# wangxb29/PPST

Hardware: AMD Instinct MI355X
Metric: 512x512 portrait swaps/sec/GPU (higher is better)
Workload: dtype bf16x3 (fp32 split into hi+lo bf16, 3 MFMA passes, fp32 accumulate); 1 GPU; simple_swapping 512x512 batch=8 per GPU, generator+encoders forward only (BASELINE configs[1]); image_parallel=1 batch per rank, no data-path collective

## Files before the change

### include/ppst_hip.h

```cpp
#ifndef PPST_HIP_H
#define PPST_HIP_H

#include <stddef.h>
#include <stdint.h>

#ifdef __cplusplus
extern "C" {
#endif

#define PPST_OK 0
#define PPST_EINVAL (-1)
#define PPST_EUNSUPPORTED (-2)
#define PPST_ENULL (-3)

enum { PPST_F32 = 0, PPST_F16 = 1, PPST_BF16 = 2, PPST_F64 = 3  };

enum { PPST_PAD_ZERO = 0, PPST_PAD_REFLECT = 1, PPST_PAD_REPLICATE = 2 };

enum { PPST_ACT_NONE = 0, PPST_ACT_LRELU = 1 , PPST_ACT_PRELU = 2 };

#define PPST_ABI_VERSION 3
int ppst_version(void);

#define PPST_ST_F32 0
// ... 80 lines not shown
  const void* noise;
  const void* prelu;
  void* stats;
  const void* residual;
  float noise_weight;
  float out_scale;
  int32_t B, in_h, in_w, in_ld;
  int32_t out_h, out_w, out_ld, cout;
  int32_t nsteps, n_groups;
  int32_t pad_mode;
  int32_t in_off_y, in_off_x;
  int32_t out_sy, out_sx;
  int32_t act;
  int32_t precision;
  int32_t res_ld;
  int32_t tile_h, tile_w;
  int32_t halo;
  int32_t bn;
  const void* in_scale_shift;
  const void* in_prelu;
  int32_t in_c, in_act;
  int32_t flop_steps;
  int32_t tile_rows;
  int32_t a_slots;
  int32_t early_a;
  int32_t variant;
  int32_t reserved0;
  int32_t dual_b;
  int32_t io_st;
  int32_t k64;
  const void* in_res;
  int32_t in_res_ld;
  int32_t ksplit;
  const int32_t* ksplit_starts;
  void* ksplit_scratch;
  unsigned* ksplit_flags;
  uint32_t ksplit_epoch;
} ppst_conv_args;

int ppst_conv2d_mfma(const ppst_conv_args* a, void* stream);
int64_t ppst_conv_pack_wino_bytes(int cout, int cin);
int ppst_conv_pack_wino(const void* w, int64_t sn, int64_t sc, int64_t sy, int64_t sx, float scale, int cout, int cin,
                        void* out, void* stream);
int ppst_conv2d_f32(const ppst_conv_args* a, const void* w, int64_t sn, int64_t sc, int64_t sy, int64_t sx, float wscale,
                    const int32_t* src_c, const int32_t* src_ky, const int32_t* src_kx, void* stream);
int ppst_conv_tiles(int tile_h, int tile_w, int tile_rows);

int ppst_conv1x1_small_cin(const void* x, const void* w, const void* bias, void* y,
                           int64_t npix, int cin, int in_ld, int cout, float wscale,
                           int act, void* stream);
int ppst_conv1x1_small_cin_st(const void* x, const void* w, const void* bias, void* y,
                              int64_t npix, int cin, int in_ld, int cout, float wscale,
                              int act, int y_st , void* stream);
int ppst_conv1x1_small_cout(const void* x, const void* w, const void* bias, void* y,
                            int64_t npix, int cin, int cout, float wscale, void* stream);
int ppst_conv1x1_small_cout_st(const void* x, const void* w, const void* bias, void* y,
                               int64_t npix, int cin, int cout, float wscale, int x_st , void* stream);
int ppst_torgb_apply_st(const void* x, const void* scale_shift, const void* res, int res_ld, float out_scale, const void* w,
                        const void* bias, void* y, int B, int H, int W, int cin, float wscale, int x_st, void* stream);

int ppst_in_stats(const void* x, void* partial, int B, int H, int W, int C, int ld,
                  int rep_pad, int* n_partials, void* stream);
int ppst_in_finalize(const void* partial, int n_partials, const void* style,
                     int style_ld ,
                     const void* post_bias ,
                     void* scale_shift , int B, int C, double count,
                     float eps, void* stream);
int ppst_affine_act(const void* x, const void* scale_shift, const void* res,
                    const void* res_scale_shift , void* y,
                    int B, int64_t hw, int C, int x_ld, int res_ld, int y_ld,
                    int act , const void* prelu,
                    float out_scale,
                    int res_up2_w ,
                    void* stream);
int ppst_affine_act_st(const void* x, const void* scale_shift, const void* res, const void* res_scale_shift, void* y,
                       int B, int64_t hw, int C, int x_ld, int res_ld, int y_ld, int act, const void* prelu,
                       float out_scale, int res_up2_w, int x_st, int y_st, void* stream);
int ppst_affine_act_stats(const void* x, const void* scale_shift, const void* res,
                          const void* res_scale_shift, void* y, void* partial,
                          int B, int H, int W, int C, int x_ld, int res_ld, int y_ld,
                          int act, const void* prelu, float out_scale, int rep_pad,
                          int res_up2 , void* stream);
int ppst_upsample_nearest2(const void* x, void* y, int B, int H, int W, int C, void* stream);
int ppst_upsample_nearest2_st(const void* x, void* y, int B, int H, int W, int C, int st, void* stream);

int64_t ppst_gap_gmp_ws(int B, int64_t hw, int C);
int ppst_gap_gmp(const void* x, const void* mask, void* out, void* ws, int B, int H, int W,
                 int C, int ld, void* stream);
int ppst_gap_gmp_st(const void* x, const void* mask, void* out, void* ws, int B, int H, int W,
                    int C, int ld, int x_st, void* stream);
int ppst_avgpool(const void* x, void* y, int B, int H, int W, int C, int x_ld, int f,
                 int y_ld, void* stream);
int ppst_bilinear(const void* x, void* y, int B, int H, int W, int C, int x_ld,
                  int OH, int OW, int y_ld, void* stream);
int ppst_head_tail(const void* x, const void* scale_shift, const void* prelu, void* feat, void* feat1,
                   int B, int H, int W, int C, int x_ld, int feat_ld, int feat1_ld, int P, int D, int act,
                   void* stream);
int ppst_maxpool2(const void* x, void* y, int B, int H, int W, int C, void* stream);

int ppst_linear(const void* x, const void* w, const void* bias, void* y,
                int B, int K, int N, float wscale, float bscale, int relu_in, int act,
                void* stream);
int ppst_l2norm_rows(const void* x, void* y, int B, int K, float eps, int mode, void* stream);
int ppst_lerp(const void* a, const void* b, void* y, int64_t n, float r, void* stream);
int ppst_spatial_modulation(const void* x, const void* scale, const void* bias, void* y,
                            int B, int64_t hw, int C, void* stream);
// ... 160 lines not shown
```

### ppst_amd/_lib.py

```python
import ctypes
import os

import torch

HERE = os.path.dirname(os.path.abspath(__file__))
LIB_PATH = os.environ.get("PPST_HIP_LIB") or os.path.join(HERE, "libppst_hip.so")

if not os.path.exists(LIB_PATH):
    raise ImportError(
        "ppst_amd: %s is missing -- build it with `python -m ppst_amd.build` "
        "(hipcc --offload-arch=gfx950). There is no CPU fallback." % LIB_PATH)

lib = ctypes.CDLL(LIB_PATH)

vp, i32, i64, f32, f64 = ctypes.c_void_p, ctypes.c_int, ctypes.c_int64, ctypes.c_float, ctypes.c_double


class PackJob(ctypes.Structure):
    _fields_ = [("w", vp), ("sn", i64), ("sc", i64), ("sy", i64), ("sx", i64), ("src_c", vp), ("src_ky", vp), ("src_kx", vp),
                ("out", vp), ("total", i64), ("block0", i64), ("scale", f32), ("cout", i32), ("bn", i32), ("nsteps", i32),
                ("n_groups", i32), ("x3", i32), ("f16", i32), ("nblocks", i32), ("dual", i32)]


class UpscaleJob(ctypes.Structure):
    _fields_ = [("w", vp), ("out", vp), ("total", i64), ("block0", i64), ("scale", f32), ("cout", i32), ("cin", i32), ("nblocks", i32)]


class ConvArgs(ctypes.Structure):
    _fields_ = [
        ("x", vp), ("wpack", vp), ("steps", vp), ("y", vp), ("bias", vp), ("noise", vp),
        ("prelu", vp), ("stats", vp), ("residual", vp),
        ("noise_weight", f32), ("out_scale", f32),
        ("B", i32), ("in_h", i32), ("in_w", i32), ("in_ld", i32),
        ("out_h", i32), ("out_w", i32), ("out_ld", i32), ("cout", i32),
        ("nsteps", i32), ("n_groups", i32), ("pad_mode", i32),
        ("in_off_y", i32), ("in_off_x", i32), ("out_sy", i32), ("out_sx", i32),
        ("act", i32), ("precision", i32), ("res_ld", i32), ("tile_h", i32), ("tile_w", i32),
        ("halo", i32), ("bn", i32), ("in_scale_shift", vp), ("in_prelu", vp), ("in_c", i32), ("in_act", i32),
        ("flop_steps", i32), ("tile_rows", i32), ("a_slots", i32), ("early_a", i32), ("variant", i32), ("reserved0", i32), ("dual_b", i32), ("io_st", i32), ("k64", i32),
        ("in_res", vp), ("in_res_ld", i32), ("ksplit", i32), ("ksplit_starts", vp),
        ("ksplit_scratch", vp), ("ksplit_flags", vp), ("ksplit_epoch", ctypes.c_uint32),
    ]


_SIGS = {
    "ppst_version": (i32, []),
    "ppst_guided_filter_tune": (i32, [i32, i32]),
    "ppst_upfirdn2d": (i32, [vp, vp, vp] + [i32] * 14 + [i32, vp]),
    "ppst_blur_nhwc": (i32, [vp, vp, vp] + [i32] * 10 + [vp, i32, vp]),
    "ppst_blur_nhwc_st": (i32, [vp, vp, vp] + [i32] * 10 + [vp, i32, i32, vp]),
    "ppst_fused_bias_act": (i32, [vp, vp, vp, vp, i64, i32, i32, i32, i32, f32, f32, i32, vp]),
    "ppst_nchw_to_nhwc": (i32, [vp, vp, i32, i32, i32, i32, vp]),
    "ppst_nhwc_to_nchw": (i32, [vp, vp, i32, i32, i32, i32, vp]),
    "ppst_conv_pack": (i32, [vp, i64, i64, i64, i64, f32, i32, i32, vp, vp, vp, i32, i32, i32, vp, vp]),
    "ppst_conv_pack_k64": (i32, [vp, i64, i64, i64, i64, f32, i32, i32, vp, vp, vp, i32, i32, i32, i32, vp, vp]),
    "ppst_conv_pack_up9_bytes": (i64, [i32, i32]),
    "ppst_conv_pack_up9": (i32, [vp, i64, i64, i64, i64, f32, i32, i32, vp, vp]),
    "ppst_conv_pack_wino_bytes": (i64, [i32, i32]),
    "ppst_conv_pack_wino": (i32, [vp, i64, i64, i64, i64, f32, i32, i32, vp, vp]),
    "ppst_conv_pack_dual": (i32, [vp, i64, i64, i64, i64, f32, i32, vp, vp, vp, i32, i32, i32, vp, vp]),
    "ppst_upscale_weight": (i32, [vp, vp, i32, i32, f32, vp]),
    "ppst_dgrad_s2d_stack_weight": (i32, [vp, vp, i32, i32, vp]),
    "ppst_depth_to_space_st": (i32, [vp, vp, i32, i32, i32, i32, i32, i32, i32, vp]),
    "ppst_pack_job_blocks": (i32, [i64]),
    "ppst_conv_pack_batch": (i32, [vp, i32, i32, vp]),
    "ppst_upscale_weight_batch": (i32, [vp, i32, i32, vp]),
    "ppst_conv2d_mfma": (i32, [ctypes.POINTER(ConvArgs), vp]),
    "ppst_conv2d_f32": (i32, [ctypes.POINTER(ConvArgs), vp, i64, i64, i64, i64, f32, vp, vp, vp, vp]),
    "ppst_conv_tiles": (i32, [i32, i32, i32]),
    "ppst_conv1x1_small_cin": (i32, [vp, vp, vp, vp, i64, i32, i32, i32, f32, i32, vp]),
    "ppst_conv1x1_small_cin_st": (i32, [vp, vp, vp, vp, i64, i32, i32, i32, f32, i32, i32, vp]),
    "ppst_conv1x1_small_cout": (i32, [vp, vp, vp, vp, i64, i32, i32, f32, vp]),
    "ppst_conv1x1_small_cout_st": (i32, [vp, vp, vp, vp, i64, i32, i32, f32, i32, vp]),
    "ppst_torgb_apply_st": (i32, [vp, vp, vp, i32, f32, vp, vp, vp, i32, i32, i32, i32, f32, i32, vp]),
    "ppst_in_stats": (i32, [vp, vp, i32, i32, i32, i32, i32, i32, ctypes.POINTER(i32), vp]),
    "ppst_in_finalize": (i32, [vp, i32, vp, i32, vp, vp, i32, i32, f64, f32, vp]),
    "ppst_affine_act": (i32, [vp, vp, vp, vp, vp, i32, i64, i32, i32, i32, i32, i32, vp, f32, i32, vp]),
    "ppst_affine_act_st": (i32, [vp, vp, vp, vp, vp, i32, i64, i32, i32, i32, i32, i32, vp, f32, i32, i32, i32, vp]),
    "ppst_affine_act_stats": (i32, [vp, vp, vp, vp, vp, vp, i32, i32, i32, i32, i32, i32, i32, i32, vp, f32, i32, i32, vp]),
    "ppst_upsample_nearest2": (i32, [vp, vp, i32, i32, i32, i32, vp]),
    "ppst_upsample_nearest2_st": (i32, [vp, vp, i32, i32, i32, i32, i32, vp]),
    "ppst_gap_gmp_ws": (i64, [i32, i64, i32]),
    "ppst_gap_gmp": (i32, [vp, vp, vp, vp, i32, i32, i32, i32, i32, vp]),
    "ppst_gap_gmp_st": (i32, [vp, vp, vp, vp, i32, i32, i32, i32, i32, i32, vp]),
    "ppst_avgpool": (i32, [vp, vp, i32, i32, i32, i32, i32, i32, i32, vp]),
    "ppst_bilinear": (i32, [vp, vp, i32, i32, i32, i32, i32, i32, i32, i32, vp]),
    "ppst_head_tail": (i32, [vp, vp, vp, vp, vp] + [i32] * 10 + [vp]),
    "ppst_maxpool2": (i32, [vp, vp, i32, i32, i32, i32, vp]),
    "ppst_linear": (i32, [vp, vp, vp, vp, i32, i32, i32, f32, f32, i32, i32, vp]),
    "ppst_l2norm_rows": (i32, [vp, vp, i32, i32, f32, i32, vp]),
    "ppst_lerp": (i32, [vp, vp, vp, i64, f32, vp]),
    "ppst_spatial_modulation": (i32, [vp, vp, vp, vp, i32, i64, i32, vp]),
    "ppst_spatial_modulation_st": (i32, [vp, vp, vp, vp, i32, i64, i32, i32, vp]),
    "ppst_rselfcorr": (i32, [vp, vp, i32, i32, i32, i32, i32, vp]),
    "ppst_corr_prep": (i32, [vp, vp, i32, i32, i32, i32, vp]),
    "ppst_gemm_nt_f32": (i32, [vp, vp, vp, i32, i32, i32, i32, f32, vp]),
    "ppst_gemm_nn_f32": (i32, [vp, vp, vp, i32, i32, i32, i32, i32, i32, vp]),
    "ppst_unfold_rows": (i32, [vp, vp, i32, i32, i32, i32, i32, vp]),
    "ppst_unfold_rows_bwd": (i32, [vp, vp, i32, i32, i32, i32, i32, vp]),
    "ppst_gemm_nt_split": (i32, [vp, vp, vp, i32, i32, i32, i32, f32, i32, vp]),
    "ppst_gemm_nn_split": (i32, [vp, vp, vp, i32, i32, i32, i32, i32, i32, i32, vp]),
    "ppst_softmax_rows": (i32, [vp, i64, i32, f32, vp]),
    "ppst_unfold_patches": (i32, [vp, vp, i32, i32, i32, i32, i32, vp]),
    "ppst_fold_patches": (i32, [vp, vp, i32, i32, i32, i32, i32, vp]),
    "ppst_tensor2im_u8": (i32, [vp, vp, i32, i32, i32, i32, vp]),
    "ppst_resample_u8": (i32, [vp, vp, i32, i32, i32, i32, i32, i32, vp, vp, i32, vp]),
    "ppst_u8_to_tensor": (i32, [vp, vp, i32, i32, i32, i32, f32, f32, vp]),
    "ppst_png_bound": (i64, [i32, i32, i32]),
    "ppst_png_ws": (i64, [i32, i32, i32, i32]),
    "ppst_png_encode": (i32, [vp, vp, vp, i32, i32, i32, i32, vp, vp]),
    "ppst_lpips_pack_floats": (i64, []),
    "ppst_lpips_pack": (i32, [vp, vp, vp, vp, vp, vp, vp]),
    "ppst_lpips_dims": (i32, [i32, i32, ctypes.POINTER(i32)]),
    "ppst_lpips_ws": (i64, [i32, i32, i32]),
    "ppst_lpips_trunk": (i32, [vp, vp, ctypes.POINTER(i64), i32, vp, ctypes.POINTER(i64), i32, i32, i32, vp, vp]),
    "ppst_lpips_feature": (i32, [vp, i32, i32, i32, i32, vp, vp]),
    "ppst_lpips_tail": (i32, [vp, vp, i32, i32, i32, vp, vp]),
    "ppst_lpips_bwd_ws": (i64, [i32, i32, i32, i32]),
    "ppst_lpips_backward": (i32, [vp, vp, vp, i32, i32, i32, i32, vp, vp, vp, vp]),
    "ppst_guided_filter_ws": (i64, [i32, i32, i32]),
    "ppst_guided_filter": (i32, [vp, vp, vp, vp, i32, i32, i32, i32, f32, vp, vp]),
    "ppst_smooth_local_affine_ws": (i64, [i32, i32, i32]),
    "ppst_smooth_local_affine": (i32, [vp, vp, vp, vp, vp, i32, i32, i32, i32, i32, f32, f32, vp]),
    "ppst_conv_wgrad_f32": (i32, [vp, vp, vp, vp, vp] + [i32] * 11 + [vp]),
# ... 83 lines not shown
```

### ppst_amd/build.py

```python
import os
import subprocess
import sys
from concurrent.futures import ThreadPoolExecutor

HERE = os.path.dirname(os.path.abspath(__file__))
CSRC = os.path.join(HERE, "csrc")
OBJ = os.path.join(HERE, "csrc", "_obj")
LIB = os.path.join(HERE, "libppst_hip.so")
SOURCES = ["upfirdn2d.hip", "fused_bias_act.hip", "elementwise.hip", "linear.hip", "conv_mfma.hip", "conv_mfma2.hip", "conv1x1.hip", "conv_wino.hip", "conv_f32.hip",
           "corr.hip", "guided_filter.hip", "train.hip", "train_g.hip", "imageio.hip", "smooth_filter.hip", "png.hip", "lpips.hip"]
FLAGS = ["--offload-arch=gfx950", "-O3", "-fPIC", "-std=c++17", "-Wno-unused-result"]
FILE_FLAGS = {"conv_wino.hip": ["-fno-slp-vectorize"]}


def _hipcc():
    for c in (os.environ.get("HIPCC"), "/opt/rocm/bin/hipcc", "hipcc"):
        if c and (os.path.isabs(c) and os.path.exists(c) or not os.path.isabs(c)):
            return c
    return "hipcc"


HEADERS = [os.path.join(CSRC, "common.h"), os.path.join(CSRC, "rscl_common.h"), os.path.join(HERE, "..", "include", "ppst_hip.h")]


def _stale(target, deps):
    return not os.path.exists(target) or any(os.path.getmtime(d) > os.path.getmtime(target) for d in deps)


def needs_build():
    return (_stale(LIB, [os.path.join(CSRC, s) for s in SOURCES] + HEADERS) or
            any(_stale(os.path.join(OBJ, s.replace(".hip", ".o")), [os.path.join(CSRC, s)]) for s in SOURCES if os.path.isdir(OBJ)))


def build(force=False, verbose=True):
    if not force and not needs_build():
        return LIB
    os.makedirs(OBJ, exist_ok=True)
    hipcc = _hipcc()

    def cc(src):
        obj = os.path.join(OBJ, src.replace(".hip", ".o"))
        if not force and not _stale(obj, [os.path.join(CSRC, src)] + HEADERS):
            return obj
        cmd = [hipcc] + FLAGS + FILE_FLAGS.get(src, []) + ["-c", os.path.join(CSRC, src), "-o", obj]
        r = subprocess.run(cmd, capture_output=True, text=True)
        if r.returncode != 0:
            raise RuntimeError("hipcc failed for %s:\n%s" % (src, r.stderr))
        return obj

    order = sorted(SOURCES, key=lambda f: 0 if f.startswith("conv") else 1)
    with ThreadPoolExecutor(max_workers=8) as ex:
        objs = dict(zip(order, ex.map(cc, order)))
    cmd = [hipcc, "--offload-arch=gfx950", "-shared", "-fPIC", "-o", LIB] + [objs[s_] for s_ in SOURCES]
    r = subprocess.run(cmd, capture_output=True, text=True)
    if r.returncode != 0:
        raise RuntimeError("link failed:\n%s" % r.stderr)
    if verbose:
        print("built", LIB)
    return LIB


if __name__ == "__main__":
    build(force="--force" in sys.argv)
```

### ppst_amd/csrc/conv1x1.hip

```cpp
#include "common.h"

struct C1Args {
  const float* x;
  const unsigned char* wpack;
  const int4* steps;
  float* y;
  const float* bias;
  const float* noise;
  const float* prelu;
  float* stats;
  const float* residual;
  float noise_weight, out_scale;
  int B, hw, in_ld, out_ld, cout, nsteps, act, res_ld, n_tiles, tiles;
  int in_h, in_w, out_h, out_w, tiles_x, pad_mode;
  const float* in_ss;
  const float* in_prelu;
  int in_c, in_act;
  const float* in_res;
  int in_res_ld;
};

#define C1_GROUP 8
#define C1_BLOB 8192

typedef _Float16 __attribute__((ext_vector_type(8))) c1_half8;
template <int PREC>
__device__ __forceinline__ void c1_cvt(float v, unsigned short& h, unsigned short& l) {
  if (PREC == 0) split_bf16(v, h, l);
  else if (PREC == 3) { h = __builtin_bit_cast(unsigned short, (_Float16)v); l = 0; }
  else { h = f2bf(v); l = 0; }
}
template <int PREC>
__device__ __forceinline__ void c1_cvt8(const float (&v)[8], bf16x8& hi, bf16x8& lo) {
  if (PREC == 3) {
#pragma unroll
    for (int j = 0; j < 8; ++j) {
      unsigned short h, l;
      c1_cvt<PREC>(v[j], h, l);
      hi[j] = (short)h;
      lo[j] = (short)l;
    }
    return;
  }
  uint2 h0, l0 = make_uint2(0u, 0u), h1, l1 = make_uint2(0u, 0u);
  if (PREC == 0) {
    split_bf16x4(make_float4(v[0], v[1], v[2], v[3]), h0, l0);
    split_bf16x4(make_float4(v[4], v[5], v[6], v[7]), h1, l1);
  } else {
    h0 = f2bf_x4(make_float4(v[0], v[1], v[2], v[3]));
    h1 = f2bf_x4(make_float4(v[4], v[5], v[6], v[7]));
  }
  hi = __builtin_bit_cast(bf16x8, make_uint4(h0.x, h0.y, h1.x, h1.y));
  lo = __builtin_bit_cast(bf16x8, make_uint4(l0.x, l0.y, l1.x, l1.y));
// ... 241 lines not shown
        if (IOS != PPST_ST_F32 && !INSS) {
          const float4 z = vok[mt] ? raw[mt][0] : make_float4(0.f, 0.f, 0.f, 0.f);
          ah[mt] = __builtin_bit_cast(bf16x8, z);
          al[mt] = ah[mt];
          continue;
        }
        float v[8] = {raw[mt][0].x, raw[mt][0].y, raw[mt][0].z, raw[mt][0].w, raw[mt][1].x, raw[mt][1].y, raw[mt][1].z, raw[mt][1].w};
        if (IOS != PPST_ST_F32) c1_unpack8<IOS>(raw[mt][0], v);
        if (INSS) {
          const float sc[8] = {ss[0].x, ss[0].z, ss[1].x, ss[1].z, ss[2].x, ss[2].z, ss[3].x, ss[3].z};
          const float sh[8] = {ss[0].y, ss[0].w, ss[1].y, ss[1].w, ss[2].y, ss[2].w, ss[3].y, ss[3].w};
#pragma unroll
          for (int j = 0; j < 8; ++j) {
            float t = sc[j] * v[j] + sh[j];
            if (INSS == 2) {
              const float4 r4 = rres[mt][j >> 2];
              t += (j & 3) == 0 ? r4.x : (j & 3) == 1 ? r4.y : (j & 3) == 2 ? r4.z : r4.w;
            }
            v[j] = in_act(t);
          }
        }
#pragma unroll
        for (int j = 0; j < 8; ++j)
          if (!vok[mt]) v[j] = 0.f;
        c1_cvt8<PREC>(v, ah[mt], al[mt]);
      }
      if (s + 1 < a.nsteps) a_load(steps[s + 1]);
      const unsigned char* bs = (const unsigned char*)sB + sl * BLOB1 + g * 1024 + r16 * 16;
#pragma unroll
      for (int nt = 0; nt < NT; ++nt) {
        const bf16x8 bh = *(const bf16x8*)(bs + nt * 256);
        bf16x8 bl = bh;
        if (X3) bl = *(const bf16x8*)(bs + nt * 256 + 4096);
#pragma unroll
        for (int mt = 0; mt < MT; ++mt) acc[mt][nt] = c1_mfma<PREC>(bh, bl, ah[mt], al[mt], acc[mt][nt]);
      }
    }
  }

  c1_epilogue<MT, NT, TAPS, X3, IOS>(a, acc, red, b, mblk, ntile, pbase, oy0, ox, tid, wave, r16, g);
}

#define C3_GROUP 9
template <int CTRL>
__device__ __forceinline__ bf16x8 c3_shift(bf16x8 edge, bf16x8 centre) {
  typedef int __attribute__((ext_vector_type(4))) i4;
  const i4 e = __builtin_bit_cast(i4, edge), c = __builtin_bit_cast(i4, centre);
  i4 r;
#pragma unroll
  for (int i = 0; i < 4; ++i) r[i] = __builtin_amdgcn_update_dpp(e[i], c[i], CTRL, 0xf, 0xf, false);
  return __builtin_bit_cast(bf16x8, r);
}

template <bool INSS, int NT_, int PREC = 0, int IOS = PPST_ST_F32>
__global__ __launch_bounds__(512, NT_ > 4 ? 2 : 4) void conv3x3_direct_kernel(C1Args a) {
  constexpr int MT = 2, NT = NT_;
  constexpr bool X3 = PREC == 0;
  static_assert(IOS == PPST_ST_F32 || IOS == (PREC == 3 ? PPST_ST_F16 : PREC == 1 ? PPST_ST_BF16 : -1), "half storage: single-pass modes");
  constexpr int ES = IOS == PPST_ST_F32 ? 4 : 2;
  constexpr int PSTR = (NT > 4 ? 128 : 64) * 16;
  constexpr int BLOB = (X3 ? 8 : 4) * PSTR;
  __shared__ uint4 sB[C3_GROUP * BLOB / 16];
  __shared__ float red[8][NT > 4 ? 128 : 64][2];
  const int tid = threadIdx.x, lane = tid & 63, wave = __builtin_amdgcn_readfirstlane(tid >> 6);
  const int r16 = lane & 15, g = lane >> 4;
  const int total = a.B * a.tiles * a.n_tiles;
  const int per = (total + (int)gridDim.x - 1) / (int)gridDim.x;
  const int w_beg = blockIdx.x * per, w_end = w_beg + per < total ? w_beg + per : total;
  const int nchunks = a.nsteps / 9;
  const bool keep_b = nchunks == 1 && a.n_tiles == 1;
  for (int wid = w_beg; wid < w_end; ++wid) {
  const int ntile = wid % a.n_tiles;
  int mblk = wid / a.n_tiles;
  const int b = mblk / a.tiles;
  mblk -= b * a.tiles;
  const int tyi = mblk / a.tiles_x, txi = mblk - tyi * a.tiles_x;
  const int oy0 = tyi * 16 + wave * 2, ox = txi * 16 + r16;
  const unsigned char* xb = (const unsigned char*)a.x + (int64_t)b * a.in_h * a.in_w * a.in_ld * ES;
  const unsigned char* wblob = a.wpack + (int64_t)ntile * a.nsteps * BLOB;
  if (wid > w_beg) __syncthreads();
#if defined(__HIP_DEVICE_COMPILE__)
  typedef const __attribute__((address_space(4))) int4* StepPtr;
#else
  typedef const int4* StepPtr;
#endif
  StepPtr steps = (StepPtr)a.steps;
  const float in_slope = (INSS && a.in_act == PPST_ACT_PRELU && a.in_prelu) ? a.in_prelu[0] : 0.f;
  auto in_act = [&](float t) -> float {
    if (a.in_act == PPST_ACT_LRELU) return (t > 0.f ? t : t * 0.2f) * 1.41421356237309515f;
    if (a.in_act == PPST_ACT_PRELU) return t >= 0.f ? t : t * in_slope;
    return t;
  };
  const int xe_raw = r16 == 0 ? ox - 1 : (r16 == 15 ? ox + 1 : ox);
  const bool cx_ok = ox < a.in_w, ex_ok = xe_raw >= 0 && xe_raw < a.in_w;
  const int cx = c1_pad(ox, a.in_w, a.pad_mode), ex = c1_pad(xe_raw, a.in_w, a.pad_mode);

  f32x4 acc[MT][NT];
#pragma unroll
  for (int i = 0; i < MT; ++i)
#pragma unroll
    for (int j = 0; j < NT; ++j) acc[i][j] = (f32x4){0.f, 0.f, 0.f, 0.f};

  float4 rawc[2], rawe[2], ss[4];
  bool okc = false, oke = false;
  auto row_load = [&](int chan, int r) {
    int iy = oy0 - 1 + r;
    const bool yok = iy >= 0 && iy < a.in_h;
    iy = c1_pad(iy, a.in_h, a.pad_mode);
    okc = a.pad_mode != PPST_PAD_ZERO || (yok && cx_ok);
    oke = a.pad_mode != PPST_PAD_ZERO || (yok && ex_ok);
    const float4* pc = (const float4*)(xb + (((int64_t)iy * a.in_w + cx) * a.in_ld + chan + g * 8) * ES);
    const float4* pe = (const float4*)(xb + (((int64_t)iy * a.in_w + ex) * a.in_ld + chan + g * 8) * ES);
    rawc[0] = pc[0];
    rawe[0] = pe[0];
    if (IOS == PPST_ST_F32) { rawc[1] = pc[1]; rawe[1] = pe[1]; }
  };
  auto ss_load = [&](int chan) {
    if (INSS) {
      const float4* q = (const float4*)(a.in_ss + ((int64_t)b * a.in_c + chan + g * 8) * 2);
      ss[0] = q[0]; ss[1] = q[1]; ss[2] = q[2]; ss[3] = q[3];
    }
  };
  auto convert = [&](const float4 (&raw)[2], bool ok, bf16x8& hi, bf16x8& lo) {
    if (IOS != PPST_ST_F32 && !INSS) {
      hi = __builtin_bit_cast(bf16x8, ok ? raw[0] : make_float4(0.f, 0.f, 0.f, 0.f));
      lo = hi;
      return;
    }
    float v[8] = {raw[0].x, raw[0].y, raw[0].z, raw[0].w, raw[1].x, raw[1].y, raw[1].z, raw[1].w};
    if (IOS != PPST_ST_F32) c1_unpack8<IOS>(raw[0], v);
    if (INSS) {
      const float sc[8] = {ss[0].x, ss[0].z, ss[1].x, ss[1].z, ss[2].x, ss[2].z, ss[3].x, ss[3].z};
      const float sh[8] = {ss[0].y, ss[0].w, ss[1].y, ss[1].w, ss[2].y, ss[2].w, ss[3].y, ss[3].w};
#pragma unroll
      for (int j = 0; j < 8; ++j) v[j] = in_act(sc[j] * v[j] + sh[j]);
    }
#pragma unroll
    for (int j = 0; j < 8; ++j)
      if (!ok) v[j] = 0.f;
    c1_cvt8<PREC>(v, hi, lo);
  };

  int chan = steps[0].x;
  ss_load(chan);
  row_load(chan, 0);
  for (int c = 0; c < nchunks; ++c) {
    if (!keep_b || wid == w_beg) {
      if (c) __syncthreads();
      for (int i = tid; i < C3_GROUP * (BLOB / 16); i += 512) sB[i] = ((const uint4*)(wblob + (int64_t)c * C3_GROUP * BLOB))[i];
      __syncthreads();
    }
    const int chan_next = c + 1 < nchunks ? steps[(c + 1) * 9].x : chan;
#pragma unroll
    for (int r = 0; r < 4; ++r) {
      bf16x8 ch, cl, eh, el;
      convert(rawc, okc, ch, cl);
      convert(rawe, oke, eh, el);
      if (r < 3) row_load(chan, r + 1);
      else if (c + 1 < nchunks) { ss_load(chan_next); row_load(chan_next, 0); }
#pragma unroll
      for (int dxi = 0; dxi < 3; ++dxi) {
        const bf16x8 fh = dxi == 0 ? c3_shift<0x111>(eh, ch) : (dxi == 1 ? ch : c3_shift<0x101>(eh, ch));
        const bf16x8 fl = dxi == 0 ? c3_shift<0x111>(el, cl) : (dxi == 1 ? cl : c3_shift<0x101>(el, cl));
#pragma unroll
        for (int mt = 0; mt < MT; ++mt) {
          const int dyi = r - mt;
          if (dyi < 0 || dyi > 2) continue;
          const unsigned char* bs = (const unsigned char*)sB + (dyi * 3 + dxi) * BLOB + g * PSTR + r16 * 16;
#pragma unroll
          for (int nt = 0; nt < NT; ++nt) {
            const bf16x8 bh = *(const bf16x8*)(bs + nt * 256);
            bf16x8 bl = bh;
            if (X3) bl = *(const bf16x8*)(bs + nt * 256 + 4 * PSTR);
            acc[mt][nt] = c1_mfma<PREC>(bh, bl, fh, fl, acc[mt][nt]);
          }
        }
// ... 13 lines not shown
  k.bias = (const float*)a->bias; k.noise = (const float*)a->noise; k.prelu = (const float*)a->prelu;
  k.stats = (float*)a->stats; k.residual = (const float*)a->residual;
  k.noise_weight = a->noise_weight; k.out_scale = a->out_scale;
  k.B = a->B; k.hw = a->out_h * a->out_w; k.in_ld = a->in_ld; k.out_ld = a->out_ld; k.cout = a->cout; k.nsteps = a->nsteps;
  k.act = a->act; k.res_ld = a->res_ld; k.n_tiles = n_tiles; k.tiles = tiles;
  k.in_ss = (const float*)a->in_scale_shift; k.in_prelu = (const float*)a->in_prelu; k.in_c = a->in_c; k.in_act = a->in_act;
  k.in_res = (const float*)a->in_res; k.in_res_ld = a->in_res_ld;
  if ((int64_t)tiles * 256 < k.hw) return PPST_EINVAL;
  if (k.in_res) {
    PPST_LAUNCH((conv1x1_stream_kernel<2, false, 4, 0, PPST_ST_F32>), dim3((unsigned)blocks_of(a, tiles, n_tiles)), dim3(512), 0, st, k);
    return PPST_LAUNCH_CHECK();
  }
  const int64_t blocks = (int64_t)a->B * tiles * n_tiles;
  if (blocks > 0x7fffffff) return PPST_EINVAL;
#define LS(PREC_, IOS_)                                                                                               \
  do {                                                                                                                \
    if (k.in_ss) PPST_LAUNCH((conv1x1_stream_kernel<1, false, 4, PREC_, IOS_>), dim3((unsigned)blocks), dim3(512), 0, st, k);   \
    else PPST_LAUNCH((conv1x1_stream_kernel<0, false, 4, PREC_, IOS_>), dim3((unsigned)blocks), dim3(512), 0, st, k);          \
  } while (0)
  if (a->precision == 1) { if (a->io_st) LS(1, PPST_ST_BF16); else LS(1, PPST_ST_F32); }
  else if (a->precision == 3) { if (a->io_st) LS(3, PPST_ST_F16); else LS(3, PPST_ST_F32); }
  else LS(0, PPST_ST_F32);
#undef LS
  return PPST_LAUNCH_CHECK();
}

int ppst_conv_direct_launch(const ppst_conv_args* a, int n_tiles, int tiles_y, int tiles_x, hipStream_t st) {
  C1Args k;
  k.x = (const float*)a->x; k.wpack = (const unsigned char*)a->wpack; k.steps = (const int4*)a->steps; k.y = (float*)a->y;
  k.bias = (const float*)a->bias; k.noise = (const float*)a->noise; k.prelu = (const float*)a->prelu;
  k.stats = (float*)a->stats; k.residual = (const float*)a->residual;
  k.noise_weight = a->noise_weight; k.out_scale = a->out_scale;
  k.B = a->B; k.hw = a->out_h * a->out_w; k.in_ld = a->in_ld; k.out_ld = a->out_ld; k.cout = a->cout; k.nsteps = a->nsteps;
  k.act = a->act; k.res_ld = a->res_ld; k.n_tiles = n_tiles; k.tiles = tiles_y * tiles_x;
  k.in_ss = (const float*)a->in_scale_shift; k.in_prelu = (const float*)a->in_prelu; k.in_c = a->in_c; k.in_act = a->in_act;
  k.in_h = a->in_h; k.in_w = a->in_w; k.out_h = a->out_h; k.out_w = a->out_w; k.tiles_x = tiles_x; k.pad_mode = a->pad_mode;
  const int64_t blocks = (int64_t)a->B * k.tiles * n_tiles;
  if (blocks > 0x7fffffff) return PPST_EINVAL;
  const bool nt2 = a->cout <= 32;
#define LD(INSS_, PREC_, IOS_)                                                                                       \
  do {                                                                                                               \
    if (nt2) PPST_LAUNCH((conv1x1_stream_kernel<INSS_, true, 2, PREC_, IOS_>), dim3((unsigned)blocks), dim3(512), 0, st, k);       \
    else PPST_LAUNCH((conv1x1_stream_kernel<INSS_, true, 4, PREC_, IOS_>), dim3((unsigned)blocks), dim3(512), 0, st, k);           \
  } while (0)
#define LDP(PREC_, IOS_) do { if (k.in_ss) LD(1, PREC_, IOS_); else LD(0, PREC_, IOS_); } while (0)
  if (a->precision == 1) { if (a->io_st) LDP(1, PPST_ST_BF16); else LDP(1, PPST_ST_F32); }
  else if (a->precision == 3) { if (a->io_st) LDP(3, PPST_ST_F16); else LDP(3, PPST_ST_F32); }
  else LDP(0, PPST_ST_F32);
#undef LDP
#undef LD
  return PPST_LAUNCH_CHECK();
}

int ppst_conv3x3_direct_launch(const ppst_conv_args* a, int n_tiles, int tiles_y, int tiles_x, hipStream_t st) {
  if (a->nsteps % 9) return PPST_EINVAL;
  C1Args k;
  k.x = (const float*)a->x; k.wpack = (const unsigned char*)a->wpack; k.steps = (const int4*)a->steps; k.y = (float*)a->y;
  k.bias = (const float*)a->bias; k.noise = (const float*)a->noise; k.prelu = (const float*)a->prelu;
  k.stats = (float*)a->stats; k.residual = (const float*)a->residual;
  k.noise_weight = a->noise_weight; k.out_scale = a->out_scale;
  k.B = a->B; k.hw = a->out_h * a->out_w; k.in_ld = a->in_ld; k.out_ld = a->out_ld; k.cout = a->cout; k.nsteps = a->nsteps;
  k.act = a->act; k.res_ld = a->res_ld; k.n_tiles = n_tiles; k.tiles = tiles_y * tiles_x;
  k.in_ss = (const float*)a->in_scale_shift; k.in_prelu = (const float*)a->in_prelu; k.in_c = a->in_c; k.in_act = a->in_act;
  k.in_h = a->in_h; k.in_w = a->in_w; k.out_h = a->out_h; k.out_w = a->out_w; k.tiles_x = tiles_x; k.pad_mode = a->pad_mode;
  int64_t blocks = (int64_t)a->B * k.tiles * n_tiles;
  if (blocks > 0x7fffffff) return PPST_EINVAL;
  if (a->nsteps == 9 && n_tiles == 1 && blocks > 512) blocks = 512;
  const bool nt2 = a->cout <= 32, nt8 = a->bn == 128;
#define LD3(INSS_, PREC_, IOS_)                                                                                      \
  do {                                                                                                               \
    if (nt8 && PREC_ == 0) PPST_LAUNCH((conv3x3_direct_kernel<INSS_, 8, 0>), dim3((unsigned)blocks), dim3(512), 0, st, k);   \
    else if (nt8) return PPST_EUNSUPPORTED;                                                                          \
    else if (nt2) PPST_LAUNCH((conv3x3_direct_kernel<INSS_, 2, PREC_, IOS_>), dim3((unsigned)blocks), dim3(512), 0, st, k); \
    else PPST_LAUNCH((conv3x3_direct_kernel<INSS_, 4, PREC_, IOS_>), dim3((unsigned)blocks), dim3(512), 0, st, k);          \
  } while (0)
#define LD3P(PREC_, IOS_) do { if (k.in_ss) LD3(true, PREC_, IOS_); else LD3(false, PREC_, IOS_); } while (0)
  if (a->precision == 1) { if (a->io_st) LD3P(1, PPST_ST_BF16); else LD3P(1, PPST_ST_F32); }
  else if (a->precision == 3) { if (a->io_st) LD3P(3, PPST_ST_F16); else LD3P(3, PPST_ST_F32); }
  else LD3P(0, PPST_ST_F32);
#undef LD3P
#undef LD3
  return PPST_LAUNCH_CHECK();
}
```

### ppst_amd/csrc/conv_mfma.hip

```cpp
#include "common.h"

struct ConvKArgs {
  const float* x;
  const unsigned short* wpack;
  const int4* steps;
  float* y;
  const float* bias;
  const float* noise;
  const float* prelu;
  float* stats;
  const float* residual;
  float noise_weight, out_scale;
  int B, in_h, in_w, in_ld, out_h, out_w, out_ld, cout;
  int nsteps, n_groups, pad_mode, in_off_y, in_off_x, out_sy, out_sx, act, res_ld, tile_h, tile_w;
  int tiles_y, tiles_x, n_tiles;
  const float* in_ss;
  const float* in_prelu;
  int in_c, in_act;
  int early_a;
  unsigned long long* dbg;
  KSplitDev ks;
  int prefetch_w;
};

__device__ __forceinline__ int pad_index(int i, int n, int mode) {
  if (mode == PPST_PAD_REFLECT) {
    if (i < 0) i = -i;
    if (i >= n) i = 2 * (n - 1) - i;
  }
  i = i < 0 ? 0 : (i >= n ? n - 1 : i);
  return i;
}

#ifdef PPST_CONV_CLOCK
__device__ unsigned long long* g_clock_buf = nullptr;
__device__ int g_clock_n = 1;
extern "C" int ppst_conv_clock_buffer(void* buf, int n) {
  if (n <= 0) return PPST_EINVAL;
  if (hipMemcpyToSymbol(HIP_SYMBOL(g_clock_buf), &buf, sizeof(buf)) != hipSuccess) return PPST_EINVAL;
  return hipMemcpyToSymbol(HIP_SYMBOL(g_clock_n), &n, sizeof(n)) == hipSuccess ? PPST_OK : PPST_EINVAL;
}
#endif
typedef _Float16 __attribute__((ext_vector_type(8))) half8;
__device__ __forceinline__ unsigned short f2h(float f) { return __builtin_bit_cast(unsigned short, (_Float16)f); }
template <int WM, int WN, int HALO, bool X3, bool INSS, int NAS = 0, bool F16 = false, int IOS = PPST_ST_F32>
__global__ __launch_bounds__(64 * WM * WN, NAS ? 2 : 1) void conv_mfma_kernel(ConvKArgs a) {
  static_assert(IOS == PPST_ST_F32 || (!X3 && IOS == (F16 ? PPST_ST_F16 : PPST_ST_BF16)), "half storage: single-pass modes");
  constexpr int ES = IOS == PPST_ST_F32 ? 4 : 2;
  constexpr int NT = 64 * WM * WN;
  constexpr int TH = 4 * WM, TW = 16;
  constexpr int HH = TH + 2 * HALO, HW = TW + 2 * HALO, HP = HH * HW;
  constexpr int PLANE = (WM == 2) ? HP * 16 : ((HP * 16 + 255) / 256) * 256;
  constexpr int NPL = X3 ? 8 : 4;
// ... 717 lines not shown

int ppst_prof_begin_(double flop, const int* info8, hipStream_t st) {
  if (!g_prof_on) return -1;
  if (g_ev_used >= PROF_MAX) { ++g_prof_dropped; return -1; }
  while (g_ev_made <= g_ev_used) {
    if (hipEventCreate(&g_ev[g_ev_made][0]) != hipSuccess || hipEventCreate(&g_ev[g_ev_made][1]) != hipSuccess) return -1;
    ++g_ev_made;
  }
  const int slot = g_ev_used++;
  g_flop[slot] = flop;
  for (int i = 0; i < 8; ++i) g_info[slot][i] = info8[i];
  (void)hipEventRecord(g_ev[slot][0], st);
  return slot;
}
void ppst_prof_end_(int slot, hipStream_t st) {
  if (slot >= 0) (void)hipEventRecord(g_ev[slot][1], st);
}

extern "C" int ppst_prof_enable(int on) {
  g_prof_on = on;
  g_ev_used = 0;
  if (on) g_prof_dropped = 0;
  return PPST_OK;
}
extern "C" int ppst_prof_collect(double* ms, int64_t* launches, double* flop) {
  double t = 0.0, f = 0.0;
  for (int i = 0; i < g_ev_used; ++i) {
    float e = 0.f;
    hipError_t err = hipEventElapsedTime(&e, g_ev[i][0], g_ev[i][1]);
    if (err != hipSuccess) return (int)err;
    t += e;
    f += g_flop[i];
  }
  if (ms) *ms = t;
  if (launches) *launches = g_ev_used;
  if (flop) *flop = f;
  g_ev_used = 0;
  return PPST_OK;
}
extern "C" int ppst_prof_detail(int idx, double* ms, double* flop, int32_t* info) {
  if (idx < 0 || idx >= g_ev_used) return PPST_EINVAL;
  float e = 0.f;
  hipError_t err = hipEventElapsedTime(&e, g_ev[idx][0], g_ev[idx][1]);
  if (err != hipSuccess) return (int)err;
  if (ms) *ms = e;
  if (flop) *flop = g_flop[idx];
  if (info) for (int i = 0; i < 8; ++i) info[i] = g_info[idx][i];
  return PPST_OK;
}

int ppst_conv2d_mfma2_launch(const ppst_conv_args* a, int n_tiles, int tiles_y, int tiles_x, hipStream_t st);
int ppst_conv1x1_stream_launch(const ppst_conv_args* a, int n_tiles, int tiles, hipStream_t st);
int ppst_conv_direct_launch(const ppst_conv_args* a, int n_tiles, int tiles_y, int tiles_x, hipStream_t st);
int ppst_conv3x3_direct_launch(const ppst_conv_args* a, int n_tiles, int tiles_y, int tiles_x, hipStream_t st);
int ppst_conv_wino_launch(const ppst_conv_args* a, int n_tiles, int tiles_y, int tiles_x, hipStream_t st);

int ppst_ksplit_prepare_(const ppst_conv_args* a, int64_t tiles, int acc_regs, int threads, KSplitDev* out) {
  const int S = a->ksplit, nsteps = a->nsteps;
  const int32_t* starts = a->ksplit_starts;
  if ((S != 2 && S != 4 && S != 8) || (!starts && nsteps % S) || tiles <= 0 || acc_regs <= 0 || acc_regs % 4 || threads <= 0) return PPST_EINVAL;
  if (S == 8 && acc_regs > 64) return PPST_EINVAL;
  for (int i = 0; i <= S; ++i) {
    out->start[i] = starts ? starts[i] : i * (nsteps / S);
    if (i && out->start[i] <= out->start[i - 1]) return PPST_EINVAL;
  }
  if (out->start[0] != 0 || out->start[S] != nsteps) return PPST_EINVAL;
  const int64_t slots = (int64_t)(S - 1) * tiles;
  if (slots > KS_MAX_SLOTS || slots > PPST_KSPLIT_FLAG_WORDS - 1 || (size_t)slots * threads * acc_regs * 4 > PPST_KSPLIT_SCRATCH_BYTES) return PPST_EINVAL;
  if (!a->ksplit_scratch || !a->ksplit_flags) return PPST_ENULL;
  if (a->ksplit_epoch == 0) return PPST_EINVAL;
  out->scratch = (float*)a->ksplit_scratch; out->flags = a->ksplit_flags; out->epoch = a->ksplit_epoch; out->S = S;
  return PPST_OK;
}

extern "C" int ppst_conv_tiles(int tile_h, int tile_w, int tile_rows) { return cdiv(tile_h, tile_rows) * cdiv(tile_w, tile_rows == 15 ? 15 : 16); }

template <int WM, int WN, int HALO, bool X3, int NAS = 0, bool F16 = false, int IOS = PPST_ST_F32>
static void launch_conv(const ConvKArgs& k, int blocks, hipStream_t st) {
  const dim3 grid(blocks, k.ks.S > 1 ? k.ks.S : 1);
  if (k.in_ss) PPST_LAUNCH((conv_mfma_kernel<WM, WN, HALO, X3, true, NAS, F16, IOS>), grid, dim3(64 * WM * WN), 0, st, k);
  else PPST_LAUNCH((conv_mfma_kernel<WM, WN, HALO, X3, false, NAS, F16, IOS>), grid, dim3(64 * WM * WN), 0, st, k);
}

extern "C" int ppst_conv2d_mfma(const ppst_conv_args* a, void* stream) {
  if (!a) return PPST_ENULL;
  if (a->B < 0 || a->in_h <= 0 || a->in_w <= 0 || a->in_ld <= 0 || a->in_ld % 4 || a->out_h <= 0 || a->out_w <= 0 ||
      a->out_ld < a->cout || a->cout <= 0 || a->cout % 4 || a->out_ld % 4 || (a->residual && a->res_ld % 4) || a->nsteps <= 0 ||
      (a->n_groups != 1 && a->n_groups != 4 && !(a->n_groups == 2 && a->dual_b)) || a->pad_mode < 0 ||
      (a->dual_b && (a->variant != 2 || a->bn != 256 || a->n_groups != 2 || a->halo != 1 || (a->precision != 0 && a->precision != 1 && a->precision != 3) || a->out_sy != 2 || a->out_sx != 2 || !a->early_a)) ||
      a->pad_mode > 2 || a->tile_h <= 0 || a->tile_w <= 0 || a->out_sy <= 0 || a->out_sx <= 0 ||
      (a->precision != 0 && a->precision != 1 && a->precision != 3) || a->halo < 0 || a->halo > 1 || (a->bn != 64 && a->bn != 128 && a->bn != 256) || (a->residual && a->res_ld < a->cout) ||
      a->variant < 0 || a->variant > 11 || (a->variant == 0 && a->bn == 256) ||
      (a->variant == 11 && (a->precision != 0 || a->bn != 256 || a->halo != 1 || a->n_groups != 1 || a->out_sy != 2 || a->out_sx != 2 ||
                            !a->early_a || a->tile_rows != 15 || a->pad_mode != PPST_PAD_ZERO || a->in_scale_shift || a->residual ||
                            (a->act & 0xff) == PPST_ACT_PRELU || a->cout % 64 || a->nsteps % 4 || a->in_off_y || a->in_off_x ||
                            a->tile_h != a->in_h || a->tile_w != a->in_w || a->out_h != 2 * a->in_h || a->out_w != 2 * a->in_w || a->io_st)) ||
      (a->variant == 10 && (a->precision != 0 || a->bn != 128 || a->halo != 1 || a->n_groups != 1 || a->out_sy != 1 || a->out_sx != 1 ||
                            a->in_off_y != 0 || a->in_off_x != 0 || a->tile_h != a->out_h || a->tile_w != a->out_w ||
                            a->in_h != a->out_h || a->in_w != a->out_w || a->nsteps % 9 != 0 || a->tile_rows != 16 ||
                            (a->in_scale_shift && a->nsteps / 9 > 32))) ||
      ((a->variant == 2 || a->variant == 7 || a->variant == 9) &&
       ((a->precision != 0 && !((a->variant == 2 || a->variant == 7 || (a->variant == 9 && a->k64)) && (a->precision == 1 || a->precision == 3))) || a->bn == 64 || !a->early_a)) ||
      (a->variant == 7 && (a->bn != 128 || a->tile_rows != 32)) ||
      (a->variant == 9 && (a->bn != 128 || a->tile_rows != 24)) ||
      (a->variant == 2 && a->bn != 256) ||
      (a->variant == 4 && ((a->precision != 0 && a->precision != 1 && a->precision != 3) || a->bn != 64 || a->halo != 0 || a->n_groups != 1 || a->out_sy != 1 || a->out_sx != 1 ||
                           a->in_off_y != 0 || a->in_off_x != 0 || a->tile_h != a->out_h || a->tile_w != a->out_w ||
                           a->in_h != a->out_h || a->in_w != a->out_w)) ||
      (a->in_res && (a->variant != 4 || !a->in_scale_shift || a->precision != 0 || a->io_st || a->in_res_ld < a->in_c || a->in_res_ld % 4 ||
                     ((uintptr_t)a->in_res % 16))) ||
      ((a->variant == 5 || a->variant == 6) && ((a->precision != 0 && a->precision != 1 && a->precision != 3) ||
                                                (a->bn != 64 && !(a->variant == 6 && a->bn == 128 && a->precision == 0)) || a->n_groups != 1 || a->out_sy != 1 || a->out_sx != 1 ||
                           a->in_off_y != 0 || a->in_off_x != 0 || a->tile_h != a->out_h || a->tile_w != a->out_w)) ||
      (a->tile_rows != 16 && !(a->variant == 7 && a->tile_rows == 32) && !(a->variant == 9 && a->tile_rows == 24) && !(a->variant == 11 && a->tile_rows == 15) &&
       !(a->variant == 0 && a->tile_rows == 8 && a->bn == 128 && a->halo == 1 && a->early_a && a->precision == 0)) || (a->in_scale_shift && a->in_c <= 0) || a->a_slots < 0 || a->a_slots > 3)
    return PPST_EINVAL;
  if (a->variant == 1 || a->variant == 3 || (a->variant == 7 && a->precision == 0) || a->variant == 8 || (a->variant == 9 && !a->k64) ||
      a->reserved0)
    return PPST_EINVAL;
  if (a->io_st && (a->io_st != (a->precision == 3 ? PPST_ST_F16 : a->precision == 1 ? PPST_ST_BF16 : -1) ||
                   (a->tile_rows != 16 && a->variant != 7 && !(a->variant == 9 && a->k64)) ||
                   !(a->variant == 0 || a->variant == 2 || a->variant == 4 || a->variant == 5 || a->variant == 6 || a->variant == 7 || (a->variant == 9 && a->k64))))
    return PPST_EINVAL;
  if (a->k64 && (!a->io_st || !a->halo || !((a->variant == 2 && a->bn == 256) || (a->variant == 9 && a->bn == 128 && a->tile_rows == 24)) || !a->early_a))
    return PPST_EINVAL;
  {
    const int64_t px = (int64_t)a->out_h * a->out_w + 64 * (int64_t)a->out_sx;
    if (px * a->out_ld > 0x7fffffff || (a->residual && px * a->res_ld > 0x7fffffff)) return PPST_EINVAL;
  }
  if ((int64_t)a->in_h * a->in_w * a->in_ld * 4 > 0x7fffffff) return PPST_EINVAL;
  if (a->io_st && (((uintptr_t)a->x | (uintptr_t)a->y | (uintptr_t)a->residual) % 8)) return PPST_EINVAL;
  if (a->io_st && a->variant >= 4 && a->variant <= 6 && (a->in_ld % 8 || (uintptr_t)a->x % 16)) return PPST_EINVAL;
  if ((a->tile_h - 1) * a->out_sy >= a->out_h || (a->tile_w - 1) * a->out_sx >= a->out_w) return PPST_EINVAL;
  if (a->B == 0) return PPST_OK;
  if (!a->x || !a->wpack || !a->steps || !a->y) return PPST_ENULL;
  ConvKArgs k;
  k.x = (const float*)a->x; k.wpack = (const unsigned short*)a->wpack; k.steps = (const int4*)a->steps; k.y = (float*)a->y;
  k.bias = (const float*)a->bias; k.noise = (const float*)a->noise; k.prelu = (const float*)a->prelu;
  k.stats = (float*)a->stats; k.residual = (const float*)a->residual;
  k.noise_weight = a->noise_weight; k.out_scale = a->out_scale;
  k.B = a->B; k.in_h = a->in_h; k.in_w = a->in_w; k.in_ld = a->in_ld; k.out_h = a->out_h; k.out_w = a->out_w;
  k.out_ld = a->out_ld; k.cout = a->cout; k.nsteps = a->nsteps; k.n_groups = a->n_groups; k.pad_mode = a->pad_mode;
  k.in_off_y = a->in_off_y; k.in_off_x = a->in_off_x; k.out_sy = a->out_sy; k.out_sx = a->out_sx; k.act = a->act;
  k.res_ld = a->res_ld; k.tile_h = a->tile_h; k.tile_w = a->tile_w;
  k.tiles_y = cdiv(a->tile_h, a->tile_rows); k.tiles_x = cdiv(a->tile_w, a->variant == 11 ? 15 : 16);
  k.n_tiles = cdiv(a->cout, a->variant == 11 ? 64 : a->dual_b ? a->bn / 2 : a->bn);
  k.in_ss = (const float*)a->in_scale_shift; k.in_prelu = (const float*)a->in_prelu;
  k.in_c = a->in_c; k.in_act = a->in_act;
  k.early_a = a->early_a ? 1 : 0;
  k.dbg = nullptr;
  k.ks.scratch = nullptr; k.ks.flags = nullptr; k.ks.epoch = 0; k.ks.S = 1;
#ifdef PPST_CONV_TRACE
  k.dbg = (unsigned long long*)a->prelu;
  k.prelu = nullptr;
#endif
  int64_t blocks64 = (int64_t)a->n_groups * k.n_tiles * a->B * k.tiles_y * k.tiles_x;
  if (blocks64 > 0x7fffffff) return PPST_EINVAL;
  int blocks = (int)blocks64;
  hipStream_t st = as_stream(stream);
  if (a->ksplit > 1) {
    if (a->variant == 0) {
      if (a->tile_rows != 16 && a->tile_rows != 8) return PPST_EINVAL;
      const int e0 = ppst_ksplit_prepare_(a, blocks, 64, (a->bn == 128 && a->tile_rows == 16) ? 512 : 256, &k.ks);
      if (e0 != PPST_OK) return e0;
    } else if (a->variant != 2 && a->variant != 10) return PPST_EINVAL;
  }
  k.prefetch_w = (int64_t)blocks * k.ks.S <= 512 ? 1 : 0;
  int slot = -1;
  if (g_prof_on) {
    const int inf[8] = {a->B, a->tile_h, a->tile_w, a->nsteps, a->cout, a->n_groups, a->halo,
                        a->bn | (a->variant << 12) | ((a->k64 ? 1 : 0) << 20) | (a->precision << 24)};
    slot = ppst_prof_begin_(2.0 * 32.0 * (a->flop_steps > 0 ? a->flop_steps : a->nsteps) * (double)((a->dual_b || a->variant == 11) ? 4 : a->n_groups) * a->cout * (double)a->B * a->tile_h * a->tile_w,
                            inf, st);
  }
  if (a->variant >= 1) {
    int e2 = a->variant == 4   ? ppst_conv1x1_stream_launch(a, k.n_tiles, k.tiles_y * k.tiles_x, st)
             : a->variant == 5 ? ppst_conv_direct_launch(a, k.n_tiles, k.tiles_y, k.tiles_x, st)
             : a->variant == 6 ? ppst_conv3x3_direct_launch(a, k.n_tiles, k.tiles_y, k.tiles_x, st)
             : a->variant == 10 ? ppst_conv_wino_launch(a, k.n_tiles, k.tiles_y, k.tiles_x, st)
                               : ppst_conv2d_mfma2_launch(a, k.n_tiles, k.tiles_y, k.tiles_x, st);
    if (slot >= 0) (void)hipEventRecord(g_ev[slot][1], st);
    return e2;
  }
  const bool x3 = a->precision == 0;
  const bool f16 = a->precision == 3, hs = a->io_st != 0;
#define DISPATCH(WM_, WN_)                                                                                         \
  do {                                                                                                             \
    if (a->halo) { if (x3) launch_conv<WM_, WN_, 1, true>(k, blocks, st); else if (f16 && hs) launch_conv<WM_, WN_, 1, false, 0, true, PPST_ST_F16>(k, blocks, st); else if (f16) launch_conv<WM_, WN_, 1, false, 0, true>(k, blocks, st); else if (hs) launch_conv<WM_, WN_, 1, false, 0, false, PPST_ST_BF16>(k, blocks, st); else launch_conv<WM_, WN_, 1, false>(k, blocks, st); } \
    else         { if (x3) launch_conv<WM_, WN_, 0, true>(k, blocks, st); else if (f16 && hs) launch_conv<WM_, WN_, 0, false, 0, true, PPST_ST_F16>(k, blocks, st); else if (f16) launch_conv<WM_, WN_, 0, false, 0, true>(k, blocks, st); else if (hs) launch_conv<WM_, WN_, 0, false, 0, false, PPST_ST_BF16>(k, blocks, st); else launch_conv<WM_, WN_, 0, false>(k, blocks, st); } \
  } while (0)
  if (a->tile_rows == 8) launch_conv<2, 2, 1, true, 2>(k, blocks, st);
  else if (a->bn == 64 && x3 && a->halo == 1 && a->a_slots == 1) launch_conv<4, 1, 1, true, 1>(k, blocks, st);
  else if (a->bn == 64 && x3 && a->halo == 0 && a->a_slots == 1) launch_conv<4, 1, 0, true, 1>(k, blocks, st);
  else if (a->bn == 64 && x3 && a->halo == 0 && a->a_slots == 2) launch_conv<4, 1, 0, true, 2>(k, blocks, st);
  else if (a->bn == 128) DISPATCH(4, 2); else DISPATCH(4, 1);
#undef DISPATCH
  int e = PPST_LAUNCH_CHECK();
  if (slot >= 0) (void)hipEventRecord(g_ev[slot][1], st);
  return e;
}
```

### ppst_amd/csrc/elementwise.hip

```cpp
#include "common.h"

#define GRID_CAP (256 * 16)
static inline unsigned grid_for(int64_t work, int threads = 256) {
  int64_t b = cdiv64(work, threads);
  if (b > GRID_CAP) b = GRID_CAP;
  if (b < 1) b = 1;
  return (unsigned)b;
}

__device__ __forceinline__ float act_apply(float t, int act, float slope);

template <int ST = PPST_ST_F32>
__device__ __forceinline__ float4 res_up2_sample(const void* __restrict__ res, int b, int oy, int ox, int H, int W, int res_ld,
                                                 int c) {
  const int h = H >> 1, w = W >> 1;
  float fy = fmaxf(((float)oy + 0.5f) * 0.5f - 0.5f, 0.f), fx = fmaxf(((float)ox + 0.5f) * 0.5f - 0.5f, 0.f);
  int y0 = (int)fy, x0 = (int)fx;
  int y1 = y0 + (y0 < h - 1), x1 = x0 + (x0 < w - 1);
  float ly = fy - (float)y0, lx = fx - (float)x0, hy = 1.f - ly, hx = 1.f - lx;
  const int64_t base = (int64_t)b * h * w * res_ld + c;
  float4 v00 = st_ld4<ST>(res, base + ((int64_t)y0 * w + x0) * res_ld);
  float4 v01 = st_ld4<ST>(res, base + ((int64_t)y0 * w + x1) * res_ld);
  float4 v10 = st_ld4<ST>(res, base + ((int64_t)y1 * w + x0) * res_ld);
  float4 v11 = st_ld4<ST>(res, base + ((int64_t)y1 * w + x1) * res_ld);
  float4 o;
  o.x = hy * (hx * v00.x + lx * v01.x) + ly * (hx * v10.x + lx * v11.x);
  o.y = hy * (hx * v00.y + lx * v01.y) + ly * (hx * v10.y + lx * v11.y);
  o.z = hy * (hx * v00.z + lx * v01.z) + ly * (hx * v10.z + lx * v11.z);
  o.w = hy * (hx * v00.w + lx * v01.w) + ly * (hx * v10.w + lx * v11.w);
  return o;
}

__global__ __launch_bounds__(256) void nchw_to_nhwc_kernel(const float* __restrict__ x, float* __restrict__ y, int C, int64_t P) {
  __shared__ float sm[32][65];
  const int64_t p0 = (int64_t)blockIdx.x * 64;
  const int c0 = blockIdx.y * 32;
  const int b = blockIdx.z;
  const float* xb = x + (int64_t)b * C * P;
  float* yb = y + (int64_t)b * C * P;
  {
    int tp = threadIdx.x & 63, tc = threadIdx.x >> 6;
#pragma unroll
    for (int i = 0; i < 8; ++i) {
      int c = c0 + tc + i * 4;
      int64_t p = p0 + tp;
      sm[tc + i * 4][tp] = (c < C && p < P) ? xb[(int64_t)c * P + p] : 0.f;
    }
  }
  __syncthreads();
  {
    int tc = threadIdx.x & 31, tp = threadIdx.x >> 5;
#pragma unroll
    for (int i = 0; i < 8; ++i) {
// ... 62 lines not shown
  __shared__ float s0[256], s1[256];
  const int b = blockIdx.y, chunk = blockIdx.x;
  const int P = H * W;
  const int pbeg = chunk * PIX_CHUNK;
  const int pend = (pbeg + PIX_CHUNK < P) ? pbeg + PIX_CHUNK : P;
  int lanesC = 1;
  while (lanesC < C && lanesC < 256) lanesC <<= 1;
  const int rows = 256 / lanesC;
  const int cl = threadIdx.x % lanesC, pr = threadIdx.x / lanesC;
  const float* xb = x + (int64_t)b * P * ld;
  const float* mb = mask ? mask + (int64_t)b * P : nullptr;
  for (int cbase = 0; cbase < C; cbase += lanesC) {
    int c = cbase + cl;
    float a0 = 0.f, a1 = (MODE == 1) ? -INFINITY : 0.f;
    if (c < C) {
      for (int p = pbeg + pr; p < pend; p += rows) {
        float v = xb[(int64_t)p * ld + c];
        if (MODE == 0) {
          float w = 1.f;
          if (rep_pad) {
            int py = p / W, px = p - py * W;
            w = (float)((1 + (py == 0) + (py == H - 1)) * (1 + (px == 0) + (px == W - 1)));
          }
          a0 += w * v;
          a1 += w * v * v;
        } else {
          if (mb) v *= mb[p];
          a0 += v;
          a1 = fmaxf(a1, v);
        }
      }
    }
    s0[threadIdx.x] = a0;
    s1[threadIdx.x] = a1;
    __syncthreads();
    if (pr == 0 && c < C) {
      for (int r = 1; r < rows; ++r) {
        a0 += s0[r * lanesC + cl];
        a1 = (MODE == 1) ? fmaxf(a1, s1[r * lanesC + cl]) : a1 + s1[r * lanesC + cl];
      }
      float* o = partial + (((int64_t)b * nchunks + chunk) * C + c) * 2;
      o[0] = a0;
      o[1] = a1;
    }
    __syncthreads();
  }
}

struct ApplyArgs {
  const float* ss; const float* res; const float* rss; float* y; const float* prelu;
  int res_ld, y_ld, actf; float out_scale;
  int res_up2;
};
template <int MODE, bool APPLY, int XS = PPST_ST_F32>
__global__ __launch_bounds__(256) void chan_reduce4_kernel(const void* __restrict__ x, const float* __restrict__ mask,
                                                           float* __restrict__ partial, int H, int W, int C, int ld,
                                                           int rep_pad, int nchunks, ApplyArgs ap, int PIX_CHUNK, FastDiv d_w) {
  __shared__ float4 s0[256], s1[256];
  const int b = blockIdx.y, chunk = blockIdx.x;
  const int P = H * W;
  const int pbeg = chunk * PIX_CHUNK;
  const int pend = (pbeg + PIX_CHUNK < P) ? pbeg + PIX_CHUNK : P;
  const int c4n = C >> 2;
  int lanes = 1;
  while (lanes < c4n && lanes < 256) lanes <<= 1;
  const int rows = 256 / lanes;
  const int cl = threadIdx.x % lanes, pr = threadIdx.x / lanes;
  const float* mb = mask ? mask + (int64_t)b * P : nullptr;
  const int act = ap.actf & 0xff;
  const bool res_first = (ap.actf >> 8) & 1;
  const float slope = (APPLY && act == PPST_ACT_PRELU && ap.prelu) ? ap.prelu[0] : 0.f;
  for (int cbase = 0; cbase < c4n; cbase += lanes) {
    const int c = (cbase + cl) * 4;
    float4 a0 = make_float4(0.f, 0.f, 0.f, 0.f);
    float4 a1 = (MODE == 1) ? make_float4(-INFINITY, -INFINITY, -INFINITY, -INFINITY) : a0;
    if (c < C) {
      float4 sa = make_float4(1.f, 1.f, 1.f, 1.f), sb = make_float4(0.f, 0.f, 0.f, 0.f);
      float4 ra = sa, rb = sb;
      if (APPLY && ap.ss) {
        const float4* q = (const float4*)(ap.ss + ((int64_t)b * C + c) * 2);
        float4 q0 = q[0], q1 = q[1];
        sa = make_float4(q0.x, q0.z, q1.x, q1.z); sb = make_float4(q0.y, q0.w, q1.y, q1.w);
      }
      if (APPLY && ap.res && ap.rss) {
        const float4* q = (const float4*)(ap.rss + ((int64_t)b * C + c) * 2);
        float4 q0 = q[0], q1 = q[1];
        ra = make_float4(q0.x, q0.z, q1.x, q1.z); rb = make_float4(q0.y, q0.w, q1.y, q1.w);
      }
      for (int p = pbeg + pr; p < pend; p += rows) {
        const int64_t bp = (int64_t)b * P + p;
        unsigned pxu = 0;
        const int py = (APPLY || MODE == 0) ? (int)fd_divmod((unsigned)p, d_w, pxu) : 0, px = (int)pxu;
        float4 v = st_ld4<XS>(x, bp * ld + c);
        if (APPLY) {
          float t[4] = {sa.x * v.x + sb.x, sa.y * v.y + sb.y, sa.z * v.z + sb.z, sa.w * v.w + sb.w};
          float r[4] = {0.f, 0.f, 0.f, 0.f};
          if (ap.res) {
            float4 rv;
            if (ap.res_up2) rv = res_up2_sample(ap.res, b, py, px, H, W, ap.res_ld, c);
            else rv = *(const float4*)(ap.res + bp * ap.res_ld + c);
            r[0] = ra.x * rv.x + rb.x; r[1] = ra.y * rv.y + rb.y; r[2] = ra.z * rv.z + rb.z; r[3] = ra.w * rv.w + rb.w;
          }
#pragma unroll
          for (int i = 0; i < 4; ++i) {
            float tt = t[i];
            if (res_first) tt += r[i];
            tt = act_apply(tt, act, slope);
            if (!res_first) tt += r[i];
            t[i] = tt * ap.out_scale;
          }
          v = make_float4(t[0], t[1], t[2], t[3]);
          *(float4*)(ap.y + bp * ap.y_ld + c) = v;
        }
        if (MODE == 0) {
          float w = 1.f;
          if (rep_pad) w = (float)((1 + (py == 0) + (py == H - 1)) * (1 + (px == 0) + (px == W - 1)));
          a0.x += w * v.x; a0.y += w * v.y; a0.z += w * v.z; a0.w += w * v.w;
          a1.x += w * v.x * v.x; a1.y += w * v.y * v.y; a1.z += w * v.z * v.z; a1.w += w * v.w * v.w;
        } else {
          if (mb) { float m = mb[p]; v.x *= m; v.y *= m; v.z *= m; v.w *= m; }
          a0.x += v.x; a0.y += v.y; a0.z += v.z; a0.w += v.w;
          a1.x = fmaxf(a1.x, v.x); a1.y = fmaxf(a1.y, v.y); a1.z = fmaxf(a1.z, v.z); a1.w = fmaxf(a1.w, v.w);
        }
      }
    }
    s0[threadIdx.x] = a0;
    s1[threadIdx.x] = a1;
    __syncthreads();
    if (pr == 0 && c < C) {
      for (int r = 1; r < rows; ++r) {
        float4 u = s0[r * lanes + cl], w = s1[r * lanes + cl];
        a0.x += u.x; a0.y += u.y; a0.z += u.z; a0.w += u.w;
        if (MODE == 1) { a1.x = fmaxf(a1.x, w.x); a1.y = fmaxf(a1.y, w.y); a1.z = fmaxf(a1.z, w.z); a1.w = fmaxf(a1.w, w.w); }
        else { a1.x += w.x; a1.y += w.y; a1.z += w.z; a1.w += w.w; }
      }
      float4* o = (float4*)(partial + (((int64_t)b * nchunks + chunk) * C + c) * 2);
      o[0] = make_float4(a0.x, a1.x, a0.y, a1.y);
      o[1] = make_float4(a0.z, a1.z, a0.w, a1.w);
    }
    __syncthreads();
  }
}

extern "C" int ppst_in_stats(const void* x, void* partial, int B, int H, int W, int C, int ld, int rep_pad,
                             int* n_partials, void* stream) {
  if (B < 0 || H <= 0 || W <= 0 || C <= 0 || ld < C || (int64_t)H * W > 0x7fffffffll) return PPST_EINVAL;
  const int chunk = pix_chunk(B, (int64_t)H * W);
  int nchunks = (int)cdiv64((int64_t)H * W, chunk);
  if (n_partials) *n_partials = nchunks;
  if (!x && !partial) return PPST_OK;
  if (B == 0) return PPST_OK;
  if (!x || !partial) return PPST_ENULL;
  if (C % 4 == 0 && ld % 4 == 0 && ((uintptr_t)x % 16) == 0) {
    ApplyArgs ap = {};
    PPST_LAUNCH((chan_reduce4_kernel<0, false>), dim3(nchunks, B), dim3(256), 0, as_stream(stream), x,
                (const float*)nullptr, (float*)partial, H, W, C, ld, rep_pad, nchunks, ap, chunk, make_fastdiv(W));
  } else {
    PPST_LAUNCH(chan_reduce_kernel<0>, dim3(nchunks, B), dim3(256), 0, as_stream(stream), (const float*)x,
                (const float*)nullptr, (float*)partial, H, W, C, ld, rep_pad, nchunks, chunk);
  }
  return PPST_LAUNCH_CHECK();
}

#define FIN_CH 8
#define FIN_ROWS 32
__global__ __launch_bounds__(256) void in_finalize_kernel(const float* __restrict__ partial, int n_partials,
                                                          const float* __restrict__ style, int style_ld,
                                                          const float* __restrict__ post_bias, float* __restrict__ ss, int B,
                                                          int C, double count, float eps, float* __restrict__ mr) {
  __shared__ double sm[FIN_ROWS][FIN_CH][2];
  const int cgroups = (C + FIN_CH - 1) / FIN_CH;
  const int b = blockIdx.x / cgroups, c0 = (blockIdx.x % cgroups) * FIN_CH;
  const int cl = threadIdx.x & (FIN_CH - 1), kk = threadIdx.x / FIN_CH;
  const int c = c0 + cl;
  double s = 0.0, q = 0.0;
  if (c < C) {
    const float2* p = (const float2*)partial + ((int64_t)b * n_partials * C + c);
    int k = kk;
    for (; k + 3 * FIN_ROWS < n_partials; k += 4 * FIN_ROWS) {
      float2 v0 = p[(int64_t)k * C], v1 = p[(int64_t)(k + FIN_ROWS) * C], v2 = p[(int64_t)(k + 2 * FIN_ROWS) * C],
             v3 = p[(int64_t)(k + 3 * FIN_ROWS) * C];
      s += (double)v0.x; q += (double)v0.y;
      s += (double)v1.x; q += (double)v1.y;
      s += (double)v2.x; q += (double)v2.y;
      s += (double)v3.x; q += (double)v3.y;
    }
    for (; k < n_partials; k += FIN_ROWS) {
      float2 v = p[(int64_t)k * C];
      s += (double)v.x;
      q += (double)v.y;
    }
  }
  sm[kk][cl][0] = s;
  sm[kk][cl][1] = q;
  __syncthreads();
  if (kk == 0 && c < C) {
    for (int r = 1; r < FIN_ROWS; ++r) { s += sm[r][cl][0]; q += sm[r][cl][1]; }
    double mean = s / count;
    double var = q / count - mean * mean;
    if (var < 0.0) var = 0.0;
    double rstd = 1.0 / sqrt(var + (double)eps);
    double a = rstd, sh = -mean * rstd;
    if (style) {
      double s0 = (double)style[(int64_t)b * style_ld + c] + 1.0;
      double s1 = (double)style[(int64_t)b * style_ld + C + c];
      a = rstd * s0;
      sh = s1 - mean * a;
    }
    if (post_bias) sh += (double)post_bias[c];
// ... 113 lines not shown
  if (total > PPST_IDX32_MAX) return PPST_EINVAL;
  const FastDiv d_cv = make_fastdiv((unsigned)(C / V)), d_hw = make_fastdiv((unsigned)hw),
                d_w = make_fastdiv(res_up2_w > 0 ? (unsigned)res_up2_w : 1u);
#define AA_GO(XS_, YS_)                                                                                                   \
  do {                                                                                                                    \
    if (w8) PPST_LAUNCH((affine_act_kernel<8, XS_, YS_>), dim3(grid_for(total)), dim3(256), 0, as_stream(stream), x,      \
                        (const float*)scale_shift, res, (const float*)res_scale_shift, y, (unsigned)hw, C, x_ld, res_ld, y_ld, act, \
                        (const float*)prelu, out_scale, (unsigned)total, res_up2_w, d_cv, d_hw, d_w);                      \
    else PPST_LAUNCH((affine_act_kernel<4, XS_, YS_>), dim3(grid_for(total)), dim3(256), 0, as_stream(stream), x,         \
                     (const float*)scale_shift, res, (const float*)res_scale_shift, y, (unsigned)hw, C, x_ld, res_ld, y_ld, act, \
                     (const float*)prelu, out_scale, (unsigned)total, res_up2_w, d_cv, d_hw, d_w);                         \
  } while (0)
  if (vec) {
    if (x_st == PPST_ST_F16 && y_st == PPST_ST_F16) AA_GO(PPST_ST_F16, PPST_ST_F16);
    else if (x_st == PPST_ST_F16) AA_GO(PPST_ST_F16, PPST_ST_F32);
    else if (x_st == PPST_ST_BF16 && y_st == PPST_ST_BF16) AA_GO(PPST_ST_BF16, PPST_ST_BF16);
    else if (x_st == PPST_ST_BF16) AA_GO(PPST_ST_BF16, PPST_ST_F32);
    else if (y_st == PPST_ST_F16) AA_GO(PPST_ST_F32, PPST_ST_F16);
    else if (y_st == PPST_ST_BF16) AA_GO(PPST_ST_F32, PPST_ST_BF16);
    else PPST_LAUNCH((affine_act_kernel<4>), dim3(grid_for(total)), dim3(256), 0, as_stream(stream), x,
                     (const float*)scale_shift, res, (const float*)res_scale_shift, y, (unsigned)hw, C, x_ld, res_ld, y_ld, act,
                     (const float*)prelu, out_scale, (unsigned)total, res_up2_w, d_cv, d_hw, d_w);
  } else
    PPST_LAUNCH(affine_act_kernel<1>, dim3(grid_for(total)), dim3(256), 0, as_stream(stream), x,
                       (const float*)scale_shift, res, (const float*)res_scale_shift, y, (unsigned)hw, C, x_ld,
                       res_ld, y_ld, act, (const float*)prelu, out_scale, (unsigned)total, 0, d_cv, d_hw, d_w);
#undef AA_GO
  return PPST_LAUNCH_CHECK();
}
extern "C" int ppst_affine_act(const void* x, const void* scale_shift, const void* res, const void* res_scale_shift, void* y,
                               int B, int64_t hw, int C, int x_ld, int res_ld, int y_ld, int act, const void* prelu,
                               float out_scale, int res_up2_w, void* stream) {
  return ppst_affine_act_st(x, scale_shift, res, res_scale_shift, y, B, hw, C, x_ld, res_ld, y_ld, act, prelu, out_scale, res_up2_w,
                            PPST_ST_F32, PPST_ST_F32, stream);
}

extern "C" int ppst_affine_act_stats(const void* x, const void* scale_shift, const void* res, const void* res_scale_shift,
                                     void* y, void* partial, int B, int H, int W, int C, int x_ld, int res_ld, int y_ld,
                                     int act, const void* prelu, float out_scale, int rep_pad, int res_up2, void* stream) {
  if (B < 0 || H <= 0 || W <= 0 || C <= 0 || C % 4 || x_ld % 4 || y_ld % 4 || x_ld < C || y_ld < C ||
      (res && (res_ld < C || res_ld % 4)))
    return PPST_EINVAL;
  if (B == 0) return PPST_OK;
  if (!x || !y || !partial) return PPST_ENULL;
  if ((int64_t)H * W > 0x7fffffffll) return PPST_EINVAL;
  const int chunk = pix_chunk(B, (int64_t)H * W);
  int nchunks = (int)cdiv64((int64_t)H * W, chunk);
  ApplyArgs ap;
  ap.ss = (const float*)scale_shift; ap.res = (const float*)res; ap.rss = (const float*)res_scale_shift; ap.y = (float*)y;
  ap.prelu = (const float*)prelu; ap.res_ld = res_ld; ap.y_ld = y_ld; ap.actf = act; ap.out_scale = out_scale;
  ap.res_up2 = (res && res_up2) ? 1 : 0;
  if (ap.res_up2 && (H % 2 || W % 2)) return PPST_EINVAL;
  PPST_LAUNCH((chan_reduce4_kernel<0, true>), dim3(nchunks, B), dim3(256), 0, as_stream(stream), x,
              (const float*)nullptr, (float*)partial, H, W, C, x_ld, rep_pad, nchunks, ap, chunk, make_fastdiv(W));
  return PPST_LAUNCH_CHECK();
}

__global__ __launch_bounds__(256) void gap_gmp_finalize_kernel(const float* __restrict__ partial, int n_partials,
                                                               float* __restrict__ out, int B, int C, double count) {
  __shared__ double ss[FIN_ROWS][FIN_CH];
  __shared__ float sm[FIN_ROWS][FIN_CH];
  const int cgroups = (C + FIN_CH - 1) / FIN_CH;
  const int b = blockIdx.x / cgroups, c0 = (blockIdx.x % cgroups) * FIN_CH;
  const int cl = threadIdx.x & (FIN_CH - 1), kk = threadIdx.x / FIN_CH;
  const int c = c0 + cl;
  double s = 0.0;
  float m = -INFINITY;
  if (c < C) {
    const float2* p = (const float2*)partial + ((int64_t)b * n_partials * C + c);
    int k = kk;
    for (; k + 3 * FIN_ROWS < n_partials; k += 4 * FIN_ROWS) {
      float2 v0 = p[(int64_t)k * C], v1 = p[(int64_t)(k + FIN_ROWS) * C], v2 = p[(int64_t)(k + 2 * FIN_ROWS) * C],
             v3 = p[(int64_t)(k + 3 * FIN_ROWS) * C];
      s += (double)v0.x; s += (double)v1.x; s += (double)v2.x; s += (double)v3.x;
      m = fmaxf(fmaxf(m, v0.y), fmaxf(v1.y, fmaxf(v2.y, v3.y)));
    }
    for (; k < n_partials; k += FIN_ROWS) {
      float2 v = p[(int64_t)k * C];
      s += (double)v.x;
      m = fmaxf(m, v.y);
    }
  }
  ss[kk][cl] = s;
  sm[kk][cl] = m;
  __syncthreads();
  if (kk == 0 && c < C) {
    for (int r = 1; r < FIN_ROWS; ++r) { s += ss[r][cl]; m = fmaxf(m, sm[r][cl]); }
    out[(int64_t)b * 2 * C + c] = (float)(s / count);
    out[(int64_t)b * 2 * C + C + c] = m;
  }
}
extern "C" int64_t ppst_gap_gmp_ws(int B, int64_t hw, int C) {
  if (B <= 0 || hw <= 0) return 0;
  return cdiv64(hw, pix_chunk(B, hw)) * C * 2 * B * (int64_t)sizeof(float);
}
extern "C" int ppst_gap_gmp_st(const void* x, const void* mask, void* out, void* ws, int B, int H, int W, int C, int ld,
                                int x_st, void* stream) {
  if ((unsigned)x_st > 2u || (x_st && (C % 4 || ld % 4 || (uintptr_t)x % 8))) return PPST_EINVAL;
  if (B < 0 || H <= 0 || W <= 0 || C <= 0 || ld < C) return PPST_EINVAL;
  if (B == 0) return PPST_OK;
  if (!x || !out || !ws) return PPST_ENULL;
  if ((int64_t)H * W > 0x7fffffffll) return PPST_EINVAL;
  const int chunk = pix_chunk(B, (int64_t)H * W);
  int nchunks = (int)cdiv64((int64_t)H * W, chunk);
  if (x_st) {
    ApplyArgs ap = {};
    if (x_st == PPST_ST_F16)
      PPST_LAUNCH((chan_reduce4_kernel<1, false, PPST_ST_F16>), dim3(nchunks, B), dim3(256), 0, as_stream(stream), x,
                  (const float*)mask, (float*)ws, H, W, C, ld, 0, nchunks, ap, chunk, make_fastdiv(W));
    else
      PPST_LAUNCH((chan_reduce4_kernel<1, false, PPST_ST_BF16>), dim3(nchunks, B), dim3(256), 0, as_stream(stream), x,
                  (const float*)mask, (float*)ws, H, W, C, ld, 0, nchunks, ap, chunk, make_fastdiv(W));
  } else if (C % 4 == 0 && ld % 4 == 0 && ((uintptr_t)x % 16) == 0) {
    ApplyArgs ap = {};
    PPST_LAUNCH((chan_reduce4_kernel<1, false>), dim3(nchunks, B), dim3(256), 0, as_stream(stream), x,
                (const float*)mask, (float*)ws, H, W, C, ld, 0, nchunks, ap, chunk, make_fastdiv(W));
  } else {
    PPST_LAUNCH(chan_reduce_kernel<1>, dim3(nchunks, B), dim3(256), 0, as_stream(stream), (const float*)x,
                (const float*)mask, (float*)ws, H, W, C, ld, 0, nchunks, chunk);
  }
  int e = PPST_LAUNCH_CHECK();
  if (e) return e;
  PPST_LAUNCH(gap_gmp_finalize_kernel, dim3(B * cdiv(C, FIN_CH)), dim3(256), 0, as_stream(stream),
                     (const float*)ws, nchunks, (float*)out, B, C, (double)H * W);
  return PPST_LAUNCH_CHECK();
}
extern "C" int ppst_gap_gmp(const void* x, const void* mask, void* out, void* ws, int B, int H, int W, int C, int ld,
                             void* stream) {
  return ppst_gap_gmp_st(x, mask, out, ws, B, H, W, C, ld, PPST_ST_F32, stream);
}


#define GGM_MAXH 4
template <int XS = PPST_ST_F32>
__global__ __launch_bounds__(256) void gap_gmp_multi_kernel(const void* __restrict__ x, const float* __restrict__ masks,
                                                            float* __restrict__ partial, int P, int C, int ld, int nm, int with_plain,
                                                            int B, int nchunks, int PIX_CHUNK) {
  __shared__ float4 s0[256], s1[256];
  const int b = blockIdx.y, chunk = blockIdx.x;
  const int pbeg = chunk * PIX_CHUNK;
  const int pend = (pbeg + PIX_CHUNK < P) ? pbeg + PIX_CHUNK : P;
  const int c4n = C >> 2;
  int lanes = 1;
  while (lanes < c4n && lanes < 256) lanes <<= 1;
  const int rows = 256 / lanes;
  const int cl = threadIdx.x % lanes, pr = threadIdx.x / lanes;
  const int nh = nm + (with_plain ? 1 : 0);
  const float* mb = masks + (int64_t)b * P * nm;
  for (int cbase = 0; cbase < c4n; cbase += lanes) {
    const int c = (cbase + cl) * 4;
    float4 a0[GGM_MAXH], a1[GGM_MAXH];
#pragma unroll
    for (int h = 0; h < GGM_MAXH; ++h) { a0[h] = make_float4(0.f, 0.f, 0.f, 0.f); a1[h] = make_float4(-INFINITY, -INFINITY, -INFINITY, -INFINITY); }
    if (c < C) {
      for (int p = pbeg + pr; p < pend; p += rows) {
        const float4 v = st_ld4<XS>(x, ((int64_t)b * P + p) * ld + c);
        float m[GGM_MAXH];
#pragma unroll
        for (int h = 0; h < GGM_MAXH; ++h) {
          const int mi = h - (with_plain ? 1 : 0);
          m[h] = (mi < 0) ? 1.f : (mi < nm ? mb[(int64_t)p * nm + mi] : 0.f);
        }
#pragma unroll
        for (int h = 0; h < GGM_MAXH; ++h) {
          if (h < nh) {
            const float4 w = make_float4(v.x * m[h], v.y * m[h], v.z * m[h], v.w * m[h]);
            a0[h].x += w.x; a0[h].y += w.y; a0[h].z += w.z; a0[h].w += w.w;
            a1[h].x = fmaxf(a1[h].x, w.x); a1[h].y = fmaxf(a1[h].y, w.y); a1[h].z = fmaxf(a1[h].z, w.z); a1[h].w = fmaxf(a1[h].w, w.w);
          }
        }
      }
    }
#pragma unroll
    for (int h = 0; h < GGM_MAXH; ++h) {
      if (h < nh) {
        s0[threadIdx.x] = a0[h];
        s1[threadIdx.x] = a1[h];
        __syncthreads();
        if (pr == 0 && c < C) {
          float4 t0 = a0[h], t1 = a1[h];
          for (int r = 1; r < rows; ++r) {
            const float4 u = s0[r * lanes + cl], w = s1[r * lanes + cl];
            t0.x += u.x; t0.y += u.y; t0.z += u.z; t0.w += u.w;
            t1.x = fmaxf(t1.x, w.x); t1.y = fmaxf(t1.y, w.y); t1.z = fmaxf(t1.z, w.z); t1.w = fmaxf(t1.w, w.w);
          }
          float4* o = (float4*)(partial + ((((int64_t)h * B + b) * nchunks + chunk) * C + c) * 2);
          o[0] = make_float4(t0.x, t1.x, t0.y, t1.y);
          o[1] = make_float4(t0.z, t1.z, t0.w, t1.w);
        }
        __syncthreads();
      }
    }
  }
}
extern "C" int64_t ppst_gap_gmp_multi_ws(int B, int64_t hw, int C, int heads) {
  if (B <= 0 || hw <= 0 || heads <= 0) return 0;
  return cdiv64(hw, pix_chunk(B, hw)) * C * 2 * B * heads * (int64_t)sizeof(float);
}
extern "C" int ppst_gap_gmp_multi(const void* x, const void* masks, void* out, void* ws, int B, int H, int W, int C, int ld, int nm,
                                  int with_plain, int x_st, void* stream) {
  if ((unsigned)x_st > 2u) return PPST_EINVAL;
  if (B < 0 || H <= 0 || W <= 0 || C <= 0 || C % 4 || ld % 4 || ld < C || nm < 1 || nm > 3 || (with_plain != 0 && with_plain != 1))
    return PPST_EINVAL;
  if (B == 0) return PPST_OK;
  if (!x || !masks || !out || !ws) return PPST_ENULL;
  if ((int64_t)H * W > 0x7fffffffll || ((uintptr_t)x % (x_st ? 8 : 16))) return PPST_EINVAL;
  const int chunk = pix_chunk(B, (int64_t)H * W);
  const int nchunks = (int)cdiv64((int64_t)H * W, chunk), heads = nm + with_plain;
  PPST_ST_SWITCH(x_st, PPST_LAUNCH(gap_gmp_multi_kernel<ST_>, dim3(nchunks, B), dim3(256), 0, as_stream(stream), x, (const float*)masks,
                                   (float*)ws, H * W, C, ld, nm, with_plain, B, nchunks, chunk));
  int e = PPST_LAUNCH_CHECK();
  if (e) return e;
  PPST_LAUNCH(gap_gmp_finalize_kernel, dim3(heads * B * cdiv(C, FIN_CH)), dim3(256), 0, as_stream(stream), (const float*)ws, nchunks,
              (float*)out, heads * B, C, (double)H * W);
  return PPST_LAUNCH_CHECK();
}

__global__ __launch_bounds__(256) void avgpool_kernel(const float* __restrict__ x, float* __restrict__ y, int H, int W,
                                                      int C, int x_ld, int f, int y_ld, unsigned total, FastDiv d_c,
                                                      FastDiv d_ow, FastDiv d_oh) {
  const int OH = H / f, OW = W / f;
  const float inv = 1.f / (float)(f * f);
  for (uint64_t t64 = (uint64_t)blockIdx.x * 256 + threadIdx.x; t64 < total; t64 += (uint64_t)gridDim.x * 256) {
    unsigned cq, oxu, oyu;
    unsigned r = fd_divmod((unsigned)t64, d_c, cq);
    r = fd_divmod(r, d_ow, oxu);
    const int b = (int)fd_divmod(r, d_oh, oyu);
    const int c = (int)cq * 4, ox = (int)oxu, oy = (int)oyu;
    float4 acc = make_float4(0.f, 0.f, 0.f, 0.f);
    for (int dy = 0; dy < f; ++dy)
      for (int dx = 0; dx < f; ++dx) {
        float4 v = *(const float4*)(x + (((int64_t)b * H + oy * f + dy) * W + ox * f + dx) * x_ld + c);
        acc.x += v.x; acc.y += v.y; acc.z += v.z; acc.w += v.w;
      }
    *(float4*)(y + (((int64_t)b * OH + oy) * OW + ox) * y_ld + c) = make_float4(acc.x * inv, acc.y * inv, acc.z * inv, acc.w * inv);
  }
}
extern "C" int ppst_avgpool(const void* x, void* y, int B, int H, int W, int C, int x_ld, int f, int y_ld, void* stream) {
  if (B < 0 || H <= 0 || W <= 0 || C <= 0 || C % 4 || x_ld % 4 || y_ld % 4 || f <= 0 || H % f || W % f || x_ld < C || y_ld < C)
    return PPST_EINVAL;
  if (B == 0) return PPST_OK;
  if (!x || !y) return PPST_ENULL;
  int64_t total = (int64_t)B * (H / f) * (W / f) * (C / 4);
  if (total > PPST_IDX32_MAX) return PPST_EINVAL;
  PPST_LAUNCH(avgpool_kernel, dim3(grid_for(total)), dim3(256), 0, as_stream(stream), (const float*)x, (float*)y,
                     H, W, C, x_ld, f, y_ld, (unsigned)total, make_fastdiv(C / 4), make_fastdiv(W / f), make_fastdiv(H / f));
  return PPST_LAUNCH_CHECK();
}

__global__ __launch_bounds__(256) void bilinear_kernel(const float* __restrict__ x, float* __restrict__ y, int H, int W,
                                                       int C, int x_ld, int OH, int OW, int y_ld, unsigned total,
                                                       FastDiv d_c, FastDiv d_ow, FastDiv d_oh) {
  const float sh = (float)H / (float)OH, sw = (float)W / (float)OW;
  for (uint64_t t64 = (uint64_t)blockIdx.x * 256 + threadIdx.x; t64 < total; t64 += (uint64_t)gridDim.x * 256) {
    unsigned cq, oxu, oyu;
    unsigned r = fd_divmod((unsigned)t64, d_c, cq);
    r = fd_divmod(r, d_ow, oxu);
    const int b = (int)fd_divmod(r, d_oh, oyu);
    const int c = (int)cq * 4, ox = (int)oxu, oy = (int)oyu;
    float fy = fmaxf(((float)oy + 0.5f) * sh - 0.5f, 0.f);
    float fx = fmaxf(((float)ox + 0.5f) * sw - 0.5f, 0.f);
    int y0 = (int)fy, x0 = (int)fx;
    int y1 = y0 + (y0 < H - 1), x1 = x0 + (x0 < W - 1);
    float ly = fy - (float)y0, lx = fx - (float)x0;
    float hy = 1.f - ly, hx = 1.f - lx;
    const float* base = x + (int64_t)b * H * W * x_ld + c;
    float4 v00 = *(const float4*)(base + ((int64_t)y0 * W + x0) * x_ld);
    float4 v01 = *(const float4*)(base + ((int64_t)y0 * W + x1) * x_ld);
    float4 v10 = *(const float4*)(base + ((int64_t)y1 * W + x0) * x_ld);
    float4 v11 = *(const float4*)(base + ((int64_t)y1 * W + x1) * x_ld);
    float4 o;
    o.x = hy * (hx * v00.x + lx * v01.x) + ly * (hx * v10.x + lx * v11.x);
    o.y = hy * (hx * v00.y + lx * v01.y) + ly * (hx * v10.y + lx * v11.y);
    o.z = hy * (hx * v00.z + lx * v01.z) + ly * (hx * v10.z + lx * v11.z);
    o.w = hy * (hx * v00.w + lx * v01.w) + ly * (hx * v10.w + lx * v11.w);
    *(float4*)(y + (((int64_t)b * OH + oy) * OW + ox) * y_ld + c) = o;
  }
}
extern "C" int ppst_bilinear(const void* x, void* y, int B, int H, int W, int C, int x_ld, int OH, int OW, int y_ld,
                             void* stream) {
  if (B < 0 || H <= 0 || W <= 0 || C <= 0 || C % 4 || x_ld % 4 || y_ld % 4 || OH <= 0 || OW <= 0 || x_ld < C || y_ld < C)
    return PPST_EINVAL;
  if (B == 0) return PPST_OK;
  if (!x || !y) return PPST_ENULL;
  int64_t total = (int64_t)B * OH * OW * (C / 4);
  if (total > PPST_IDX32_MAX) return PPST_EINVAL;
  PPST_LAUNCH(bilinear_kernel, dim3(grid_for(total)), dim3(256), 0, as_stream(stream), (const float*)x, (float*)y,
                     H, W, C, x_ld, OH, OW, y_ld, (unsigned)total, make_fastdiv(C / 4), make_fastdiv(OW), make_fastdiv(OH));
  return PPST_LAUNCH_CHECK();
}

__global__ __launch_bounds__(256) void head_tail_kernel(const float* __restrict__ x, const float* __restrict__ ss,
                                                        const float* __restrict__ prelu, float* __restrict__ feat,
                                                        float* __restrict__ feat1, int H, int W, int C, int x_ld, int f_ld,
                                                        int f1_ld, int P, int D, int actf, unsigned total, FastDiv d_c,
                                                        FastDiv d_w, FastDiv d_h) {
  const int act = actf & 0xff;
  const float slope = (act == PPST_ACT_PRELU && prelu) ? prelu[0] : 0.f;
  const int OW = W / P, OH = H / P, W1 = W / D, H1 = H / D;
// ... 73 lines not shown
  if ((unsigned)st > 2u) return PPST_EINVAL;
  if (st) {
    if (C % 8) return PPST_EINVAL;
    C /= 2;
  }
  if (B < 0 || H <= 0 || W <= 0 || C <= 0 || C % 4) return PPST_EINVAL;
  if (B == 0) return PPST_OK;
  if (!x || !y) return PPST_ENULL;
  int64_t total = (int64_t)B * 4 * H * W * (C / 4);
  if (total > PPST_IDX32_MAX) return PPST_EINVAL;
  PPST_LAUNCH(upsample_nearest2_kernel, dim3(grid_for(total)), dim3(256), 0, as_stream(stream), (const float4*)x,
                     (float4*)y, H, W, C / 4, (unsigned)total, make_fastdiv(C / 4), make_fastdiv(2 * W), make_fastdiv(2 * H));
  return PPST_LAUNCH_CHECK();
}
extern "C" int ppst_upsample_nearest2(const void* x, void* y, int B, int H, int W, int C, void* stream) {
  return ppst_upsample_nearest2_st(x, y, B, H, W, C, PPST_ST_F32, stream);
}

__global__ __launch_bounds__(256) void maxpool2_kernel(const float* __restrict__ x, float* __restrict__ y, int H, int W, int C,
                                                       unsigned total, FastDiv d_c, FastDiv d_ow, FastDiv d_oh) {
  for (uint64_t t64 = (uint64_t)blockIdx.x * 256 + threadIdx.x; t64 < total; t64 += (uint64_t)gridDim.x * 256) {
    const unsigned t = (unsigned)t64;
    unsigned cq, oxu, oyu;
    unsigned r = fd_divmod(t, d_c, cq);
    r = fd_divmod(r, d_ow, oxu);
    const int b = (int)fd_divmod(r, d_oh, oyu);
    const int c = (int)cq, ox = (int)oxu, oy = (int)oyu;
    const float* p = x + (((int64_t)b * H + oy * 2) * W + ox * 2) * C + c;
    y[t] = fmaxf(fmaxf(p[0], p[C]), fmaxf(p[(int64_t)W * C], p[(int64_t)W * C + C]));
  }
}
extern "C" int ppst_maxpool2(const void* x, void* y, int B, int H, int W, int C, void* stream) {
  if (B < 0 || H <= 1 || W <= 1 || C <= 0) return PPST_EINVAL;
  if (B == 0) return PPST_OK;
  if (!x || !y) return PPST_ENULL;
  int64_t total = (int64_t)B * (H / 2) * (W / 2) * C;
  if (total > PPST_IDX32_MAX) return PPST_EINVAL;
  PPST_LAUNCH(maxpool2_kernel, dim3(grid_for(total)), dim3(256), 0, as_stream(stream), (const float*)x, (float*)y, H, W, C,
              (unsigned)total, make_fastdiv(C), make_fastdiv(W / 2), make_fastdiv(H / 2));
  return PPST_LAUNCH_CHECK();
}

template <int YS = PPST_ST_F32>
__global__ __launch_bounds__(256) void conv1x1_small_cin_kernel(const float* __restrict__ x, const float* __restrict__ w,
                                                                const float* __restrict__ bias, void* __restrict__ y,
                                                                int64_t npix, int cin, int in_ld, int cout, float wscale,
                                                                int act, FastDiv d_c) {
  const unsigned t0 = blockIdx.x * 256 + threadIdx.x;
  unsigned cq;
  int64_t p = fd_divmod(t0, d_c, cq);
  const int64_t pstep = ((int64_t)gridDim.x * 256) / d_c.d;
  const int co = (int)cq * 4;
  float wr[4][4], br[4];
#pragma unroll
  for (int j = 0; j < 4; ++j) {
    br[j] = bias ? bias[co + j] : 0.f;
#pragma unroll
    for (int ci = 0; ci < 4; ++ci) wr[j][ci] = ci < cin ? w[(co + j) * cin + ci] * wscale : 0.f;
  }
  for (; p < npix; p += pstep) {
    float xv[4];
#pragma unroll
    for (int ci = 0; ci < 4; ++ci) xv[ci] = ci < cin ? x[p * in_ld + ci] : 0.f;
    float o[4];
#pragma unroll
    for (int j = 0; j < 4; ++j) {
      float acc = 0.f;
#pragma unroll
      for (int ci = 0; ci < 4; ++ci) acc += xv[ci] * wr[j][ci];
      o[j] = act_apply(acc + br[j], act, 0.f);
    }
    st_st4<YS>(y, p * cout + co, make_float4(o[0], o[1], o[2], o[3]));
  }
}
extern "C" int ppst_conv1x1_small_cin_st(const void* x, const void* w, const void* bias, void* y, int64_t npix, int cin,
                                         int in_ld, int cout, float wscale, int act, int y_st, void* stream) {
  if ((unsigned)y_st > 2u) return PPST_EINVAL;
  if (npix < 0 || cin <= 0 || cin > 4 || in_ld < cin || cout <= 0 || cout % 4) return PPST_EINVAL;
  if (npix == 0) return PPST_OK;
  if (!x || !w || !y) return PPST_ENULL;
  const int c4n = cout / 4;
  int64_t total = npix * c4n;
  int g = c4n, t256 = 256;
  while (t256) { int r = g % t256; g = t256; t256 = r; }
  const int unit = c4n / g;
  int64_t blocks = (int64_t)grid_for(total);
  blocks = ((blocks + unit - 1) / unit) * unit;
  PPST_ST_SWITCH(y_st, PPST_LAUNCH(conv1x1_small_cin_kernel<ST_>, dim3((unsigned)blocks), dim3(256), 0, as_stream(stream), (const float*)x,
                                   (const float*)w, (const float*)bias, y, npix, cin, in_ld, cout, wscale, act, make_fastdiv(c4n)));
  return PPST_LAUNCH_CHECK();
}
extern "C" int ppst_conv1x1_small_cin(const void* x, const void* w, const void* bias, void* y, int64_t npix, int cin,
                                      int in_ld, int cout, float wscale, int act, void* stream) {
  return ppst_conv1x1_small_cin_st(x, w, bias, y, npix, cin, in_ld, cout, wscale, act, PPST_ST_F32, stream);
}

template <int XS = PPST_ST_F32>
__global__ __launch_bounds__(256) void conv1x1_small_cout_kernel(const void* __restrict__ x, const float* __restrict__ w,
                                                                 const float* __restrict__ bias, float* __restrict__ y,
                                                                 int64_t npix, int cin, int cout, float wscale) {
  const int hl = threadIdx.x & 31;
  const int64_t half_id = ((int64_t)blockIdx.x * 256 + threadIdx.x) >> 5;
  const int64_t nhalf = ((int64_t)gridDim.x * 256) >> 5;
  for (int64_t p = half_id; p < npix; p += nhalf) {
    float acc[4] = {0.f, 0.f, 0.f, 0.f};
    for (int c = hl * 4; c < cin; c += 128) {
      float4 v = st_ld4<XS>(x, p * cin + c);
      for (int j = 0; j < cout; ++j) {
        float4 ww = *(const float4*)(w + (int64_t)j * cin + c);
        acc[j] += v.x * ww.x + v.y * ww.y + v.z * ww.z + v.w * ww.w;
      }
    }
#pragma unroll
    for (int o = 16; o > 0; o >>= 1)
#pragma unroll
      for (int j = 0; j < 4; ++j) acc[j] += __shfl_xor(acc[j], o, 64);
    if (hl < cout) {
      float r = hl == 0 ? acc[0] : hl == 1 ? acc[1] : hl == 2 ? acc[2] : acc[3];
      y[p * cout + hl] = r * wscale + (bias ? bias[hl] : 0.f);
    }
  }
}
template <int XS = PPST_ST_F32>
__global__ __launch_bounds__(256) void conv1x1_cout3_kernel(const void* __restrict__ x, const float* __restrict__ w,
// ... 223 lines not shown
```

### ppst_amd/csrc/upfirdn2d.hip

```cpp
#include "common.h"
#include <stdlib.h>

#define UF_MAXK 8

struct UfParams {
  int major, in_h, in_w, minor, kh, kw;
  int up_x, up_y, down_x, down_y, pad_x0, pad_y0;
  int out_h, out_w;
  const float* k;
  int pad_mode;
  const float* in_ss;
  int in_act;
};

__device__ __forceinline__ int uf_reflect(int i, int n) {
  if (i < 0) i = -i;
  if (i >= n) i = 2 * (n - 1) - i;
  return i < 0 ? 0 : (i >= n ? n - 1 : i);
}

template <int KH, int KW, int ST = PPST_ST_F32>
__global__ __launch_bounds__(256) void upfirdn2d_planes(const void* __restrict__ x, void* __restrict__ y, UfParams p) {
  constexpr int TH = 32, TW = 64, IH = TH + KH - 1, IW = TW + KW - 1;
  __shared__ float sx[IH][IW + 1];
  float kf[KH * KW];
#pragma unroll
  for (int i = 0; i < KH * KW; ++i) kf[i] = p.k[KH * KW - 1 - i];
  const int tiles_x = (p.out_w + TW - 1) / TW;
  const int tile_x = (blockIdx.x % tiles_x) * TW;
  const int tile_y = (blockIdx.x / tiles_x) * TH;
  const int64_t plane = blockIdx.y;
  const int64_t xp = plane * (int64_t)p.in_h * p.in_w, yp = plane * (int64_t)p.out_h * p.out_w;
  const int in_x0 = tile_x - p.pad_x0, in_y0 = tile_y - p.pad_y0;
  for (int i = threadIdx.x; i < IH * IW; i += 256) {
    int ry = i / IW, rx = i - ry * IW;
    int iy = in_y0 + ry, ix = in_x0 + rx;
    float v = 0.f;
    if (iy >= 0 && iy < p.in_h && ix >= 0 && ix < p.in_w) v = st_ld1<ST>(x, xp + (int64_t)iy * p.in_w + ix);
    sx[ry][rx] = v;
  }
  __syncthreads();
  const int lane = threadIdx.x & 63, w = threadIdx.x >> 6;
  const int ox = tile_x + lane;
  float win[KH][KW];
#pragma unroll
  for (int r = 0; r < KH - 1; ++r)
#pragma unroll
    for (int c = 0; c < KW; ++c) win[r + 1][c] = sx[w * 8 + r][lane + c];
#pragma unroll
  for (int r = 0; r < 8; ++r) {
#pragma unroll
    for (int rr = 0; rr < KH - 1; ++rr)
#pragma unroll
      for (int c = 0; c < KW; ++c) win[rr][c] = win[rr + 1][c];
#pragma unroll
    for (int c = 0; c < KW; ++c) win[KH - 1][c] = sx[w * 8 + r + KH - 1][lane + c];
    float acc = 0.f;
#pragma unroll
    for (int ky = 0; ky < KH; ++ky)
#pragma unroll
      for (int kx = 0; kx < KW; ++kx) acc += win[ky][kx] * kf[ky * KW + kx];
    int oy = tile_y + w * 8 + r;
    if (oy < p.out_h && ox < p.out_w) st_st1<ST>(y, yp + (int64_t)oy * p.out_w + ox, acc);
  }
}

#ifndef UF_PY
#define UF_PY 4
#endif
template <int KH, int KW, int DOWN, bool S2D, int ST = PPST_ST_F32, int CV = 4>
__global__ __launch_bounds__(256) void upfirdn2d_chan(const void* __restrict__ x, void* __restrict__ y, UfParams p, unsigned nwork,
                                                      FastDiv d_c, FastDiv d_xs, FastDiv d_oh) {
  constexpr int PX = 4, PY = (DOWN == 1) ? (CV == 8 ? UF_PY / 2 : UF_PY) : 1;
  constexpr int NQ = CV / 4;
  const int cvn = p.minor / CV;
  float kf[KH * KW];
#pragma unroll
  for (int i = 0; i < KH * KW; ++i) kf[i] = p.k[KH * KW - 1 - i];
  const int ew = S2D ? ((p.out_w + 1) & ~1) : p.out_w;
  const unsigned nblk = (nwork + 255u) >> 8, per = (nblk + 7u) >> 3;
  auto ldv = [&](float4 (&v)[NQ], int64_t item) {
    if (CV == 8) st_ld8<ST>(x, item * 8, v[0], v[NQ - 1]);
    else v[0] = st_ld4<ST>(x, item * 4);
  };
  auto stv = [&](int64_t item, const float4 (&v)[NQ]) {
    if (CV == 8) st_st8<ST>(y, item * 8, v[0], v[NQ - 1]);
    else st_st4<ST>(y, item * 4, v[0]);
  };
  for (unsigned v = blockIdx.x; v < per * 8u; v += gridDim.x) {
    const unsigned wblk = (v & 7u) * per + (v >> 3);
    const uint64_t t64 = (uint64_t)wblk * 256 + threadIdx.x;
    if (wblk >= nblk || t64 >= nwork) continue;
    unsigned cqu, sxu, oyu;
    unsigned r = fd_divmod((unsigned)t64, d_c, cqu);
    r = fd_divmod(r, d_xs, sxu);
    const int m = (int)fd_divmod(r, d_oh, oyu);
    const int cq = (int)cqu, oy0 = (int)oyu * PY;
    int ox0 = (int)sxu * PX;
    float4 acc[PY][PX][NQ];
#pragma unroll
    for (int j = 0; j < PY; ++j)
#pragma unroll
      for (int i = 0; i < PX; ++i)
#pragma unroll
        for (int q = 0; q < NQ; ++q) acc[j][i][q] = make_float4(0.f, 0.f, 0.f, 0.f);
    float4 sa[NQ], sb[NQ];
#pragma unroll
    for (int q = 0; q < NQ; ++q) { sa[q] = make_float4(1.f, 1.f, 1.f, 1.f); sb[q] = make_float4(0.f, 0.f, 0.f, 0.f); }
    if (p.in_ss) {
#pragma unroll
      for (int q = 0; q < NQ; ++q) {
        const float4* qp = (const float4*)(p.in_ss + ((int64_t)m * p.minor + cq * CV + q * 4) * 2);
        float4 q0 = qp[0], q1 = qp[1];
        sa[q] = make_float4(q0.x, q0.z, q1.x, q1.z); sb[q] = make_float4(q0.y, q0.w, q1.y, q1.w);
      }
    }
    const bool any_row = oy0 < p.out_h;
#pragma unroll
    for (int ry = 0; ry < (PY - 1) * DOWN + KH; ++ry) {
      int iy = oy0 * DOWN + ry - p.pad_y0;
      if (p.pad_mode == PPST_PAD_REFLECT) iy = uf_reflect(iy, p.in_h);
      bool yok = any_row && iy >= 0 && iy < p.in_h;
      const int64_t row = ((int64_t)m * p.in_h + (yok ? iy : 0)) * p.in_w * cvn + cq;
#pragma unroll
      for (int j = 0; j < (PX - 1) * DOWN + KW; ++j) {
        int ix = ox0 * DOWN + j - p.pad_x0;
        if (p.pad_mode == PPST_PAD_REFLECT) ix = uf_reflect(ix, p.in_w);
        float4 vv[NQ];
#pragma unroll
        for (int q = 0; q < NQ; ++q) vv[q] = make_float4(0.f, 0.f, 0.f, 0.f);
        if (yok && ix >= 0 && ix < p.in_w) {
          ldv(vv, row + (int64_t)ix * cvn);
          if (p.in_ss) {
#pragma unroll
            for (int q = 0; q < NQ; ++q) {
              float4& v = vv[q];
              v.x = sa[q].x * v.x + sb[q].x; v.y = sa[q].y * v.y + sb[q].y; v.z = sa[q].z * v.z + sb[q].z; v.w = sa[q].w * v.w + sb[q].w;
              if (p.in_act == PPST_ACT_LRELU) {
                v.x = (v.x > 0.f ? v.x : v.x * 0.2f) * 1.41421356237309515f; v.y = (v.y > 0.f ? v.y : v.y * 0.2f) * 1.41421356237309515f;
                v.z = (v.z > 0.f ? v.z : v.z * 0.2f) * 1.41421356237309515f; v.w = (v.w > 0.f ? v.w : v.w * 0.2f) * 1.41421356237309515f;
              }
            }
          }
        }
#pragma unroll
        for (int py = 0; py < PY; ++py) {
          const int ky = ry - py * DOWN;
          if (ky < 0 || ky >= KH) continue;
#pragma unroll
          for (int i = 0; i < PX; ++i) {
            int kx = j - i * DOWN;
            if (kx >= 0 && kx < KW) {
              float f = kf[ky * KW + kx];
#pragma unroll
              for (int q = 0; q < NQ; ++q) {
                acc[py][i][q].x += vv[q].x * f; acc[py][i][q].y += vv[q].y * f; acc[py][i][q].z += vv[q].z * f; acc[py][i][q].w += vv[q].w * f;
              }
            }
          }
        }
      }
    }
    float4 zero[NQ];
#pragma unroll
    for (int q = 0; q < NQ; ++q) zero[q] = make_float4(0.f, 0.f, 0.f, 0.f);
#pragma unroll
    for (int py = 0; py < PY; ++py) {
      const int oy = oy0 + py;
      const bool row_ok = oy < p.out_h;
      if (S2D) {
        const int oh2 = (p.out_h + 1) >> 1, ow2 = (p.out_w + 1) >> 1;
        if (oy >= 2 * oh2) continue;
#pragma unroll
        for (int i = 0; i < PX; ++i) {
          int ox = ox0 + i;
          if (ox < ew)
            stv(((((int64_t)m * oh2 + (oy >> 1)) * ow2 + (ox >> 1)) * 4 + (oy & 1) * 2 + (ox & 1)) * cvn + cq,
                (row_ok && ox < p.out_w) ? acc[py][i] : zero);
        }
      } else {
        if (!row_ok) continue;
        const int64_t orow = ((int64_t)m * p.out_h + oy) * p.out_w * cvn + cq;
#pragma unroll
        for (int i = 0; i < PX; ++i)
          if (ox0 + i < p.out_w) stv(orow + (int64_t)(ox0 + i) * cvn, acc[py][i]);
// ... 195 lines not shown
}

template <int ST = PPST_ST_F32>
__global__ __launch_bounds__(256) void upfirdn2d_up2_chan(const void* __restrict__ x, void* __restrict__ y, UfParams p, unsigned total,
                                                          FastDiv d_c, FastDiv d_w, FastDiv d_h) {
  const int c4n = p.minor >> 2;
  for (uint64_t t64 = (uint64_t)blockIdx.x * 256 + threadIdx.x; t64 < total; t64 += (uint64_t)gridDim.x * 256) {
    unsigned c4, oxu, oyu;
    unsigned r = fd_divmod((unsigned)t64, d_c, c4);
    r = fd_divmod(r, d_w, oxu);
    const int m = (int)fd_divmod(r, d_h, oyu);
    const int ox = (int)oxu, oy = (int)oyu;
    float4 acc = make_float4(0.f, 0.f, 0.f, 0.f);
    for (int ky = 0; ky < p.kh; ++ky) {
      const int Y = oy + ky - p.pad_y0;
      if (Y < 0 || (Y & 1) || (Y >> 1) >= p.in_h) continue;
      const int64_t row = ((int64_t)m * p.in_h + (Y >> 1)) * p.in_w * c4n + c4;
      for (int kx = 0; kx < p.kw; ++kx) {
        const int X = ox + kx - p.pad_x0;
        if (X < 0 || (X & 1) || (X >> 1) >= p.in_w) continue;
        const float4 v = st_ld4<ST>(x, (row + (int64_t)(X >> 1) * c4n) * 4);
        const float f = p.k[(p.kh - 1 - ky) * p.kw + (p.kw - 1 - kx)];
        acc.x += v.x * f; acc.y += v.y * f; acc.z += v.z * f; acc.w += v.w * f;
      }
    }
    st_st4<ST>(y, ((((int64_t)m * p.out_h + oy) * p.out_w + ox) * c4n + c4) * 4, acc);
  }
}

template <int KH, int KW, int ST = PPST_ST_F32, int CV = 4>
static int launch_chan(const void* x, void* y, const UfParams& p, int down, bool s2d, hipStream_t st) {
  const int eh = s2d ? ((p.out_h + 1) & ~1) : p.out_h, ew = s2d ? ((p.out_w + 1) & ~1) : p.out_w;
  static const bool no_slide = getenv("PPST_UF_NO_SLIDE") != nullptr;
  if (KH * KW >= 16 && down == 1 && !no_slide && ST != PPST_ST_F32 && eh >= 192) {
    const int bands = cdiv(eh, UF_SLIDE);
    const int64_t nwork = (int64_t)p.major * bands * cdiv(ew, 4) * (p.minor / CV);
    if (nwork > PPST_IDX32_MAX) return PPST_EINVAL;
    int64_t blocks = cdiv64(cdiv64(nwork, 256), 8) * 8;
    if (blocks > 256 * 16) blocks = 256 * 16;
    const FastDiv d_c = make_fastdiv(p.minor / CV), d_xs = make_fastdiv(cdiv(ew, 4)), d_oh = make_fastdiv(bands);
    if (s2d) PPST_LAUNCH((upfirdn2d_slide<KH, KW, true, ST, CV>), dim3((unsigned)blocks), dim3(256), 0, st, x, y, p, (unsigned)nwork, d_c, d_xs, d_oh);
    else PPST_LAUNCH((upfirdn2d_slide<KH, KW, false, ST, CV>), dim3((unsigned)blocks), dim3(256), 0, st, x, y, p, (unsigned)nwork, d_c, d_xs, d_oh);
    return PPST_LAUNCH_CHECK();
  }
  const int upy = CV == 8 ? UF_PY / 2 : UF_PY;
  const int rows = down == 1 ? cdiv(eh, upy) : eh;
  int64_t nwork = (int64_t)p.major * rows * cdiv(ew, 4) * (p.minor / CV);
  if (nwork > PPST_IDX32_MAX) return PPST_EINVAL;
  int64_t blocks = cdiv64(cdiv64(nwork, 256), 8) * 8;
  if (blocks > 256 * 16) blocks = 256 * 16;
  dim3 g((unsigned)blocks), b(256);
  const FastDiv d_c = make_fastdiv(p.minor / CV), d_xs = make_fastdiv(cdiv(ew, 4)), d_oh = make_fastdiv(rows);
  const unsigned nw = (unsigned)nwork;
  if (s2d) PPST_LAUNCH((upfirdn2d_chan<KH, KW, 1, true, ST, CV>), g, b, 0, st, x, y, p, nw, d_c, d_xs, d_oh);
  else if (down == 2) PPST_LAUNCH((upfirdn2d_chan<KH, KW, 2, false, ST, CV>), g, b, 0, st, x, y, p, nw, d_c, d_xs, d_oh);
  else PPST_LAUNCH((upfirdn2d_chan<KH, KW, 1, false, ST, CV>), g, b, 0, st, x, y, p, nw, d_c, d_xs, d_oh);
  return PPST_LAUNCH_CHECK();
}

template <int KH, int KW, int ST = PPST_ST_F32>
static int launch_fast(const void* x, void* y, const UfParams& p, hipStream_t st) {
  if (p.minor == 1) {
    dim3 grid(cdiv(p.out_w, 64) * cdiv(p.out_h, 32), p.major);
    PPST_LAUNCH((upfirdn2d_planes<KH, KW, ST>), grid, dim3(256), 0, st, x, y, p);
  } else {
    return launch_chan<KH, KW, ST>(x, y, p, 1, false, st);
  }
  return PPST_LAUNCH_CHECK();
}

extern "C" int ppst_upfirdn2d(const void* x, const void* k, void* y, int major, int in_h, int in_w, int minor,
                              int kh, int kw, int up_x, int up_y, int down_x, int down_y, int pad_x0, int pad_x1,
                              int pad_y0, int pad_y1, int dtype, void* stream) {
  if (dtype != PPST_F32 && dtype != PPST_F16 && dtype != PPST_BF16 && dtype != PPST_F64) return PPST_EUNSUPPORTED;
  if (dtype != PPST_F32 && (((uintptr_t)x | (uintptr_t)y) % 8)) return PPST_EINVAL;
  if (major != 0 && (!x || !k || !y)) return PPST_ENULL;
  if (major < 0 || in_h <= 0 || in_w <= 0 || minor <= 0 || kh <= 0 || kw <= 0 || kh > UF_MAXK || kw > UF_MAXK ||
      up_x <= 0 || up_y <= 0 || down_x <= 0 || down_y <= 0)
    return PPST_EINVAL;
  UfParams p;
  p.major = major; p.in_h = in_h; p.in_w = in_w; p.minor = minor; p.kh = kh; p.kw = kw;
  p.up_x = up_x; p.up_y = up_y; p.down_x = down_x; p.down_y = down_y; p.pad_x0 = pad_x0; p.pad_y0 = pad_y0;
  p.out_h = (in_h * up_y + pad_y0 + pad_y1 - kh + down_y) / down_y;
  p.out_w = (in_w * up_x + pad_x0 + pad_x1 - kw + down_x) / down_x;
  if (p.out_h <= 0 || p.out_w <= 0) return PPST_EINVAL;
  if (major == 0) return PPST_OK;
  p.in_ss = nullptr; p.in_act = PPST_ACT_NONE;
  p.k = (const float*)k;
  p.pad_mode = PPST_PAD_ZERO;
  hipStream_t st = as_stream(stream);
  const float* xf = (const float*)x;
  float* yf = (float*)y;
  bool fast = up_x == 1 && up_y == 1 && down_x == 1 && down_y == 1 && (minor == 1 || minor % 4 == 0) && kh == kw;
  bool down2 = up_x == 1 && up_y == 1 && down_x == 2 && down_y == 2 && minor % 4 == 0 && kh == kw;
  int64_t n = (int64_t)major * p.out_h * p.out_w * minor;
  if (dtype == PPST_F64) {
    int64_t nb = cdiv64(n, 256);
    if (nb > 256 * 32) nb = 256 * 32;
    PPST_LAUNCH(upfirdn2d_generic_f64, dim3((unsigned)nb), dim3(256), 0, st, (const double*)x, (const double*)k, (double*)y, p, n);
    return PPST_LAUNCH_CHECK();
  }
  if (dtype != PPST_F32) {
#define UF_HALF(ST_)                                                                            \
  do {                                                                                          \
    if (fast && kh == 3) return launch_fast<3, 3, ST_>(x, y, p, st);                            \
    if (fast && kh == 4) return launch_fast<4, 4, ST_>(x, y, p, st);                            \
    if (down2 && kh == 3) return launch_chan<3, 3, ST_>(x, y, p, 2, false, st);                 \
    if (down2 && kh == 4) return launch_chan<4, 4, ST_>(x, y, p, 2, false, st);                 \
    if (up_x == 2 && up_y == 2 && down_x == 1 && down_y == 1 && minor % 4 == 0 && n / 4 <= PPST_IDX32_MAX) {   \
// ... 18 lines not shown
  if (down2 && kh == 4) return launch_chan<4, 4>(xf, yf, p, 2, false, st);
  if (up_x == 2 && up_y == 2 && down_x == 1 && down_y == 1 && minor % 4 == 0 && n / 4 <= PPST_IDX32_MAX &&
      (((uintptr_t)x | (uintptr_t)y) % 16) == 0) {
    int64_t b4 = cdiv64(n / 4, 256);
    if (b4 > 256 * 32) b4 = 256 * 32;
    PPST_LAUNCH(upfirdn2d_up2_chan<PPST_ST_F32>, dim3((unsigned)b4), dim3(256), 0, st, (const void*)xf, (void*)yf, p, (unsigned)(n / 4),
                make_fastdiv((unsigned)(minor / 4)), make_fastdiv((unsigned)p.out_w), make_fastdiv((unsigned)p.out_h));
    return PPST_LAUNCH_CHECK();
  }
  int64_t blocks = cdiv64(n, 256);
  if (blocks > 256 * 32) blocks = 256 * 32;
  PPST_LAUNCH(upfirdn2d_generic<PPST_ST_F32>, dim3((unsigned)blocks), dim3(256), 0, st, xf, yf, p, n);
  return PPST_LAUNCH_CHECK();
}

extern "C" int ppst_blur_nhwc_st(const void* x, const void* k, void* y, int B, int in_h, int in_w, int C, int ksize, int pad0,
                                 int pad1, int pad_mode, int down, int s2d, const void* in_scale_shift, int in_act, int st,
                                 void* stream) {
  if (!x || !k || !y) return PPST_ENULL;
  if ((unsigned)st > 2u) return PPST_EINVAL;
  if (B < 0 || in_h <= 0 || in_w <= 0 || C <= 0 || C % 4 || (ksize != 3 && ksize != 4) || (down != 1 && down != 2) ||
      (s2d && down != 1) || (pad_mode != PPST_PAD_ZERO && pad_mode != PPST_PAD_REFLECT) ||
      (in_act != PPST_ACT_NONE && in_act != PPST_ACT_LRELU) || (in_act != PPST_ACT_NONE && !in_scale_shift))
    return PPST_EINVAL;
  UfParams p;
  p.major = B; p.in_h = in_h; p.in_w = in_w; p.minor = C; p.kh = ksize; p.kw = ksize;
  p.up_x = p.up_y = 1; p.down_x = p.down_y = down; p.pad_x0 = pad0; p.pad_y0 = pad0;
  p.out_h = (in_h + pad0 + pad1 - ksize + down) / down;
  p.out_w = (in_w + pad0 + pad1 - ksize + down) / down;
  p.k = (const float*)k;
  p.pad_mode = pad_mode;
  p.in_ss = (const float*)in_scale_shift; p.in_act = in_act;
  if (p.out_h <= 0 || p.out_w <= 0) return PPST_EINVAL;
  if (B == 0) return PPST_OK;
  static const bool c8_4x4 = getenv("PPST_UF_C8_4X4") != nullptr;
  const bool c8 = st != PPST_ST_F32 && C % 8 == 0 && (((uintptr_t)x | (uintptr_t)y) % 16) == 0 && (ksize == 3 || c8_4x4);
  if (st != PPST_ST_F32 && (((uintptr_t)x | (uintptr_t)y) % 8)) return PPST_EINVAL;
#define UF_GO(K_)                                                                                             \
  do {                                                                                                        \
    if (st == PPST_ST_F16) return c8 ? launch_chan<K_, K_, PPST_ST_F16, 8>(x, y, p, down, s2d != 0, as_stream(stream))   \
                                     : launch_chan<K_, K_, PPST_ST_F16, 4>(x, y, p, down, s2d != 0, as_stream(stream));  \
    if (st == PPST_ST_BF16) return c8 ? launch_chan<K_, K_, PPST_ST_BF16, 8>(x, y, p, down, s2d != 0, as_stream(stream)) \
                                      : launch_chan<K_, K_, PPST_ST_BF16, 4>(x, y, p, down, s2d != 0, as_stream(stream)); \
    return launch_chan<K_, K_, PPST_ST_F32, 4>(x, y, p, down, s2d != 0, as_stream(stream));                   \
  } while (0)
  if (ksize == 3) UF_GO(3);
  UF_GO(4);
#undef UF_GO
}
extern "C" int ppst_blur_nhwc(const void* x, const void* k, void* y, int B, int in_h, int in_w, int C, int ksize, int pad0,
                              int pad1, int pad_mode, int down, int s2d, const void* in_scale_shift, int in_act, void* stream) {
  return ppst_blur_nhwc_st(x, k, y, B, in_h, in_w, C, ksize, pad0, pad1, pad_mode, down, s2d, in_scale_shift, in_act, PPST_ST_F32, stream);
}
```

### ppst_amd/networks/base_network.py

```python
import math

import torch
from torch import nn

from .. import ops, weights

SQRT2 = math.sqrt(2.0)
INV_SQRT2 = 1.0 / SQRT2


class _Node(nn.Module):
    """parameter container (no behaviour)."""


def to_nhwc(x):
    if x.dim() != 4:
        raise RuntimeError("expected a 4-D NCHW tensor")
    v = x.permute(0, 2, 3, 1)
    if v.is_contiguous():
        ops._chk(v, "input")
        return v
    return ops.nchw_to_nhwc(x)


# ... 35 lines not shown
            for part in parts[:-1]:
                node = node._modules[part]
            t = node._parameters.get(parts[-1])
            if t is None:
                t = node._buffers[parts[-1]]
            self._flat[name] = t
        return t

    def _apply(self, fn, *a, **k):
        self._flat.clear()
        self._cache.clear()
        return super()._apply(fn, *a, **k)

    def load_state_dict(self, *a, **k):
        self._flat.clear()
        self._cache.clear()
        return super().load_state_dict(*a, **k)

    def cached(self, key, params, build):
        ver = tuple((id(t), t._version, t.data_ptr()) for t in params) + (ops.PRECISION["value"],)
        hit = self._cache.get(key)
        if hit is not None and hit[0] == ver:
            return hit[1]
        val = build()
        self._cache[key] = (ver, val)
        return val

    def plan(self, wname, kind="conv", scale=1.0):
        w = self.p(wname)
        return self.cached(("plan", wname, kind), [w], lambda: ops.ConvPlan(w, kind=kind, scale=scale))

    def refresh_plans(self):
        plans, keep = [], {}
        for key, (ver, val) in self._cache.items():
            if isinstance(key, tuple) and key and key[0] == "plan" and isinstance(val, ops.ConvPlan) and val.precision != 2 \
                    and val.wparam.data_ptr() == self.p(key[1]).data_ptr():
                plans.append(val)
                keep[key] = (ver, val)
        self._cache.clear()
        if not plans:
            return
        sig = tuple((id(pl), tuple(sorted(map(str, pl._packs)))) for pl in plans)
        hit = self.__dict__.get("_repack")
        if hit is not None and hit[0] == sig:
            ops.run_repack(hit[1])
        else:
            self.__dict__["_repack"] = (sig, ops.repack_plans(plans), plans)
        self._cache.update(keep)

    def print_architecture(self, verbose=False):
        n = sum(p.numel() for p in self.parameters())
        print("[Network %s] Total number of parameters : %.3f M" % (type(self).__name__, n / 1e6))

    def from_rgb(self, x, p, out_dtype=torch.float32):
        w = self.p(p + "Conv.weight")
        return ops.conv1x1_small_cin(x, w, self.p(p + "Act.bias"), 1.0 / math.sqrt(w.shape[1]), ops.ACT_LRELU, out_dtype=out_dtype)

    def _norm_act(self, y, st, count, act_bias=None, act=ops.ACT_NONE, **kw):
        ss = ops.in_finalize(st, count, post_bias=act_bias)
        return ops.affine_act(y, ss, act=act, **kw), ss

    def res_block(self, x, p, blur_pad_mode, norm):
        B, H, W, cin = x.shape
        k = self.p(p + "conv2.Blur.kernel")
        ks = k.shape[0]
        w1, w2, ws = self.p(p + "conv1.Conv.weight"), self.p(p + "conv2.Conv.weight"), self.p(p + "skip.Conv.weight")
        sc1 = 1.0 / math.sqrt(cin * 9)
        scs = 1.0 / math.sqrt(cin)
        conv_pad = ops.PAD_REFLECT if blur_pad_mode == ops.PAD_REFLECT else ops.PAD_ZERO
        pad_c = (ks - 2) + 2
        pad_s = (ks - 2) + 0
        xs, _ = ops.blur_nhwc(x, self.p(p + "skip.Blur.kernel"), (pad_s + 1) // 2, pad_s // 2, ops.PAD_ZERO, down=2)
        if not norm:
            y1 = self.plan(p + "conv1.Conv.weight", scale=sc1)(x, bias=self.p(p + "conv1.Act.bias"), act=ops.ACT_LRELU,
                                                                pad_mode=conv_pad)
            skip = self.plan(p + "skip.Conv.weight", scale=scs)(xs)
            xb, bhw = ops.blur_nhwc(y1, k, (pad_c + 1) // 2, pad_c // 2, blur_pad_mode, s2d=True)
            ohw = ((bhw[0] - 3) // 2 + 1, (bhw[1] - 3) // 2 + 1)
            return self.plan(p + "conv2.Conv.weight", "s2d", sc1)(
                xb, bias=self.p(p + "conv2.Act.bias"), act=ops.ACT_LRELU, residual=skip, res_after_act=True,
                out_scale=INV_SQRT2, out_hw=ohw)
        y1, st1 = self.plan(p + "conv1.Conv.weight", scale=sc1)(x, stats=True, pad_mode=conv_pad)
        ss1 = ops.in_finalize(st1, H * W, post_bias=self.p(p + "conv1.Act.bias"))
        ys, sts = self.plan(p + "skip.Conv.weight", scale=scs)(xs, stats=True)
        xb, bhw = ops.blur_nhwc(y1, k, (pad_c + 1) // 2, pad_c // 2, blur_pad_mode, s2d=True, in_ss=ss1, in_act=ops.ACT_LRELU)
        ohw = ((bhw[0] - 3) // 2 + 1, (bhw[1] - 3) // 2 + 1)
        y2, st2 = self.plan(p + "conv2.Conv.weight", "s2d", sc1)(xb, stats=True, out_hw=ohw)
        cnt = ohw[0] * ohw[1]
        ss_s = ops.in_finalize(sts, cnt)
        ss2 = ops.in_finalize(st2, cnt, post_bias=self.p(p + "conv2.Act.bias"))
        return ops.affine_act(y2, ss2, res=ys, res_scale_shift=ss_s, act=ops.ACT_LRELU, out_scale=INV_SQRT2)
```

### ppst_amd/networks/encoder_col.py

```python
import torch

from .. import ops
from .base_network import BaseNetwork, to_nhwc

TAGS = ["9", "0", "1", "2"]
CH = [32, 64, 128, 256]


class StyleGAN2ResnetEncodercol(BaseNetwork):
    prefix = "E2."

    def _head(self, tag, x, mask=None):
        v = ops.gap_gmp(x, mask)
        w = self.p("conv1x1_%s.weight" % tag)
        v = ops.linear(v, w.reshape(w.shape[0], -1), self.p("conv1x1_%s.bias" % tag))
        q = "projector%s." % tag
        v = ops.linear(v, self.p(q + "1.weight"), self.p(q + "1.bias"), relu_in=True)
        v = ops.linear(v, self.p(q + "3.weight"), self.p(q + "3.bias"), relu_in=True)
        v = ops.linear(v, self.p(q + "5.weight"), self.p(q + "5.bias"), relu_in=True)
        return ops.l2norm_rows(v, 1e-12, 1)

    def trunk(self, x, dtype=torch.float32):
        feats = [self.from_rgb(to_nhwc(x), "FromRGB.", out_dtype=dtype)]
        for i in range(3):
            feats.append(self.res_block(feats[-1], "DownToGlobalCode1.ResBlockDownBy%d." % (2 ** i), ops.PAD_REFLECT, norm=False))
        return feats

    def warp_levels(self, feats, corr):
        B = feats[0].shape[0]
        V = torch.empty((B, 64, 64, sum(CH)), device=corr.device, dtype=torch.float32)
        off = 0
        for f, c in zip(feats, CH):
            assert f.shape[1] == f.shape[2] and f.shape[1] % 64 == 0, "correspondence needs square inputs (64x64 code grid)"
            ops.avgpool(f, f.shape[1] // 64, out=V[..., off:off + c])
            off += c
        Wv = ops.gemm_nn(corr, V.view(B, 4096, sum(CH)), mode="x3").view(B, 64, 64, sum(CH))
        out, off = [], 0
        for f, c in zip(feats, CH):
            sl = Wv[..., off:off + c]
            out.append(sl if f.shape[1] == 64 else ops.bilinear(sl, f.shape[1], f.shape[2]))
            off += c
        return out

    @staticmethod
    def _mask_planes(mask):
        m = to_nhwc(mask)
        if not m.is_contiguous():
            m = m.contiguous()
        levels = [m]
        for _ in range(3):
            levels.append(ops.maxpool2(levels[-1]))
        return levels

    def forward(self, x=None, extract_features=False, mask=None, corrmatrix=None):
        feats = self.trunk(x, ops.act_dtype() if (corrmatrix is None and mask is None) else torch.float32)
        vectors = [self._head(t, f) for t, f in zip(TAGS, feats)]
        vectors_w, pm, pmw = [], [], []
        warped = None
        if corrmatrix is not None:
            if isinstance(corrmatrix, (list, tuple)):
                corrmatrix = corrmatrix[0]
            warped = self.warp_levels(feats, corrmatrix.detach())
            vectors_w = [self._head(t, f) for t, f in zip(TAGS, warped)]
        if mask is not None:
            from .. import glue
            levels = self._mask_planes(mask)
            sw_levels = self._mask_planes(glue.swap(mask)) if warped is not None else None
            for lvl, (t, f) in enumerate(zip(TAGS, feats)):
                for i in range(3):
                    pm.append(self._head(t, f, levels[lvl][..., i].contiguous()))
                    if warped is not None:
                        pmw.append(self._head(t, warped[lvl], sw_levels[lvl][..., i].contiguous()))
            return vectors, pm, vectors_w, pmw
        return vectors, vectors_w
```

### ppst_amd/networks/encoder_con.py

```python
import math

import torch

from .. import ops
from .base_network import BaseNetwork, as_nchw, to_nhwc


class StyleGAN2ResnetEncodercon(BaseNetwork):
    prefix = "E1."

    def forward(self, x, extract_features=False, patch_ids=None):
        x = self.from_rgb(to_nhwc(x), "FromRGB.", out_dtype=ops.act_dtype())
        for i in range(3):
            x = self.res_block(x, "DownToSpatialCode.ResBlockDownBy%d." % (2 ** i), ops.PAD_REFLECT, norm=True)
        B, H, W, C = x.shape
        sc = 1.0 / math.sqrt(C)
        y, st = self.plan("ToSpatialCode.0.Conv.weight", scale=sc)(x, stats=True)
        if ops.FUSE_TAIL["value"]:
            ss = ops.in_finalize(st, H * W, post_bias=self.p("ToSpatialCode.0.Act.bias"))
            y, st = self.plan("ToSpatialCode.1.Conv.weight", scale=sc)(y, bias=self.p("ToSpatialCode.1.Conv.bias"), stats=True,
                                                                       in_ss=ss, in_act=ops.ACT_LRELU)
        else:
            x, _ = self._norm_act(y, st, H * W, self.p("ToSpatialCode.0.Act.bias"), ops.ACT_LRELU)
            y, st = self.plan("ToSpatialCode.1.Conv.weight", scale=sc)(x, bias=self.p("ToSpatialCode.1.Conv.bias"), stats=True)
        sp, _ = self._norm_act(y, st, H * W, out_dtype=torch.float32)
        return as_nchw(sp)
```

### ppst_amd/ops.py

```python
import ctypes
import math
import os
import threading

import torch

from . import _lib
from ._lib import lib, check

PAD_ZERO, PAD_REFLECT, PAD_REPLICATE = 0, 1, 2
ACT_NONE, ACT_LRELU, ACT_PRELU = 0, 1, 2
RES_BEFORE_ACT = 1 << 8

PRECISION = {"value": 0}
TILE_ROWS = {"value": 16}
CONV_VARIANT = {"value": 2}
DUAL_CONVT = {"value": True, "min_blocks": 32}
UP9 = {"value": True, "min_blocks": 64, "min_fill": 0.85}
DIRECT_MAX = {"cout": 64, "nsteps": 40, "cout3x3": 64}
WGRAD_SPLIT = {"blocks": 1024, "min_tiles": 4}
WGRAD_X3 = {"value": True}
STREAM_1X1 = {"value": True}
KSPLIT = {"value": os.environ.get("PPST_KSPLIT", "1") != "0", "max_blocks": 256, "min_steps": 16, "variants": (0, 2, 10)}
KSPLIT_SCRATCH_BYTES = 256 * 512 * 128 * 4
# ... 91 lines not shown

def empty_nhwc(B, H, W, C, like):
    return torch.empty((B, H, W, C), device=like.device, dtype=torch.float32)


def nchw_to_nhwc(x):
    _chk(x, "x")
    x = x.contiguous()
    B, C, H, W = x.shape
    y = torch.empty((B, H, W, C), device=x.device, dtype=torch.float32)
    check(lib.ppst_nchw_to_nhwc(_p(x), _p(y), B, C, H, W, _stream()), "ppst_nchw_to_nhwc")
    return y


def nhwc_to_nchw(x):
    ld = _nhwc_ld(x)
    B, H, W, C = x.shape
    if ld != C:
        raise RuntimeError("nhwc_to_nchw needs a dense tensor")
    y = torch.empty((B, C, H, W), device=x.device, dtype=torch.float32)
    check(lib.ppst_nhwc_to_nchw(_p(x), _p(y), B, C, H, W, _stream()), "ppst_nhwc_to_nchw")
    return y


_DT_F64 = 3


def _chk_op(t, name):
    if t is None:
        return
    if not isinstance(t, torch.Tensor) or not t.is_cuda:
        raise RuntimeError("%s must be a CUDA (HIP) tensor" % name)
    if t.dtype not in _ST and t.dtype != torch.float64:
        raise RuntimeError("%s must be float32, float16, bfloat16 or float64, got %s" % (name, t.dtype))


def upfirdn2d_raw(x4, kernel, up_x, up_y, down_x, down_y, px0, px1, py0, py1):
    _chk_op(x4, "input")
    _chk_op(kernel, "kernel")
    x4 = x4.contiguous()
    f64 = x4.dtype == torch.float64
    kernel = (kernel.double() if f64 else kernel.float()).contiguous()
    major, in_h, in_w, minor = x4.shape
    kh, kw = kernel.shape
    out_h = (in_h * up_y + py0 + py1 - kh + down_y) // down_y
    out_w = (in_w * up_x + px0 + px1 - kw + down_x) // down_x
    y = torch.empty((major, out_h, out_w, minor), device=x4.device, dtype=x4.dtype)
    check(lib.ppst_upfirdn2d(_p(x4), _p(kernel), _p(y), major, in_h, in_w, minor, kh, kw, up_x, up_y, down_x, down_y,
                             px0, px1, py0, py1, _DT_F64 if f64 else _ST[x4.dtype], _stream()), "ppst_upfirdn2d")
    return y


def blur_nhwc(x, kernel, pad0, pad1, pad_mode=PAD_ZERO, down=1, s2d=False, in_ss=None, in_act=ACT_NONE):
    ld = _nhwc_ld(x, half_ok=True)
    B, H, W, C = x.shape
    if ld != C:
        raise RuntimeError("blur_nhwc needs a dense tensor")
    _chk(kernel, "kernel")
    ks = kernel.shape[0]
    oh = (H + pad0 + pad1 - ks + down) // down
    ow = (W + pad0 + pad1 - ks + down) // down
    if s2d:
        y = torch.empty((B, (oh + 1) // 2, (ow + 1) // 2, 4 * C), device=x.device, dtype=x.dtype)
    else:
        y = torch.empty((B, oh, ow, C), device=x.device, dtype=x.dtype)
    _chk(in_ss, "in_ss")
    check(lib.ppst_blur_nhwc_st(_p(x), _p(kernel.contiguous()), _p(y), B, H, W, C, ks, pad0, pad1, pad_mode, down,
                                1 if s2d else 0, _p(in_ss), in_act, _ST[x.dtype], _stream()), "ppst_blur_nhwc")
    return y, (oh, ow)


def fused_bias_act_raw(x, b, ref, act, grad, alpha, scale):
    _chk_op(x, "input")
    x = x.contiguous()
    b = None if (b is None or b.numel() == 0) else b.to(x.dtype).contiguous()
    ref = None if (ref is None or ref.numel() == 0) else ref.to(x.dtype).contiguous()
    _chk_op(b, "bias")
    _chk_op(ref, "refer")
    y = torch.empty_like(x)
    step_b = 1
    for i in range(2, x.dim()):
        step_b *= x.size(i)
    size_b = b.numel() if b is not None else 1
    check(lib.ppst_fused_bias_act(_p(x), _p(b), _p(ref), _p(y), x.numel(), step_b, size_b, act, grad, float(alpha),
                                  float(scale), _DT_F64 if x.dtype == torch.float64 else _ST[x.dtype], _stream()), "ppst_fused_bias_act")
    return y


class ConvPlan:

    _GEOMETRY = {}
    _GEOM_ATTRS = ("kind", "cout", "cin", "k", "bn", "n_groups", "halo", "src", "max_chan", "wstrides", "nsteps", "flop_steps",
                   "early_a", "chunk_starts0", "chunk_starts0_k64", "steps", "src_dev", "chunk_start", "chunks_per_group", "w4_shape", "max_chunk_steps",
                   "min_chunk_steps", "full_cover", "steps_dual", "src_dual", "steps_up9", "steps_k64", "src_k64", "steps_dual_k64",
                   "src_dual_k64")

    def __init__(self, weight, kind="conv", scale=1.0, chan_base=0, precision=None):
        _chk(weight, "weight")
        w = weight.detach().contiguous()
        gkey = (kind, tuple(w.shape), int(chan_base), str(w.device))
        geom = ConvPlan._GEOMETRY.get(gkey)
        if geom is None:
            self._build(w, kind, scale, chan_base, precision)
            ConvPlan._GEOMETRY[gkey] = {a: getattr(self, a) for a in ConvPlan._GEOM_ATTRS if hasattr(self, a)}
            return
        self.__dict__.update(geom)
# ... 352 lines not shown
                return 10, 128, 16
        tiles16 = ((th + 15) // 16) * ((tw + 15) // 16) * self.n_groups
        if (UP9["value"] and allow_up9 and self.kind == "convT" and self.precision == 0 and getattr(self, "steps_up9", None) is not None
                and self.early_a and ((th + 14) // 15) * ((tw + 14) // 15) * (self.cout // 64) >= UP9["min_blocks"]
                and th * tw >= UP9["min_fill"] * (((th + 14) // 15) * 15) * (((tw + 14) // 15) * 15)):
            return "up9", 256, 15
        if (DUAL_CONVT["value"] and self.kind == "convT" and getattr(self, "steps_dual", None) is not None
                and self.cout % 256 != 0 and cv == 2 and self.early_a
                and ((th + 15) // 16) * ((tw + 15) // 16) * 2 * (self.cout // 128) >= DUAL_CONVT["min_blocks"]):
            return "dual", 256, 16
        n256_ok = self.cout % 256 == 0 and tiles16 * (self.cout // 256) >= FAT_MIN_BLOCKS
        aware = BATCH_AWARE["value"] and B is not None and not single and self.bn == 128 and self.early_a and self.halo == 1
        if aware and n256_ok and tiles16 * (self.cout // 256) * B < BATCH_AWARE["fill"]:
            n256_ok = False
        small = (aware and tiles16 * ((self.cout + 127) // 128) * B < BATCH_AWARE["fill"]
                 and not (KSPLIT["value"] and 0 in KSPLIT["variants"]))
        if cv == 2 and self.early_a:
            if n256_ok:
                variant, bn = 2, 256
            elif single:
                if (self.bn == 128 and self.halo == 1 and self.n_groups == 1 and TALL_TILE_SINGLE["value"] and
                        ((th + 31) // 32) * ((tw + 15) // 16) * ((self.cout + 127) // 128) >= TALL_TILE_SINGLE["min_blocks"]):
                    variant, rows = 7, 32
            elif (self.bn == 128 and self.halo == 1 and (small or (TWO_BLOCK_8ROW["value"] and
                  ((th + 7) // 8) * ((tw + 15) // 16) * self.n_groups * ((self.cout + 127) // 128) >= TWO_BLOCK_8ROW["min_blocks"]))):
                rows = 8
        same = (th, tw) == (oh, ow)
        if STREAM_1X1["value"] and self.halo == 0 and self.n_groups == 1 and osy == 1 and same and (oh, ow) == (H, W):
            variant, bn, rows = 4, 64, TILE_ROWS["value"]
        elif (self.halo == 1 and self.n_groups == 1 and osy == 1 and same and self.cout <= DIRECT_MAX["cout"]
              and self.nsteps <= DIRECT_MAX["nsteps"]):
            variant, bn, rows = (6 if (self.kind in ("conv", "dgrad") and self.k == 3) else 5), 64, TILE_ROWS["value"]
        elif (not single and self.kind in ("conv", "dgrad") and self.k == 3 and 64 < self.cout <= DIRECT_MAX["cout3x3"] and same):
            variant, bn, rows = 6, 128, TILE_ROWS["value"]
        return variant, bn, rows

    def _ksplit(self, variant, a, skip):
        if (skip or variant not in KSPLIT["variants"]
                or not (a.tile_rows == 16 or (variant == 0 and a.tile_rows == 8))):
            return 0, None
        cs = self.chunk_starts0_k64 if a.k64 else self.chunk_starts0
        if cs is None or cs[-1] != a.nsteps:
            return 0, None
        if a.dual_b or (variant == 2 and ((self.precision == 0) != (a.io_st == 0) or (a.k64 and not a.halo))):
            return 0, None
        n_tiles = -(-self.cout // a.bn)
        blocks = a.B * lib.ppst_conv_tiles(a.tile_h, a.tile_w, a.tile_rows) * a.n_groups * n_tiles
        max_s, min_steps = {0: (8, KSPLIT["min_steps"]), 2: (4, 24), 10: (2, 36)}[variant]
        return _ksplit_choice(blocks, cs, KSPLIT["max_blocks"], min_steps, max_s)

    def __call__(self, x, bias=None, noise=None, noise_weight=0.0, act=ACT_NONE, prelu=None, stats=False,
                 residual=None, out=None, out_scale=1.0, pad_mode=PAD_ZERO, out_hw=None, res_after_act=False,
                 in_ss=None, in_act=ACT_NONE, in_prelu=None, in_res=None):
        in_ld = _nhwc_ld(x, "conv input", half_ok=True)
        B, H, W, xc = x.shape
        if x.dtype != torch.float32 and {torch.float16: 3, torch.bfloat16: 1}[x.dtype] != self.precision:
            raise RuntimeError("conv input stored as %s needs a plan of the matching single-pass precision mode (plan: mode %d)"
                               % (x.dtype, self.precision))
        need_c = self.max_chan + 32
        if xc < need_c:
            raise RuntimeError("conv input has %d channels (pixel stride %d); the %s plan reads %d" % (xc, in_ld, self.kind, need_c))
        if in_ss is not None and (in_ss.dim() != 3 or in_ss.shape[0] != B or in_ss.shape[1] < need_c or in_ss.shape[2] != 2
                                  or not in_ss.is_contiguous()):
            raise RuntimeError("in_ss must be a contiguous (B=%d, >=%d, 2) table, got %s" % (B, need_c, tuple(in_ss.shape)))
        if self.kind == "convT":
            th, tw, oh, ow, osy = H, W, 2 * H, 2 * W, 2
        elif self.kind == "dgrad_s2d":
            oh, ow = out_hw
            th, tw, osy = (oh + 1) // 2, (ow + 1) // 2, 2
        elif self.kind in ("s2d", "dgrad_s2ds"):
            oh, ow = out_hw
            th, tw, osy = oh, ow, 1
        else:
            th, tw, oh, ow, osy = H, W, H, W, 1
        if out is None:
            out = torch.empty((B, oh, ow, self.cout), device=x.device, dtype=x.dtype)
        out_ld = _nhwc_ld(out, "conv output", half_ok=True)
        if out.dtype != x.dtype or (residual is not None and residual.dtype != x.dtype):
            raise RuntimeError("conv input, residual and output share one storage type (ppst_conv_args.io_st): got %s / %s / %s"
                               % (x.dtype, None if residual is None else residual.dtype, out.dtype))
        if tuple(out.shape) != (B, oh, ow, self.cout):
            raise RuntimeError("conv output must be %s, got %s" % ((B, oh, ow, self.cout), tuple(out.shape)))
        if noise is not None and (noise.numel() != B * oh * ow or not noise.is_contiguous()):
            raise RuntimeError("noise must be a contiguous (B,1,%d,%d) tensor with B = %d rows, got %s" % (oh, ow, B, tuple(noise.shape)))
        if residual is not None and tuple(residual.shape) != (B, oh, ow, self.cout):
            raise RuntimeError("residual must match the output shape %s, got %s" % ((B, oh, ow, self.cout), tuple(residual.shape)))
        for t, n in ((bias, "bias"), (noise, "noise"), (prelu, "prelu")):
            _chk(t, n)
        up9_ok = in_ss is None and residual is None and act != ACT_PRELU and pad_mode == PAD_ZERO
        variant, bn, rows = self.choose_kernel(th, tw, oh, ow, H, W, osy, B, allow_up9=up9_ok)
        if variant == 10 and in_ss is not None and self.cin > 1024:
            variant, bn, rows = self.choose_kernel(th, tw, oh, ow, H, W, osy, B, allow_up9=up9_ok, allow_wino=False)
        k64 = (K64["value"] and x.dtype != torch.float32 and self.precision in (1, 3) and variant in (2, 7, "dual")
               and (self.steps_dual_k64 if variant == "dual" else self.steps_k64) is not None)
        if k64 and variant == 7:
            variant, rows = 9, 24
        st = None
        if stats:
            tiles = lib.ppst_conv_tiles(th, tw, rows)
            st = torch.empty((B, (1 if variant == "up9" else self.n_groups) * tiles, self.cout, 2), device=x.device, dtype=torch.float32)
        a = _lib.ConvArgs()
        dual, up9 = variant == "dual", variant == "up9"
        if dual:
            variant = 2
        if up9:
            variant = 11
        if k64:
            wp = self.pack_k64(bn, dual)
            steps_t = self.steps_dual_k64 if dual else self.steps_k64
        else:
            wp = None if self.precision == 2 else (self.pack_wino() if variant == 10 else self.pack_up9() if up9 else self.pack_dual() if dual
                                                   else self.pack_for(bn))
            steps_t = self.steps_up9 if up9 else self.steps_dual if dual else self.steps
        a.x, a.wpack, a.steps, a.y = _p(x), _p(wp), _p(steps_t), _p(out)
        a.k64 = 1 if k64 else 0
        a.variant = variant
        a.dual_b = 1 if dual else 0
        a.bias, a.noise, a.prelu, a.stats = _p(bias), _p(noise), _p(prelu), _p(st)
        a.residual = _p(residual)
        a.res_ld = _nhwc_ld(residual, "residual", half_ok=True) if residual is not None else 0
        a.io_st = _ST[x.dtype]
        a.noise_weight, a.out_scale = float(noise_weight), float(out_scale)
        a.B, a.in_h, a.in_w, a.in_ld = B, H, W, in_ld
        a.out_h, a.out_w, a.out_ld, a.cout = oh, ow, out_ld, self.cout
        a.nsteps, a.n_groups, a.pad_mode = (self.nsteps // 2 if k64 else self.nsteps), (1 if up9 else 2 if dual else self.n_groups), pad_mode
        a.in_off_y = a.in_off_x = 0
        a.out_sy = a.out_sx = osy
        a.act, a.precision = act | (0x100 if res_after_act else 0), self.precision
        a.tile_h, a.tile_w, a.halo, a.bn, a.tile_rows = th, tw, self.halo, bn, rows
        _chk(in_ss, "in_ss"); _chk(in_prelu, "in_prelu")
        a.in_scale_shift, a.in_prelu, a.in_act = _p(in_ss), _p(in_prelu), in_act
        a.in_c = in_ss.shape[1] if in_ss is not None else 0
        if in_res is not None:
            if variant != 4 or in_ss is None or self.precision != 0 or x.dtype != torch.float32:
                raise RuntimeError("in_res needs a 1x1 plan on the streaming kernel (ops.STREAM_1X1), in_ss, precision 0 and fp32 storage")
            if tuple(in_res.shape) != tuple(x.shape):
                raise RuntimeError("in_res must have the conv input's shape %s, got %s" % (tuple(x.shape), tuple(in_res.shape)))
            a.in_res, a.in_res_ld = _p(in_res), _nhwc_ld(in_res, "in_res")
        a.flop_steps = self.flop_steps
        a.a_slots = min(3, self.chunks_per_group)
        a.early_a = self.early_a
        ks_S, ks_cuts = self._ksplit(variant, a, self.precision == 2) if (KSPLIT["value"] and BATCH_AWARE["value"]) else (0, None)
        stream = _stream()
        if ks_S:
            ks_arr = (ctypes.c_int32 * (ks_S + 1))(*ks_cuts)
            a.ksplit, a.ksplit_starts = ks_S, ctypes.cast(ks_arr, ctypes.c_void_p)
            a.ksplit_scratch, a.ksplit_flags, a.ksplit_epoch = _ksplit_next(stream)
        if self.precision == 2:
            sn, sc, sy, sx = self.wstrides
            c_, ky_, kx_ = self.src_dev
            check(lib.ppst_conv2d_f32(ctypes.byref(a), _p(self.wsrc), sn, sc, sy, sx, self.scale, _p(c_), _p(ky_), _p(kx_), stream),
                  "ppst_conv2d_f32")
        else:
            check(lib.ppst_conv2d_mfma(ctypes.byref(a), stream), "ppst_conv2d_mfma")
        if stats:
            return out, st
        return out


class _KsWorkspace:
    __slots__ = ("scratch", "flags", "ptrs", "launches")

    def __init__(self):
        self.scratch = torch.empty(KSPLIT_SCRATCH_BYTES, dtype=torch.uint8, device="cuda")
        self.flags = torch.zeros(KSPLIT_FLAG_WORDS, dtype=torch.int32, device="cuda")
        self.ptrs = self.scratch.data_ptr(), self.flags.data_ptr()
        self.launches = 0


_ks_ws = {}
_ks_lock = threading.Lock()


def _ks_key(stream):
    return (_cur_device() if _cur_device is not None else torch.cuda.current_device()), stream.value


def _ksplit_next(stream):
    key = _ks_key(stream)
    with _ks_lock:
        ws = _ks_ws.get(key)
        if ws is None:
            ws = _ks_ws[key] = _KsWorkspace()
        ws.launches += 1
        epoch = (ws.launches - 1) % 0xFFFFFFFF + 1
    return ws.ptrs + (epoch,)


def ksplit_launches():
    ws = _ks_ws.get(_ks_key(_stream()))
    return ws.launches if ws is not None else 0


def ksplit_check():
    ws = _ks_ws.get(_ks_key(_stream()))
    if ws is None:
        torch.cuda.current_stream().synchronize()
        return True
    marker = ws.flags[KSPLIT_FLAG_WORDS - 1:]
    if marker.item() == 0:
        return True
    marker.zero_()
    return False


# ... 269 lines not shown


def lsgan(pred, target, weight):
    _chk(pred)
    pred = pred.contiguous()
    loss = torch.empty((1,), device=pred.device, dtype=torch.float32)
    grad = torch.empty_like(pred)
    check(lib.ppst_lsgan(_p(pred), _p(loss), _p(grad), pred.numel(), float(target), float(weight), _stream()), "ppst_lsgan")
    return loss, grad


def l1_mean(a, b, weight=1.0):
    _chk(a); _chk(b)
    a, b = a.contiguous(), b.contiguous()
    assert a.shape == b.shape
    n = a.numel()
    ws = torch.empty(lib.ppst_l1_mean_ws(n) // 4, device=a.device, dtype=torch.float32)
    out = torch.empty((1,), device=a.device, dtype=torch.float32)
    check(lib.ppst_l1_mean(_p(a), _p(b), _p(out), _p(ws), n, float(weight), _stream()), "ppst_l1_mean")
    return out


def rscl_loss(q, k, k0, queue, nce_T=0.07):
    for t in (q, k, k0, queue):
        _chk(t)
    q, k, k0, queue = q.contiguous(), k.contiguous(), k0.contiguous(), queue.contiguous()
    n, C = q.shape
    ws = torch.empty((n,), device=q.device, dtype=torch.float32)
    out = torch.empty((1,), device=q.device, dtype=torch.float32)
    check(lib.ppst_rscl_loss(_p(q), _p(k), _p(k0), _p(queue), _p(out), _p(ws), n, k0.shape[0], C, queue.shape[1], float(nce_T), _stream()),
          "ppst_rscl_loss")
    return out


def adam_step_(p, g, m, v, lr, beta1, beta2, eps, step):
    for t in (p, g, m, v):
        _chk(t)
        assert t.is_contiguous()
    check(lib.ppst_adam_step(_p(p), _p(g), _p(m), _p(v), p.numel(), float(lr), float(beta1), float(beta2), float(eps), int(step),
                             _stream()), "ppst_adam_step")


def conv1x1_small_cin(x, w, bias, wscale, act, out_dtype=torch.float32):
    ld = _nhwc_ld(x)
    B, H, W, cin = x.shape
    cout = w.shape[0]
    y = torch.empty((B, H, W, cout), device=x.device, dtype=out_dtype)
    w2 = w.detach().reshape(cout, cin).contiguous()
    check(lib.ppst_conv1x1_small_cin_st(_p(x), _p(w2), _p(bias), _p(y), B * H * W, cin, ld, cout, float(wscale), act,
                                        _ST[out_dtype], _stream()), "ppst_conv1x1_small_cin")
    return y


def conv1x1_small_cout(x, w, bias, wscale):
    ld = _nhwc_ld(x, half_ok=True)
    B, H, W, cin = x.shape
    assert ld == cin
    cout = w.shape[0]
    y = torch.empty((B, H, W, cout), device=x.device, dtype=torch.float32)
    w2 = w.detach().reshape(cout, cin).contiguous()
    check(lib.ppst_conv1x1_small_cout_st(_p(x), _p(w2), _p(bias), _p(y), B * H * W, cin, cout, float(wscale), _ST[x.dtype], _stream()),
          "ppst_conv1x1_small_cout")
    return y


def torgb_apply(x, scale_shift, res, out_scale, w, bias, wscale):
    ld = _nhwc_ld(x, half_ok=True)
    B, H, W, cin = x.shape
    if ld != cin or w.shape[0] != 3:
        raise RuntimeError("torgb_apply needs a dense input and a 3-channel weight")
    _chk(scale_shift, "scale_shift"); _chk(bias, "bias")
    res_ld = 0
    if res is not None:
        res_ld = _nhwc_ld(res, "res", half_ok=True)
        if res.dtype != x.dtype or tuple(res.shape) != (B, H // 2, W // 2, cin):
            raise RuntimeError("torgb_apply: res must be the half-resolution tensor of x's type")
    if tuple(scale_shift.shape) != (B, cin, 2) or not scale_shift.is_contiguous():
        raise RuntimeError("torgb_apply: scale_shift must be a contiguous (B, C, 2) table")
    y = torch.empty((B, H, W, 3), device=x.device, dtype=torch.float32)
    w2 = w.detach().reshape(3, cin).contiguous()
    check(lib.ppst_torgb_apply_st(_p(x), _p(scale_shift), _p(res), res_ld, float(out_scale), _p(w2), _p(bias), _p(y), B, H, W, cin,
                                  float(wscale), _ST[x.dtype], _stream()), "ppst_torgb_apply")
    return y


def upscale_weight_bwd(dw4, cout, cin, scale=1.0, out=None, accumulate=False):
    _chk(dw4)
    dw = _grad_out(out, (cout, cin, 3, 3), dw4)
    check(lib.ppst_upscale_weight_bwd(_p(dw4.contiguous()), _p(dw), cout, cin, float(scale), 1 if (accumulate and out is not None) else 0,
                                      _stream()), "ppst_upscale_weight_bwd")
    return dw


DGRAD_S2D_STACK = {"value": os.environ.get("PPST_DGRAD_S2D_STACK", "1") != "0", "max_cin": int(os.environ.get("PPST_DGRAD_S2D_MAXCIN", "64"))}


def depth_to_space(x, out_hw):
    ld = _nhwc_ld(x, "depth_to_space input", half_ok=True)
    B, th, tw, c4 = x.shape
    if ld != c4 or c4 % 4:
        raise RuntimeError("depth_to_space needs a dense tensor with 4 C channels")
    oh, ow = out_hw
    y = torch.empty((B, oh, ow, c4 // 4), device=x.device, dtype=x.dtype)
    check(lib.ppst_depth_to_space_st(_p(x), _p(y), B, th, tw, oh, ow, c4 // 4, _ST[x.dtype], _stream()), "ppst_depth_to_space_st")
    return y

# ... 276 lines not shown


def affine_act(x, scale_shift=None, res=None, act=ACT_NONE, prelu=None, out_scale=1.0, res_before_act=False, out=None,
               res_scale_shift=None, res_up2=False, out_dtype=None):
    x_ld = _nhwc_ld(x, half_ok=True)
    B, H, W, C = x.shape
    if out is None:
        out = torch.empty((B, H, W, C), device=x.device, dtype=out_dtype or x.dtype)
    y_ld = _nhwc_ld(out, half_ok=True)
    res_ld = _nhwc_ld(res, "res", half_ok=True) if res is not None else 0
    if res is not None and res.dtype != x.dtype:
        raise RuntimeError("affine_act: res must have the storage type of x (%s), got %s" % (x.dtype, res.dtype))
    _chk(scale_shift, "scale_shift")
    _chk(res_scale_shift, "res_scale_shift")
    _chk(prelu, "prelu")
    if res_up2:
        assert res.shape[1] * 2 == H and res.shape[2] * 2 == W
    flag = act | (RES_BEFORE_ACT if res_before_act else 0)
    check(lib.ppst_affine_act_st(_p(x), _p(scale_shift), _p(res), _p(res_scale_shift), _p(out), B, H * W, C, x_ld, res_ld, y_ld,
                                 flag, _p(prelu), float(out_scale), W if res_up2 else 0, _ST[x.dtype], _ST[out.dtype], _stream()),
          "ppst_affine_act")
    return out


def affine_act_stats(x, scale_shift=None, res=None, act=ACT_NONE, prelu=None, out_scale=1.0, res_before_act=False,
                     res_scale_shift=None, rep_pad=False, res_up2=False):
    x_ld = _nhwc_ld(x)
    B, H, W, C = x.shape
    out = torch.empty((B, H, W, C), device=x.device, dtype=torch.float32)
    res_ld = _nhwc_ld(res, "res") if res is not None else 0
    for t in (scale_shift, res_scale_shift, prelu):
        _chk(t)
    n = ctypes.c_int(0)
    check(lib.ppst_in_stats(None, None, B, H, W, C, x_ld, 0, ctypes.byref(n), None), "ppst_in_stats(size)")
    part = torch.empty((B, n.value, C, 2), device=x.device, dtype=torch.float32)
    flag = act | (RES_BEFORE_ACT if res_before_act else 0)
    check(lib.ppst_affine_act_stats(_p(x), _p(scale_shift), _p(res), _p(res_scale_shift), _p(out), _p(part), B, H, W, C, x_ld,
                                    res_ld, C, flag, _p(prelu), float(out_scale), 1 if rep_pad else 0, 1 if res_up2 else 0,
                                    _stream()),
          "ppst_affine_act_stats")
    return out, part


def upsample_nearest2(x):
    ld = _nhwc_ld(x, half_ok=True)
    B, H, W, C = x.shape
    assert ld == C
    y = torch.empty((B, 2 * H, 2 * W, C), device=x.device, dtype=x.dtype)
    check(lib.ppst_upsample_nearest2_st(_p(x), _p(y), B, H, W, C, _ST[x.dtype], _stream()), "ppst_upsample_nearest2")
    return y


def gap_gmp(x, mask=None):
    ld = _nhwc_ld(x, half_ok=True)
    B, H, W, C = x.shape
    _chk(mask, "mask")
    ws = torch.empty(lib.ppst_gap_gmp_ws(B, H * W, C) // 4, device=x.device, dtype=torch.float32)
    out = torch.empty((B, 2 * C), device=x.device, dtype=torch.float32)
    check(lib.ppst_gap_gmp_st(_p(x), _p(mask), _p(out), _p(ws), B, H, W, C, ld, _ST[x.dtype], _stream()), "ppst_gap_gmp")
    return out


def avgpool(x, f, out=None):
    x_ld = _nhwc_ld(x)
    B, H, W, C = x.shape
    if out is None:
        out = torch.empty((B, H // f, W // f, C), device=x.device, dtype=torch.float32)
    y_ld = _nhwc_ld(out)
    check(lib.ppst_avgpool(_p(x), _p(out), B, H, W, C, x_ld, f, y_ld, _stream()), "ppst_avgpool")
    return out


def bilinear(x, OH, OW, out=None):
    x_ld = _nhwc_ld(x)
    B, H, W, C = x.shape
    if out is None:
        out = torch.empty((B, OH, OW, C), device=x.device, dtype=torch.float32)
    y_ld = _nhwc_ld(out)
    check(lib.ppst_bilinear(_p(x), _p(out), B, H, W, C, x_ld, OH, OW, y_ld, _stream()), "ppst_bilinear")
    return out


def head_tail(x, scale_shift, feat, feat1, act=ACT_NONE, prelu=None):
    x_ld = _nhwc_ld(x)
    B, H, W, C = x.shape
    P, D = H // feat.shape[1], H // feat1.shape[1]
    _chk(scale_shift, "scale_shift"); _chk(prelu, "prelu")
    check(lib.ppst_head_tail(_p(x), _p(scale_shift), _p(prelu), _p(feat), _p(feat1), B, H, W, C, x_ld, _nhwc_ld(feat), _nhwc_ld(feat1),
                             P, D, act, _stream()), "ppst_head_tail")


def maxpool2(x):
    ld = _nhwc_ld(x)
    B, H, W, C = x.shape
    assert ld == C
    y = torch.empty((B, H // 2, W // 2, C), device=x.device, dtype=torch.float32)
    check(lib.ppst_maxpool2(_p(x), _p(y), B, H, W, C, _stream()), "ppst_maxpool2")
    return y


def linear(x, w, bias=None, wscale=1.0, bscale=1.0, relu_in=False, act=ACT_NONE):
    _chk(x, "x"); _chk(w, "weight"); _chk(bias, "bias")
    x = x.contiguous()
    w = w.detach().contiguous()
    B, K = x.shape
    N = w.shape[0]
    assert w.numel() == N * K
    y = torch.empty((B, N), device=x.device, dtype=torch.float32)
    check(lib.ppst_linear(_p(x), _p(w), _p(bias), _p(y), B, K, N, float(wscale), float(bscale), 1 if relu_in else 0, act,
                          _stream()), "ppst_linear")
    return y


def l2norm_rows(x, eps, mode):
    _chk(x)
    x = x.contiguous()
# ... 275 lines not shown
```

Baseline: 159.3 swaps/s (all GPUs).

## Fuse FromRGB 1x1 conv lazily into its consumer kernels (conv3x3, blur, GAP/GMP, avgpool)

Adds a lazy RgbSource wrapper so the FromRGB 1x1 convolution of the encoders is not materialised as a 32-channel tensor. Instead the consumer kernels (direct 3x3 conv, blur downsample, GAP/GMP, avgpool) read the 3-channel image and recompute the 1x1 conv plus leaky ReLU on the fly. This removes a full-resolution 32-channel write and its reads at the cost of redundant per-pixel recomputation in each consumer. Any consumer without a fused path falls back to materialising the tensor.

Measured after the change: 159.5 swaps/s (all GPUs), median of 6. Within noise of the previous version (+0.2%).

```diff
diff --git a/include/ppst_hip.h b/include/ppst_hip.h
--- a/include/ppst_hip.h
+++ b/include/ppst_hip.h
@@ -156,6 +156,17 @@
 int ppst_conv1x1_small_cin_st(const void* x, const void* w, const void* bias, void* y,
                               int64_t npix, int cin, int in_ld, int cout, float wscale,
                               int act, int y_st , void* stream);
+int ppst_conv2d_mfma_rgb(const ppst_conv_args* a, const void* rgb_w, const void* rgb_bias, float rgb_wscale,
+                         int rgb_act, int img_ld, void* stream);
+int ppst_blur_nhwc_rgb(const void* img, const void* rgb_w, const void* rgb_bias, float rgb_wscale, int rgb_act,
+                       int img_ld, const void* k, void* y, int B, int in_h, int in_w, int C, int ksize,
+                       int pad0, int pad1, int pad_mode, int st , void* stream);
+int ppst_gap_gmp_rgb(const void* img, const void* rgb_w, const void* rgb_bias, float rgb_wscale, int rgb_act,
+                     int img_ld, void* out, void* ws, int B, int H, int W, int C, int x_st ,
+                     void* stream);
+int ppst_avgpool_rgb(const void* img, const void* rgb_w, const void* rgb_bias, float rgb_wscale, int rgb_act,
+                     int img_ld, void* y, int B, int H, int W, int C, int f, int y_ld, int x_st ,
+                     void* stream);
 int ppst_conv1x1_small_cout(const void* x, const void* w, const void* bias, void* y,
                             int64_t npix, int cin, int cout, float wscale, void* stream);
 int ppst_conv1x1_small_cout_st(const void* x, const void* w, const void* bias, void* y,
diff --git a/ppst_amd/_lib.py b/ppst_amd/_lib.py
--- a/ppst_amd/_lib.py
+++ b/ppst_amd/_lib.py
@@ -70,6 +70,10 @@
     "ppst_conv_tiles": (i32, [i32, i32, i32]),
     "ppst_conv1x1_small_cin": (i32, [vp, vp, vp, vp, i64, i32, i32, i32, f32, i32, vp]),
     "ppst_conv1x1_small_cin_st": (i32, [vp, vp, vp, vp, i64, i32, i32, i32, f32, i32, i32, vp]),
+    "ppst_conv2d_mfma_rgb": (i32, [ctypes.POINTER(ConvArgs), vp, vp, f32, i32, i32, vp]),
+    "ppst_blur_nhwc_rgb": (i32, [vp, vp, vp, f32, i32, i32, vp, vp] + [i32] * 9 + [vp]),
+    "ppst_gap_gmp_rgb": (i32, [vp, vp, vp, f32, i32, i32, vp, vp] + [i32] * 5 + [vp]),
+    "ppst_avgpool_rgb": (i32, [vp, vp, vp, f32, i32, i32, vp] + [i32] * 7 + [vp]),
     "ppst_conv1x1_small_cout": (i32, [vp, vp, vp, vp, i64, i32, i32, f32, vp]),
     "ppst_conv1x1_small_cout_st": (i32, [vp, vp, vp, vp, i64, i32, i32, f32, i32, vp]),
     "ppst_torgb_apply_st": (i32, [vp, vp, vp, i32, f32, vp, vp, vp, i32, i32, i32, i32, f32, i32, vp]),
diff --git a/ppst_amd/build.py b/ppst_amd/build.py
--- a/ppst_amd/build.py
+++ b/ppst_amd/build.py
@@ -20,7 +20,7 @@
     return "hipcc"
 
 
-HEADERS = [os.path.join(CSRC, "common.h"), os.path.join(CSRC, "rscl_common.h"), os.path.join(HERE, "..", "include", "ppst_hip.h")]
+HEADERS = [os.path.join(CSRC, "common.h"), os.path.join(CSRC, "rscl_common.h"), os.path.join(CSRC, "from_rgb.h"), os.path.join(HERE, "..", "include", "ppst_hip.h")]
 
 
 def _stale(target, deps):
diff --git a/ppst_amd/csrc/conv1x1.hip b/ppst_amd/csrc/conv1x1.hip
--- a/ppst_amd/csrc/conv1x1.hip
+++ b/ppst_amd/csrc/conv1x1.hip
@@ -1,4 +1,5 @@
 #include "common.h"
+#include "from_rgb.h"
 
 struct C1Args {
   const float* x;
@@ -346,10 +347,11 @@
   return __builtin_bit_cast(bf16x8, r);
 }
 
-template <bool INSS, int NT_, int PREC = 0, int IOS = PPST_ST_F32>
-__global__ __launch_bounds__(512, NT_ > 4 ? 2 : 4) void conv3x3_direct_kernel(C1Args a) {
+template <bool INSS, int NT_, int PREC = 0, int IOS = PPST_ST_F32, bool RGB = false>
+__global__ __launch_bounds__(512, NT_ > 4 ? 2 : 4) void conv3x3_direct_kernel(C1Args a, RgbSrc rgb) {
   constexpr int MT = 2, NT = NT_;
   constexpr bool X3 = PREC == 0;
+  static_assert(!RGB || (!INSS && NT_ == 2), "image source: the plain Cin = 32, Cout <= 32 layer");
   static_assert(IOS == PPST_ST_F32 || IOS == (PREC == 3 ? PPST_ST_F16 : PREC == 1 ? PPST_ST_BF16 : -1), "half storage: single-pass modes");
   constexpr int ES = IOS == PPST_ST_F32 ? 4 : 2;
   constexpr int PSTR = (NT > 4 ? 128 : 64) * 16;
@@ -363,6 +365,14 @@
   const int w_beg = blockIdx.x * per, w_end = w_beg + per < total ? w_beg + per : total;
   const int nchunks = a.nsteps / 9;
   const bool keep_b = nchunks == 1 && a.n_tiles == 1;
+  __shared__ float4 srgb[RGB ? 32 : 1];
+  if constexpr (RGB) {
+    if (tid < 32) {
+      float w1[1][4], b1[1];
+      from_rgb_weights<1>(rgb.w, rgb.bias, FROM_RGB_CIN, rgb.wscale, tid, w1, b1);
+      srgb[tid] = make_float4(w1[0][0], w1[0][1], w1[0][2], b1[0]);
+    }
+  }
   for (int wid = w_beg; wid < w_end; ++wid) {
   const int ntile = wid % a.n_tiles;
   int mblk = wid / a.n_tiles;
@@ -370,7 +380,7 @@
   mblk -= b * a.tiles;
   const int tyi = mblk / a.tiles_x, txi = mblk - tyi * a.tiles_x;
   const int oy0 = tyi * 16 + wave * 2, ox = txi * 16 + r16;
-  const unsigned char* xb = (const unsigned char*)a.x + (int64_t)b * a.in_h * a.in_w * a.in_ld * ES;
+  const unsigned char* xb = (const unsigned char*)a.x + (int64_t)b * a.in_h * a.in_w * (RGB ? rgb.ld * 4 : a.in_ld * ES);
   const unsigned char* wblob = a.wpack + (int64_t)ntile * a.nsteps * BLOB;
   if (wid > w_beg) __syncthreads();
 #if defined(__HIP_DEVICE_COMPILE__)
@@ -403,6 +413,13 @@
     iy = c1_pad(iy, a.in_h, a.pad_mode);
     okc = a.pad_mode != PPST_PAD_ZERO || (yok && cx_ok);
     oke = a.pad_mode != PPST_PAD_ZERO || (yok && ex_ok);
+    if (RGB) {
+      const float* qc = (const float*)xb + ((int64_t)iy * a.in_w + cx) * rgb.ld;
+      const float* qe = (const float*)xb + ((int64_t)iy * a.in_w + ex) * rgb.ld;
+      rawc[0] = make_float4(qc[0], qc[1], qc[2], 0.f);
+      rawe[0] = make_float4(qe[0], qe[1], qe[2], 0.f);
+      return;
+    }
     const float4* pc = (const float4*)(xb + (((int64_t)iy * a.in_w + cx) * a.in_ld + chan + g * 8) * ES);
     const float4* pe = (const float4*)(xb + (((int64_t)iy * a.in_w + ex) * a.in_ld + chan + g * 8) * ES);
     rawc[0] = pc[0];
@@ -416,6 +433,28 @@
     }
   };
   auto convert = [&](const float4 (&raw)[2], bool ok, bf16x8& hi, bf16x8& lo) {
+    if constexpr (RGB) {
+      const float xv[4] = {raw[0].x, raw[0].y, raw[0].z, 0.f};
+      float o[8], rw[8][4], rbias[8];
+      asm volatile("" ::: "memory");
+#pragma unroll
+      for (int j = 0; j < 8; ++j) {
+        const float4 q = srgb[g * 8 + j];
+        rw[j][0] = q.x; rw[j][1] = q.y; rw[j][2] = q.z; rw[j][3] = 0.f; rbias[j] = q.w;
+      }
+      from_rgb_value<8>(xv, rw, rbias, rgb.act, o);
+      if (IOS != PPST_ST_F32) {
+        const uint2 p = st_pack4<IOS>(make_float4(o[0], o[1], o[2], o[3])), q = st_pack4<IOS>(make_float4(o[4], o[5], o[6], o[7]));
+        hi = __builtin_bit_cast(bf16x8, ok ? make_uint4(p.x, p.y, q.x, q.y) : make_uint4(0u, 0u, 0u, 0u));
+        lo = hi;
+        return;
+      }
+      float v[8];
+#pragma unroll
+      for (int j = 0; j < 8; ++j) v[j] = ok ? o[j] : 0.f;
+      c1_cvt8<PREC>(v, hi, lo);
+      return;
+    }
     if (IOS != PPST_ST_F32 && !INSS) {
       hi = __builtin_bit_cast(bf16x8, ok ? raw[0] : make_float4(0.f, 0.f, 0.f, 0.f));
       lo = hi;
@@ -535,8 +574,10 @@
   return PPST_LAUNCH_CHECK();
 }
 
-int ppst_conv3x3_direct_launch(const ppst_conv_args* a, int n_tiles, int tiles_y, int tiles_x, hipStream_t st) {
+int ppst_conv3x3_direct_launch(const ppst_conv_args* a, int n_tiles, int tiles_y, int tiles_x, const RgbSrc* rgb, hipStream_t st) {
   if (a->nsteps % 9) return PPST_EINVAL;
+  if (rgb && (a->nsteps != 9 || a->cout > 32 || a->bn != 64 || a->in_scale_shift || n_tiles != 1)) return PPST_EINVAL;
+  const RgbSrc rs = rgb ? *rgb : RgbSrc{};
   C1Args k;
   k.x = (const float*)a->x; k.wpack = (const unsigned char*)a->wpack; k.steps = (const int4*)a->steps; k.y = (float*)a->y;
   k.bias = (const float*)a->bias; k.noise = (const float*)a->noise; k.prelu = (const float*)a->prelu;
@@ -552,12 +593,17 @@
   const bool nt2 = a->cout <= 32, nt8 = a->bn == 128;
 #define LD3(INSS_, PREC_, IOS_)                                                                                      \
   do {                                                                                                               \
-    if (nt8 && PREC_ == 0) PPST_LAUNCH((conv3x3_direct_kernel<INSS_, 8, 0>), dim3((unsigned)blocks), dim3(512), 0, st, k);   \
+    if (nt8 && PREC_ == 0) PPST_LAUNCH((conv3x3_direct_kernel<INSS_, 8, 0>), dim3((unsigned)blocks), dim3(512), 0, st, k, rs);   \
     else if (nt8) return PPST_EUNSUPPORTED;                                                                          \
-    else if (nt2) PPST_LAUNCH((conv3x3_direct_kernel<INSS_, 2, PREC_, IOS_>), dim3((unsigned)blocks), dim3(512), 0, st, k); \
-    else PPST_LAUNCH((conv3x3_direct_kernel<INSS_, 4, PREC_, IOS_>), dim3((unsigned)blocks), dim3(512), 0, st, k);          \
+    else if (nt2) PPST_LAUNCH((conv3x3_direct_kernel<INSS_, 2, PREC_, IOS_>), dim3((unsigned)blocks), dim3(512), 0, st, k, rs); \
+    else PPST_LAUNCH((conv3x3_direct_kernel<INSS_, 4, PREC_, IOS_>), dim3((unsigned)blocks), dim3(512), 0, st, k, rs);          \
   } while (0)
-#define LD3P(PREC_, IOS_) do { if (k.in_ss) LD3(true, PREC_, IOS_); else LD3(false, PREC_, IOS_); } while (0)
+#define LD3P(PREC_, IOS_)                                                                                            \
+  do {                                                                                                               \
+    if (rgb) PPST_LAUNCH((conv3x3_direct_kernel<false, 2, PREC_, IOS_, true>), dim3((unsigned)blocks), dim3(512), 0, st, k, rs); \
+    else if (k.in_ss) LD3(true, PREC_, IOS_);                                                                        \
+    else LD3(false, PREC_, IOS_);                                                                                    \
+  } while (0)
   if (a->precision == 1) { if (a->io_st) LD3P(1, PPST_ST_BF16); else LD3P(1, PPST_ST_F32); }
   else if (a->precision == 3) { if (a->io_st) LD3P(3, PPST_ST_F16); else LD3P(3, PPST_ST_F32); }
   else LD3P(0, PPST_ST_F32);
diff --git a/ppst_amd/csrc/conv_mfma.hip b/ppst_amd/csrc/conv_mfma.hip
--- a/ppst_amd/csrc/conv_mfma.hip
+++ b/ppst_amd/csrc/conv_mfma.hip
@@ -1,4 +1,5 @@
 #include "common.h"
+#include "from_rgb.h"
 
 struct ConvKArgs {
   const float* x;
@@ -822,7 +823,7 @@
 int ppst_conv2d_mfma2_launch(const ppst_conv_args* a, int n_tiles, int tiles_y, int tiles_x, hipStream_t st);
 int ppst_conv1x1_stream_launch(const ppst_conv_args* a, int n_tiles, int tiles, hipStream_t st);
 int ppst_conv_direct_launch(const ppst_conv_args* a, int n_tiles, int tiles_y, int tiles_x, hipStream_t st);
-int ppst_conv3x3_direct_launch(const ppst_conv_args* a, int n_tiles, int tiles_y, int tiles_x, hipStream_t st);
+int ppst_conv3x3_direct_launch(const ppst_conv_args* a, int n_tiles, int tiles_y, int tiles_x, const RgbSrc* rgb, hipStream_t st);
 int ppst_conv_wino_launch(const ppst_conv_args* a, int n_tiles, int tiles_y, int tiles_x, hipStream_t st);
 
 int ppst_ksplit_prepare_(const ppst_conv_args* a, int64_t tiles, int acc_regs, int threads, KSplitDev* out) {
@@ -852,7 +853,7 @@
   else PPST_LAUNCH((conv_mfma_kernel<WM, WN, HALO, X3, false, NAS, F16, IOS>), grid, dim3(64 * WM * WN), 0, st, k);
 }
 
-extern "C" int ppst_conv2d_mfma(const ppst_conv_args* a, void* stream) {
+static int conv2d_mfma_(const ppst_conv_args* a, const RgbSrc* rgb, void* stream) {
   if (!a) return PPST_ENULL;
   if (a->B < 0 || a->in_h <= 0 || a->in_w <= 0 || a->in_ld <= 0 || a->in_ld % 4 || a->out_h <= 0 || a->out_w <= 0 ||
       a->out_ld < a->cout || a->cout <= 0 || a->cout % 4 || a->out_ld % 4 || (a->residual && a->res_ld % 4) || a->nsteps <= 0 ||
@@ -946,7 +947,7 @@
   if (a->variant >= 1) {
     int e2 = a->variant == 4   ? ppst_conv1x1_stream_launch(a, k.n_tiles, k.tiles_y * k.tiles_x, st)
              : a->variant == 5 ? ppst_conv_direct_launch(a, k.n_tiles, k.tiles_y, k.tiles_x, st)
-             : a->variant == 6 ? ppst_conv3x3_direct_launch(a, k.n_tiles, k.tiles_y, k.tiles_x, st)
+             : a->variant == 6 ? ppst_conv3x3_direct_launch(a, k.n_tiles, k.tiles_y, k.tiles_x, rgb, st)
              : a->variant == 10 ? ppst_conv_wino_launch(a, k.n_tiles, k.tiles_y, k.tiles_x, st)
                                : ppst_conv2d_mfma2_launch(a, k.n_tiles, k.tiles_y, k.tiles_x, st);
     if (slot >= 0) (void)hipEventRecord(g_ev[slot][1], st);
@@ -969,3 +970,13 @@
   if (slot >= 0) (void)hipEventRecord(g_ev[slot][1], st);
   return e;
 }
+extern "C" int ppst_conv2d_mfma(const ppst_conv_args* a, void* stream) { return conv2d_mfma_(a, nullptr, stream); }
+extern "C" int ppst_conv2d_mfma_rgb(const ppst_conv_args* a, const void* rgb_w, const void* rgb_bias, float rgb_wscale, int rgb_act,
+                                    int img_ld, void* stream) {
+  if (!a) return PPST_ENULL;
+  const RgbSrc rs = {(const float*)rgb_w, (const float*)rgb_bias, rgb_wscale, rgb_act, FROM_RGB_CIN, img_ld};
+  if (a->variant != 6 || a->in_ld != 32 || a->nsteps != 9 || a->cout > 32 || a->in_scale_shift || a->ksplit > 1 || !rgb_src_ok(rs, 32))
+    return PPST_EINVAL;
+  if (a->B != 0 && !rgb_w) return PPST_ENULL;
+  return conv2d_mfma_(a, &rs, stream);
+}
diff --git a/ppst_amd/csrc/elementwise.hip b/ppst_amd/csrc/elementwise.hip
--- a/ppst_amd/csrc/elementwise.hip
+++ b/ppst_amd/csrc/elementwise.hip
@@ -1,4 +1,5 @@
 #include "common.h"
+#include "from_rgb.h"
 
 #define GRID_CAP (256 * 16)
 static inline unsigned grid_for(int64_t work, int threads = 256) {
@@ -167,10 +168,12 @@
   int res_ld, y_ld, actf; float out_scale;
   int res_up2;
 };
-template <int MODE, bool APPLY, int XS = PPST_ST_F32>
+template <int MODE, bool APPLY, int XS = PPST_ST_F32, bool RGB = false>
 __global__ __launch_bounds__(256) void chan_reduce4_kernel(const void* __restrict__ x, const float* __restrict__ mask,
                                                            float* __restrict__ partial, int H, int W, int C, int ld,
-                                                           int rep_pad, int nchunks, ApplyArgs ap, int PIX_CHUNK, FastDiv d_w) {
+                                                           int rep_pad, int nchunks, ApplyArgs ap, int PIX_CHUNK, FastDiv d_w,
+                                                           RgbSrc rgb) {
+  static_assert(!RGB || (MODE == 1 && !APPLY), "image source: the mask-free GAP/GMP");
   __shared__ float4 s0[256], s1[256];
   const int b = blockIdx.y, chunk = blockIdx.x;
   const int P = H * W;
@@ -202,11 +205,21 @@
         float4 q0 = q[0], q1 = q[1];
         ra = make_float4(q0.x, q0.z, q1.x, q1.z); rb = make_float4(q0.y, q0.w, q1.y, q1.w);
       }
+      float rw[4][4], rbias[4];
+      if constexpr (RGB) from_rgb_weights<4>(rgb.w, rgb.bias, FROM_RGB_CIN, rgb.wscale, c, rw, rbias);
       for (int p = pbeg + pr; p < pend; p += rows) {
         const int64_t bp = (int64_t)b * P + p;
         unsigned pxu = 0;
         const int py = (APPLY || MODE == 0) ? (int)fd_divmod((unsigned)p, d_w, pxu) : 0, px = (int)pxu;
-        float4 v = st_ld4<XS>(x, bp * ld + c);
+        float4 v;
+        if constexpr (RGB) {
+          float xv[4], o[4];
+          from_rgb_pixel((const float*)x + bp * rgb.ld, FROM_RGB_CIN, xv);
+          from_rgb_stored<XS, 4>(xv, rw, rbias, rgb.act, o);
+          v = make_float4(o[0], o[1], o[2], o[3]);
+        } else {
+          v = st_ld4<XS>(x, bp * ld + c);
+        }
         if (APPLY) {
           float t[4] = {sa.x * v.x + sb.x, sa.y * v.y + sb.y, sa.z * v.z + sb.z, sa.w * v.w + sb.w};
           float r[4] = {0.f, 0.f, 0.f, 0.f};
@@ -269,7 +282,7 @@
   if (C % 4 == 0 && ld % 4 == 0 && ((uintptr_t)x % 16) == 0) {
     ApplyArgs ap = {};
     PPST_LAUNCH((chan_reduce4_kernel<0, false>), dim3(nchunks, B), dim3(256), 0, as_stream(stream), x,
-                (const float*)nullptr, (float*)partial, H, W, C, ld, rep_pad, nchunks, ap, chunk, make_fastdiv(W));
+                (const float*)nullptr, (float*)partial, H, W, C, ld, rep_pad, nchunks, ap, chunk, make_fastdiv(W), RgbSrc{});
   } else {
     PPST_LAUNCH(chan_reduce_kernel<0>, dim3(nchunks, B), dim3(256), 0, as_stream(stream), (const float*)x,
                 (const float*)nullptr, (float*)partial, H, W, C, ld, rep_pad, nchunks, chunk);
@@ -489,7 +502,7 @@
   ap.res_up2 = (res && res_up2) ? 1 : 0;
   if (ap.res_up2 && (H % 2 || W % 2)) return PPST_EINVAL;
   PPST_LAUNCH((chan_reduce4_kernel<0, true>), dim3(nchunks, B), dim3(256), 0, as_stream(stream), x,
-              (const float*)nullptr, (float*)partial, H, W, C, x_ld, rep_pad, nchunks, ap, chunk, make_fastdiv(W));
+              (const float*)nullptr, (float*)partial, H, W, C, x_ld, rep_pad, nchunks, ap, chunk, make_fastdiv(W), RgbSrc{});
   return PPST_LAUNCH_CHECK();
 }
 
@@ -544,14 +557,14 @@
     ApplyArgs ap = {};
     if (x_st == PPST_ST_F16)
       PPST_LAUNCH((chan_reduce4_kernel<1, false, PPST_ST_F16>), dim3(nchunks, B), dim3(256), 0, as_stream(stream), x,
-                  (const float*)mask, (float*)ws, H, W, C, ld, 0, nchunks, ap, chunk, make_fastdiv(W));
+                  (const float*)mask, (float*)ws, H, W, C, ld, 0, nchunks, ap, chunk, make_fastdiv(W), RgbSrc{});
     else
       PPST_LAUNCH((chan_reduce4_kernel<1, false, PPST_ST_BF16>), dim3(nchunks, B), dim3(256), 0, as_stream(stream), x,
-                  (const float*)mask, (float*)ws, H, W, C, ld, 0, nchunks, ap, chunk, make_fastdiv(W));
+                  (const float*)mask, (float*)ws, H, W, C, ld, 0, nchunks, ap, chunk, make_fastdiv(W), RgbSrc{});
   } else if (C % 4 == 0 && ld % 4 == 0 && ((uintptr_t)x % 16) == 0) {
     ApplyArgs ap = {};
     PPST_LAUNCH((chan_reduce4_kernel<1, false>), dim3(nchunks, B), dim3(256), 0, as_stream(stream), x,
-                (const float*)mask, (float*)ws, H, W, C, ld, 0, nchunks, ap, chunk, make_fastdiv(W));
+                (const float*)mask, (float*)ws, H, W, C, ld, 0, nchunks, ap, chunk, make_fastdiv(W), RgbSrc{});
   } else {
     PPST_LAUNCH(chan_reduce_kernel<1>, dim3(nchunks, B), dim3(256), 0, as_stream(stream), (const float*)x,
                 (const float*)mask, (float*)ws, H, W, C, ld, 0, nchunks, chunk);
@@ -565,6 +578,24 @@
 extern "C" int ppst_gap_gmp(const void* x, const void* mask, void* out, void* ws, int B, int H, int W, int C, int ld,
                              void* stream) {
   return ppst_gap_gmp_st(x, mask, out, ws, B, H, W, C, ld, PPST_ST_F32, stream);
+}
+extern "C" int ppst_gap_gmp_rgb(const void* img, const void* rgb_w, const void* rgb_bias, float rgb_wscale, int rgb_act, int img_ld,
+                                void* out, void* ws, int B, int H, int W, int C, int x_st, void* stream) {
+  const RgbSrc rs = {(const float*)rgb_w, (const float*)rgb_bias, rgb_wscale, rgb_act, FROM_RGB_CIN, img_ld};
+  if ((unsigned)x_st > 2u || B < 0 || H <= 0 || W <= 0 || !rgb_src_ok(rs, C)) return PPST_EINVAL;
+  if (B == 0) return PPST_OK;
+  if (!img || !rgb_w || !out || !ws) return PPST_ENULL;
+  if ((int64_t)H * W > 0x7fffffffll) return PPST_EINVAL;
+  const int chunk = pix_chunk(B, (int64_t)H * W);
+  const int nchunks = (int)cdiv64((int64_t)H * W, chunk);
+  ApplyArgs ap = {};
+  PPST_ST_SWITCH(x_st, PPST_LAUNCH((chan_reduce4_kernel<1, false, ST_, true>), dim3(nchunks, B), dim3(256), 0, as_stream(stream), img,
+                                   (const float*)nullptr, (float*)ws, H, W, C, C, 0, nchunks, ap, chunk, make_fastdiv(W), rs));
+  int e = PPST_LAUNCH_CHECK();
+  if (e) return e;
+  PPST_LAUNCH(gap_gmp_finalize_kernel, dim3(B * cdiv(C, FIN_CH)), dim3(256), 0, as_stream(stream),
+                     (const float*)ws, nchunks, (float*)out, B, C, (double)H * W);
+  return PPST_LAUNCH_CHECK();
 }
 
 
@@ -653,9 +684,10 @@
   return PPST_LAUNCH_CHECK();
 }
 
+template <bool RGB = false, int XS = PPST_ST_F32>
 __global__ __launch_bounds__(256) void avgpool_kernel(const float* __restrict__ x, float* __restrict__ y, int H, int W,
                                                       int C, int x_ld, int f, int y_ld, unsigned total, FastDiv d_c,
-                                                      FastDiv d_ow, FastDiv d_oh) {
+                                                      FastDiv d_ow, FastDiv d_oh, RgbSrc rgb) {
   const int OH = H / f, OW = W / f;
   const float inv = 1.f / (float)(f * f);
   for (uint64_t t64 = (uint64_t)blockIdx.x * 256 + threadIdx.x; t64 < total; t64 += (uint64_t)gridDim.x * 256) {
@@ -664,10 +696,21 @@
     r = fd_divmod(r, d_ow, oxu);
     const int b = (int)fd_divmod(r, d_oh, oyu);
     const int c = (int)cq * 4, ox = (int)oxu, oy = (int)oyu;
+    float rw[4][4], rbias[4];
+    if constexpr (RGB) from_rgb_weights<4>(rgb.w, rgb.bias, FROM_RGB_CIN, rgb.wscale, c, rw, rbias);
     float4 acc = make_float4(0.f, 0.f, 0.f, 0.f);
     for (int dy = 0; dy < f; ++dy)
       for (int dx = 0; dx < f; ++dx) {
-        float4 v = *(const float4*)(x + (((int64_t)b * H + oy * f + dy) * W + ox * f + dx) * x_ld + c);
+        const int64_t pix = ((int64_t)b * H + oy * f + dy) * W + ox * f + dx;
+        float4 v;
+        if constexpr (RGB) {
+          float xv[4], o[4];
+          from_rgb_pixel(x + pix * rgb.ld, FROM_RGB_CIN, xv);
+          from_rgb_stored<XS, 4>(xv, rw, rbias, rgb.act, o);
+          v = make_float4(o[0], o[1], o[2], o[3]);
+        } else {
+          v = *(const float4*)(x + pix * x_ld + c);
+        }
         acc.x += v.x; acc.y += v.y; acc.z += v.z; acc.w += v.w;
       }
     *(float4*)(y + (((int64_t)b * OH + oy) * OW + ox) * y_ld + c) = make_float4(acc.x * inv, acc.y * inv, acc.z * inv, acc.w * inv);
@@ -680,8 +723,22 @@
   if (!x || !y) return PPST_ENULL;
   int64_t total = (int64_t)B * (H / f) * (W / f) * (C / 4);
   if (total > PPST_IDX32_MAX) return PPST_EINVAL;
-  PPST_LAUNCH(avgpool_kernel, dim3(grid_for(total)), dim3(256), 0, as_stream(stream), (const float*)x, (float*)y,
-                     H, W, C, x_ld, f, y_ld, (unsigned)total, make_fastdiv(C / 4), make_fastdiv(W / f), make_fastdiv(H / f));
+  PPST_LAUNCH((avgpool_kernel<false>), dim3(grid_for(total)), dim3(256), 0, as_stream(stream), (const float*)x, (float*)y,
+                     H, W, C, x_ld, f, y_ld, (unsigned)total, make_fastdiv(C / 4), make_fastdiv(W / f), make_fastdiv(H / f), RgbSrc{});
+  return PPST_LAUNCH_CHECK();
+}
+extern "C" int ppst_avgpool_rgb(const void* img, const void* rgb_w, const void* rgb_bias, float rgb_wscale, int rgb_act, int img_ld,
+                                void* y, int B, int H, int W, int C, int f, int y_ld, int x_st, void* stream) {
+  const RgbSrc rs = {(const float*)rgb_w, (const float*)rgb_bias, rgb_wscale, rgb_act, FROM_RGB_CIN, img_ld};
+  if ((unsigned)x_st > 2u || B < 0 || H <= 0 || W <= 0 || !rgb_src_ok(rs, C) || y_ld % 4 || f <= 0 || H % f || W % f || y_ld < C)
+    return PPST_EINVAL;
+  if (B == 0) return PPST_OK;
+  if (!img || !rgb_w || !y) return PPST_ENULL;
+  int64_t total = (int64_t)B * (H / f) * (W / f) * (C / 4);
+  if (total > PPST_IDX32_MAX) return PPST_EINVAL;
+  PPST_ST_SWITCH(x_st, PPST_LAUNCH((avgpool_kernel<true, ST_>), dim3(grid_for(total)), dim3(256), 0, as_stream(stream), (const float*)img,
+                                   (float*)y, H, W, C, C, f, y_ld, (unsigned)total, make_fastdiv(C / 4), make_fastdiv(W / f),
+                                   make_fastdiv(H / f), rs));
   return PPST_LAUNCH_CHECK();
 }
 
@@ -861,24 +918,11 @@
   const int64_t pstep = ((int64_t)gridDim.x * 256) / d_c.d;
   const int co = (int)cq * 4;
   float wr[4][4], br[4];
-#pragma unroll
-  for (int j = 0; j < 4; ++j) {
-    br[j] = bias ? bias[co + j] : 0.f;
-#pragma unroll
-    for (int ci = 0; ci < 4; ++ci) wr[j][ci] = ci < cin ? w[(co + j) * cin + ci] * wscale : 0.f;
-  }
+  from_rgb_weights<4>(w, bias, cin, wscale, co, wr, br);
   for (; p < npix; p += pstep) {
-    float xv[4];
-#pragma unroll
-    for (int ci = 0; ci < 4; ++ci) xv[ci] = ci < cin ? x[p * in_ld + ci] : 0.f;
-    float o[4];
-#pragma unroll
-    for (int j = 0; j < 4; ++j) {
-      float acc = 0.f;
-#pragma unroll
-      for (int ci = 0; ci < 4; ++ci) acc += xv[ci] * wr[j][ci];
-      o[j] = act_apply(acc + br[j], act, 0.f);
-    }
+    float xv[4], o[4];
+    from_rgb_pixel(x + p * in_ld, cin, xv);
+    from_rgb_value<4>(xv, wr, br, act, o);
     st_st4<YS>(y, p * cout + co, make_float4(o[0], o[1], o[2], o[3]));
   }
 }
diff --git a/ppst_amd/csrc/from_rgb.h b/ppst_amd/csrc/from_rgb.h
--- /dev/null
+++ b/ppst_amd/csrc/from_rgb.h
@@ -0,0 +1,59 @@
+#pragma once
+#include "common.h"
+
+#define FROM_RGB_CIN 3
+
+struct RgbSrc {
+  const float* w;
+  const float* bias;
+  float wscale;
+  int act;
+  int cin, ld;
+};
+
+template <int N>
+__device__ __forceinline__ void from_rgb_weights(const float* __restrict__ w, const float* __restrict__ bias, int cin, float wscale,
+                                                 int co, float (&wr)[N][4], float (&br)[N]) {
+#pragma clang fp contract(off)
+#pragma unroll
+  for (int j = 0; j < N; ++j) {
+    br[j] = bias ? bias[co + j] : 0.f;
+#pragma unroll
+    for (int ci = 0; ci < 4; ++ci) wr[j][ci] = ci < cin ? w[(co + j) * cin + ci] * wscale : 0.f;
+  }
+}
+__device__ __forceinline__ void from_rgb_pixel(const float* __restrict__ px, int cin, float (&xv)[4]) {
+#pragma unroll
+  for (int ci = 0; ci < 4; ++ci) xv[ci] = ci < cin ? px[ci] : 0.f;
+}
+template <int N>
+__device__ __forceinline__ void from_rgb_value(const float (&xv)[4], const float (&wr)[N][4], const float (&br)[N], int act,
+                                               float (&o)[N]) {
+#pragma clang fp contract(off)
+#pragma unroll
+  for (int j = 0; j < N; ++j) {
+    float acc = 0.f;
+#pragma unroll
+    for (int ci = 0; ci < 4; ++ci) acc += xv[ci] * wr[j][ci];
+    float t = acc + br[j];
+    if (act == PPST_ACT_LRELU) t = (t > 0.f ? t : t * 0.2f) * 1.41421356237309515f;
+    else if (act == PPST_ACT_PRELU) t = t >= 0.f ? t : t * 0.f;
+    o[j] = t;
+  }
+}
+template <int ST, int N>
+__device__ __forceinline__ void from_rgb_stored(const float (&xv)[4], const float (&wr)[N][4], const float (&br)[N], int act,
+                                                float (&o)[N]) {
+  static_assert(N % 4 == 0, "whole 4-channel items");
+  from_rgb_value<N>(xv, wr, br, act, o);
+  if (ST != PPST_ST_F32) {
+#pragma unroll
+    for (int q = 0; q < N; q += 4) {
+      const float4 r = st_unpack4<ST>(st_pack4<ST>(make_float4(o[q], o[q + 1], o[q + 2], o[q + 3])));
+      o[q] = r.x; o[q + 1] = r.y; o[q + 2] = r.z; o[q + 3] = r.w;
+    }
+  }
+}
+static inline bool rgb_src_ok(const RgbSrc& s, int C) {
+  return s.cin == FROM_RGB_CIN && s.ld >= s.cin && C > 0 && C % 4 == 0;
+}
diff --git a/ppst_amd/csrc/upfirdn2d.hip b/ppst_amd/csrc/upfirdn2d.hip
--- a/ppst_amd/csrc/upfirdn2d.hip
+++ b/ppst_amd/csrc/upfirdn2d.hip
@@ -1,4 +1,5 @@
 #include "common.h"
+#include "from_rgb.h"
 #include <stdlib.h>
 
 #define UF_MAXK 8
@@ -68,9 +69,10 @@
 #ifndef UF_PY
 #define UF_PY 4
 #endif
-template <int KH, int KW, int DOWN, bool S2D, int ST = PPST_ST_F32, int CV = 4>
+template <int KH, int KW, int DOWN, bool S2D, int ST = PPST_ST_F32, int CV = 4, bool RGB = false>
 __global__ __launch_bounds__(256) void upfirdn2d_chan(const void* __restrict__ x, void* __restrict__ y, UfParams p, unsigned nwork,
-                                                      FastDiv d_c, FastDiv d_xs, FastDiv d_oh) {
+                                                      FastDiv d_c, FastDiv d_xs, FastDiv d_oh, RgbSrc rgb) {
+  static_assert(!RGB || CV == 4, "image source: 4 channels per thread");
   constexpr int PX = 4, PY = (DOWN == 1) ? (CV == 8 ? UF_PY / 2 : UF_PY) : 1;
   constexpr int NQ = CV / 4;
   const int cvn = p.minor / CV;
@@ -115,6 +117,8 @@
         sa[q] = make_float4(q0.x, q0.z, q1.x, q1.z); sb[q] = make_float4(q0.y, q0.w, q1.y, q1.w);
       }
     }
+    float rw[4][4], rbias[4];
+    if constexpr (RGB) from_rgb_weights<4>(rgb.w, rgb.bias, FROM_RGB_CIN, rgb.wscale, cq * 4, rw, rbias);
     const bool any_row = oy0 < p.out_h;
 #pragma unroll
     for (int ry = 0; ry < (PY - 1) * DOWN + KH; ++ry) {
@@ -130,7 +134,14 @@
 #pragma unroll
         for (int q = 0; q < NQ; ++q) vv[q] = make_float4(0.f, 0.f, 0.f, 0.f);
         if (yok && ix >= 0 && ix < p.in_w) {
-          ldv(vv, row + (int64_t)ix * cvn);
+          if constexpr (RGB) {
+            float xv[4], o[4];
+            from_rgb_pixel((const float*)x + (((int64_t)m * p.in_h + iy) * p.in_w + ix) * rgb.ld, FROM_RGB_CIN, xv);
+            from_rgb_stored<ST, 4>(xv, rw, rbias, rgb.act, o);
+            vv[0] = make_float4(o[0], o[1], o[2], o[3]);
+          } else {
+            ldv(vv, row + (int64_t)ix * cvn);
+          }
           if (p.in_ss) {
 #pragma unroll
             for (int q = 0; q < NQ; ++q) {
@@ -432,9 +443,9 @@
   dim3 g((unsigned)blocks), b(256);
   const FastDiv d_c = make_fastdiv(p.minor / CV), d_xs = make_fastdiv(cdiv(ew, 4)), d_oh = make_fastdiv(rows);
   const unsigned nw = (unsigned)nwork;
-  if (s2d) PPST_LAUNCH((upfirdn2d_chan<KH, KW, 1, true, ST, CV>), g, b, 0, st, x, y, p, nw, d_c, d_xs, d_oh);
-  else if (down == 2) PPST_LAUNCH((upfirdn2d_chan<KH, KW, 2, false, ST, CV>), g, b, 0, st, x, y, p, nw, d_c, d_xs, d_oh);
-  else PPST_LAUNCH((upfirdn2d_chan<KH, KW, 1, false, ST, CV>), g, b, 0, st, x, y, p, nw, d_c, d_xs, d_oh);
+  if (s2d) PPST_LAUNCH((upfirdn2d_chan<KH, KW, 1, true, ST, CV>), g, b, 0, st, x, y, p, nw, d_c, d_xs, d_oh, RgbSrc{});
+  else if (down == 2) PPST_LAUNCH((upfirdn2d_chan<KH, KW, 2, false, ST, CV>), g, b, 0, st, x, y, p, nw, d_c, d_xs, d_oh, RgbSrc{});
+  else PPST_LAUNCH((upfirdn2d_chan<KH, KW, 1, false, ST, CV>), g, b, 0, st, x, y, p, nw, d_c, d_xs, d_oh, RgbSrc{});
   return PPST_LAUNCH_CHECK();
 }
 
@@ -559,3 +570,33 @@
                               int pad1, int pad_mode, int down, int s2d, const void* in_scale_shift, int in_act, void* stream) {
   return ppst_blur_nhwc_st(x, k, y, B, in_h, in_w, C, ksize, pad0, pad1, pad_mode, down, s2d, in_scale_shift, in_act, PPST_ST_F32, stream);
 }
+
+extern "C" int ppst_blur_nhwc_rgb(const void* img, const void* rgb_w, const void* rgb_bias, float rgb_wscale, int rgb_act, int img_ld,
+                                  const void* k, void* y, int B, int in_h, int in_w, int C, int ksize, int pad0, int pad1,
+                                  int pad_mode, int st, void* stream) {
+  const RgbSrc rs = {(const float*)rgb_w, (const float*)rgb_bias, rgb_wscale, rgb_act, FROM_RGB_CIN, img_ld};
+  if (!img || !rgb_w || !k || !y) return PPST_ENULL;
+  if ((unsigned)st > 2u || B < 0 || in_h <= 0 || in_w <= 0 || !rgb_src_ok(rs, C) ||
+      (pad_mode != PPST_PAD_ZERO && pad_mode != PPST_PAD_REFLECT))
+    return PPST_EINVAL;
+  if (ksize != 3) return PPST_EUNSUPPORTED;
+  if (st != PPST_ST_F32 && ((uintptr_t)y % 8)) return PPST_EINVAL;
+  UfParams p;
+  p.major = B; p.in_h = in_h; p.in_w = in_w; p.minor = C; p.kh = ksize; p.kw = ksize;
+  p.up_x = p.up_y = 1; p.down_x = p.down_y = 2; p.pad_x0 = pad0; p.pad_y0 = pad0;
+  p.out_h = (in_h + pad0 + pad1 - ksize + 2) / 2;
+  p.out_w = (in_w + pad0 + pad1 - ksize + 2) / 2;
+  p.k = (const float*)k;
+  p.pad_mode = pad_mode;
+  p.in_ss = nullptr; p.in_act = PPST_ACT_NONE;
+  if (p.out_h <= 0 || p.out_w <= 0) return PPST_EINVAL;
+  if (B == 0) return PPST_OK;
+  const int64_t nwork = (int64_t)B * p.out_h * cdiv(p.out_w, 4) * (C / 4);
+  if (nwork > PPST_IDX32_MAX) return PPST_EINVAL;
+  int64_t blocks = cdiv64(cdiv64(nwork, 256), 8) * 8;
+  if (blocks > 256 * 16) blocks = 256 * 16;
+  const FastDiv d_c = make_fastdiv(C / 4), d_xs = make_fastdiv(cdiv(p.out_w, 4)), d_oh = make_fastdiv(p.out_h);
+  PPST_ST_SWITCH(st, PPST_LAUNCH((upfirdn2d_chan<3, 3, 2, false, ST_, 4, true>), dim3((unsigned)blocks), dim3(256), 0, as_stream(stream),
+                                 img, y, p, (unsigned)nwork, d_c, d_xs, d_oh, rs));
+  return PPST_LAUNCH_CHECK();
+}
diff --git a/ppst_amd/networks/base_network.py b/ppst_amd/networks/base_network.py
--- a/ppst_amd/networks/base_network.py
+++ b/ppst_amd/networks/base_network.py
@@ -111,9 +111,10 @@
         n = sum(p.numel() for p in self.parameters())
         print("[Network %s] Total number of parameters : %.3f M" % (type(self).__name__, n / 1e6))
 
-    def from_rgb(self, x, p, out_dtype=torch.float32):
+    def from_rgb(self, x, p, out_dtype=torch.float32, lazy=False):
         w = self.p(p + "Conv.weight")
-        return ops.conv1x1_small_cin(x, w, self.p(p + "Act.bias"), 1.0 / math.sqrt(w.shape[1]), ops.ACT_LRELU, out_dtype=out_dtype)
+        make = ops.from_rgb_source if lazy else ops.conv1x1_small_cin
+        return make(x, w, self.p(p + "Act.bias"), 1.0 / math.sqrt(w.shape[1]), ops.ACT_LRELU, out_dtype=out_dtype)
 
     def _norm_act(self, y, st, count, act_bias=None, act=ops.ACT_NONE, **kw):
         ss = ops.in_finalize(st, count, post_bias=act_bias)
diff --git a/ppst_amd/networks/encoder_col.py b/ppst_amd/networks/encoder_col.py
--- a/ppst_amd/networks/encoder_col.py
+++ b/ppst_amd/networks/encoder_col.py
@@ -20,8 +20,8 @@
         v = ops.linear(v, self.p(q + "5.weight"), self.p(q + "5.bias"), relu_in=True)
         return ops.l2norm_rows(v, 1e-12, 1)
 
-    def trunk(self, x, dtype=torch.float32):
-        feats = [self.from_rgb(to_nhwc(x), "FromRGB.", out_dtype=dtype)]
+    def trunk(self, x, dtype=torch.float32, lazy=True):
+        feats = [self.from_rgb(to_nhwc(x), "FromRGB.", out_dtype=dtype, lazy=lazy)]
         for i in range(3):
             feats.append(self.res_block(feats[-1], "DownToGlobalCode1.ResBlockDownBy%d." % (2 ** i), ops.PAD_REFLECT, norm=False))
         return feats
@@ -53,7 +53,7 @@
         return levels
 
     def forward(self, x=None, extract_features=False, mask=None, corrmatrix=None):
-        feats = self.trunk(x, ops.act_dtype() if (corrmatrix is None and mask is None) else torch.float32)
+        feats = self.trunk(x, ops.act_dtype() if (corrmatrix is None and mask is None) else torch.float32, lazy=mask is None)
         vectors = [self._head(t, f) for t, f in zip(TAGS, feats)]
         vectors_w, pm, pmw = [], [], []
         warped = None
diff --git a/ppst_amd/networks/encoder_con.py b/ppst_amd/networks/encoder_con.py
--- a/ppst_amd/networks/encoder_con.py
+++ b/ppst_amd/networks/encoder_con.py
@@ -10,7 +10,7 @@
     prefix = "E1."
 
     def forward(self, x, extract_features=False, patch_ids=None):
-        x = self.from_rgb(to_nhwc(x), "FromRGB.", out_dtype=ops.act_dtype())
+        x = self.from_rgb(to_nhwc(x), "FromRGB.", out_dtype=ops.act_dtype(), lazy=True)
         for i in range(3):
             x = self.res_block(x, "DownToSpatialCode.ResBlockDownBy%d." % (2 ** i), ops.PAD_REFLECT, norm=True)
         B, H, W, C = x.shape
diff --git a/ppst_amd/ops.py b/ppst_amd/ops.py
--- a/ppst_amd/ops.py
+++ b/ppst_amd/ops.py
@@ -167,6 +167,16 @@
 
 
 def blur_nhwc(x, kernel, pad0, pad1, pad_mode=PAD_ZERO, down=1, s2d=False, in_ss=None, in_act=ACT_NONE):
+    if isinstance(x, RgbSource):
+        if kernel.shape[0] == 3 and down == 2 and not s2d and in_ss is None:
+            _chk(kernel, "kernel")
+            B, H, W, C = x.shape
+            oh, ow = (H + pad0 + pad1 - 3 + 2) // 2, (W + pad0 + pad1 - 3 + 2) // 2
+            y = torch.empty((B, oh, ow, C), device=x.device, dtype=x.dtype)
+            check(lib.ppst_blur_nhwc_rgb(*x.args(), _p(kernel.contiguous()), _p(y), B, H, W, C, 3, pad0, pad1, pad_mode,
+                                         _ST[x.dtype], _stream()), "ppst_blur_nhwc_rgb")
+            return y, (oh, ow)
+        x = x.tensor()
     ld = _nhwc_ld(x, half_ok=True)
     B, H, W, C = x.shape
     if ld != C:
@@ -625,7 +635,16 @@
     def __call__(self, x, bias=None, noise=None, noise_weight=0.0, act=ACT_NONE, prelu=None, stats=False,
                  residual=None, out=None, out_scale=1.0, pad_mode=PAD_ZERO, out_hw=None, res_after_act=False,
                  in_ss=None, in_act=ACT_NONE, in_prelu=None, in_res=None):
-        in_ld = _nhwc_ld(x, "conv input", half_ok=True)
+        rgb = None
+        if isinstance(x, RgbSource):
+            B, H, W, xc = x.shape
+            if (self.kind == "conv" and self.k == 3 and self.nsteps == 9 and self.cout <= 32 and xc == 32 and in_ss is None
+                    and in_res is None and residual is None and self.precision in (0, 1, 3)
+                    and self.choose_kernel(H, W, H, W, H, W, 1, B)[:2] == (6, 64)):
+                rgb = x
+            else:
+                x = x.tensor()
+        in_ld = x.shape[3] if rgb is not None else _nhwc_ld(x, "conv input", half_ok=True)
         B, H, W, xc = x.shape
         if x.dtype != torch.float32 and {torch.float16: 3, torch.bfloat16: 1}[x.dtype] != self.precision:
             raise RuntimeError("conv input stored as %s needs a plan of the matching single-pass precision mode (plan: mode %d)"
@@ -685,7 +704,7 @@
             wp = None if self.precision == 2 else (self.pack_wino() if variant == 10 else self.pack_up9() if up9 else self.pack_dual() if dual
                                                    else self.pack_for(bn))
             steps_t = self.steps_up9 if up9 else self.steps_dual if dual else self.steps
-        a.x, a.wpack, a.steps, a.y = _p(x), _p(wp), _p(steps_t), _p(out)
+        a.x, a.wpack, a.steps, a.y = _p(x.img if rgb is not None else x), _p(wp), _p(steps_t), _p(out)
         a.k64 = 1 if k64 else 0
         a.variant = variant
         a.dual_b = 1 if dual else 0
@@ -724,6 +743,9 @@
             c_, ky_, kx_ = self.src_dev
             check(lib.ppst_conv2d_f32(ctypes.byref(a), _p(self.wsrc), sn, sc, sy, sx, self.scale, _p(c_), _p(ky_), _p(kx_), stream),
                   "ppst_conv2d_f32")
+        elif rgb is not None:
+            check(lib.ppst_conv2d_mfma_rgb(ctypes.byref(a), _p(rgb.w), _p(rgb.bias), rgb.wscale, rgb.act, rgb.img.stride(2), stream),
+                  "ppst_conv2d_mfma_rgb")
         else:
             check(lib.ppst_conv2d_mfma(ctypes.byref(a), stream), "ppst_conv2d_mfma")
         if stats:
@@ -1099,6 +1121,44 @@
     return y
 
 
+class RgbSource:
+    __slots__ = ("img", "w", "bias", "wscale", "act", "dtype", "_t")
+
+    def __init__(self, img, w, bias, wscale, act, dtype):
+        self.img, self.w, self.bias, self.wscale, self.act, self.dtype, self._t = img, w, bias, float(wscale), act, dtype, None
+
+    @property
+    def shape(self):
+        B, H, W, _ = self.img.shape
+        return torch.Size((B, H, W, self.w.shape[0]))
+
+    @property
+    def device(self):
+        return self.img.device
+
+    def tensor(self):
+        if self._t is None:
+            self._t = conv1x1_small_cin(self.img, self.w, self.bias, self.wscale, self.act, out_dtype=self.dtype)
+        return self._t
+
+    def args(self):
+        return _p(self.img), _p(self.w), _p(self.bias), self.wscale, self.act, self.img.stride(2)
+
+
+def from_rgb_source(x, w, bias, wscale, act, out_dtype=torch.float32):
+    cout = w.shape[0]
+    if x.shape[3] != 3 or cout % 4 or x.dtype != torch.float32:
+        return conv1x1_small_cin(x, w, bias, wscale, act, out_dtype=out_dtype)
+    _nhwc_ld(x)
+    _chk(w, "weight")
+    _chk(bias, "bias")
+    return RgbSource(x, w.detach().reshape(cout, 3).contiguous(), bias, wscale, act, out_dtype)
+
+
+def materialise(x):
+    return x.tensor() if isinstance(x, RgbSource) else x
+
+
 def conv1x1_small_cout(x, w, bias, wscale):
     ld = _nhwc_ld(x, half_ok=True)
     B, H, W, cin = x.shape
@@ -1481,6 +1541,14 @@
 
 
 def gap_gmp(x, mask=None):
+    if isinstance(x, RgbSource):
+        if mask is None:
+            B, H, W, C = x.shape
+            ws = torch.empty(lib.ppst_gap_gmp_ws(B, H * W, C) // 4, device=x.device, dtype=torch.float32)
+            out = torch.empty((B, 2 * C), device=x.device, dtype=torch.float32)
+            check(lib.ppst_gap_gmp_rgb(*x.args(), _p(out), _p(ws), B, H, W, C, _ST[x.dtype], _stream()), "ppst_gap_gmp_rgb")
+            return out
+        x = x.tensor()
     ld = _nhwc_ld(x, half_ok=True)
     B, H, W, C = x.shape
     _chk(mask, "mask")
@@ -1491,6 +1559,12 @@
 
 
 def avgpool(x, f, out=None):
+    if isinstance(x, RgbSource):
+        B, H, W, C = x.shape
+        if out is None:
+            out = torch.empty((B, H // f, W // f, C), device=x.device, dtype=torch.float32)
+        check(lib.ppst_avgpool_rgb(*x.args(), _p(out), B, H, W, C, f, _nhwc_ld(out), _ST[x.dtype], _stream()), "ppst_avgpool_rgb")
+        return out
     x_ld = _nhwc_ld(x)
     B, H, W, C = x.shape
     if out is None:
```
